# frosinastojanovska/image-captioning

Hardware: AMD Instinct MI355X
Metric: captions/sec (train step) on 1024px x 32RoI x 15tok synth (higher is better)
Workload: dtype f32 (split-bf16x3 products, fp32 accumulate: 73 of 85 conv layers on the bf16 pipe, the rest and the decoder exact fp32 MFMA); 1 GPU; BASELINE configs[2] (configs[3] at 8 GPUs): frozen ResNet-101+FPN fwd + PyramidROIAlign + RoI head + v2-inject decoder fwd/bwd + AMSGrad, 1024x1024 synth images, 32 RoI/img, 15-token captions, V=10000; backbone=resnet101, images_per_gpu=2, global_batch_images=2, parallelism=dp1, stage4_blocks=22, pipeline=encoder(i+1) || decoder(i), 2 HIP streams, rccl_ranks=1

## Files before the change

### image-captioning_amd/_lib.py

```python
import ctypes as C
import os

_HERE = os.path.dirname(os.path.abspath(__file__))
LIB_PATH = os.path.join(_HERE, "csrc", "libdcap_hip.so")

c_float_p = C.POINTER(C.c_float)
c_int32_p = C.POINTER(C.c_int32)
c_uint8_p = C.POINTER(C.c_uint8)


class GemmDesc(C.Structure):
    _fields_ = [("M", C.c_int), ("N", C.c_int), ("K", C.c_int),
                ("A", C.c_void_p), ("lda", C.c_int), ("a_trans", C.c_int),
                ("a_gather", C.c_void_p),
                ("B", C.c_void_p), ("ldb", C.c_int), ("b_trans", C.c_int),
                ("C", C.c_void_p), ("ldc", C.c_int),
                ("scale", C.c_void_p), ("shift", C.c_void_p),
                ("residual", C.c_void_p), ("ldr", C.c_int), ("res_rows", C.c_int),
                ("relu", C.c_int), ("accumulate", C.c_int), ("split_k", C.c_int)]


class GemmBf16Desc(C.Structure):
    _fields_ = [("M", C.c_int), ("N", C.c_int), ("K", C.c_int),
                ("A", C.c_void_p), ("lda", C.c_int), ("a_trans", C.c_int),
# ... 128 lines not shown


class RpnLossDesc(C.Structure):
    _fields_ = [("levels", C.c_int), ("anchors_per_loc", C.c_int), ("head_stride", C.c_int),
                ("heads", C.c_void_p * 5), ("dheads", C.c_void_p * 5), ("Hs", C.c_int * 5), ("Ws", C.c_int * 5),
                ("n_sel", C.c_int), ("n_pos", C.c_int),
                ("sel_level", C.c_void_p), ("sel_index", C.c_void_p), ("sel_match", C.c_void_p),
                ("target_deltas", C.c_void_p), ("losses", C.c_void_p), ("counts_dev", C.c_void_p)]


class DetectionTargetsDesc(C.Structure):
    _fields_ = [("n_proposals", C.c_int), ("n_gt", C.c_int), ("n_rois", C.c_int), ("T", C.c_int),
                ("proposals", C.c_void_p), ("gt_boxes", C.c_void_p), ("gt_captions", C.c_void_p),
                ("max_positive", C.c_int), ("inv_ratio", C.c_float), ("shuffle", C.c_int),
                ("seed", C.c_uint32), ("offset", C.c_uint32), ("offset_dev", C.c_void_p),
                ("rois", C.c_void_p), ("captions", C.c_void_p), ("counts", C.c_void_p)]


class PwChainDesc(C.Structure):
    _fields_ = [("M", C.c_int), ("K1", C.c_int), ("N1", C.c_int), ("N2", C.c_int),
                ("x", C.c_void_p), ("w1", C.c_void_p), ("scale1", C.c_void_p), ("shift1", C.c_void_p), ("residual", C.c_void_p),
                ("relu1", C.c_int), ("y", C.c_void_p), ("w2", C.c_void_p), ("scale2", C.c_void_p), ("shift2", C.c_void_p),
                ("relu2", C.c_int), ("z", C.c_void_p), ("w1_b3", C.c_void_p), ("w2_b3", C.c_void_p)]


class RegSegments(C.Structure):
    _fields_ = [("start", C.c_void_p), ("coef", C.c_void_p), ("mask", C.c_void_p), ("nseg", C.c_int)]


class AmsgradDesc(C.Structure):
    _fields_ = [("n", C.c_size_t), ("p", C.c_void_p), ("g", C.c_void_p), ("m", C.c_void_p),
                ("v", C.c_void_p), ("vhat", C.c_void_p),
                ("lr_t", C.c_float), ("beta1", C.c_float), ("beta2", C.c_float), ("eps", C.c_float),
                ("grad_scale", C.c_float), ("gnorm_sq", C.c_void_p), ("clipnorm", C.c_float),
                ("p_bf16", C.c_void_p), ("n_bf16", C.c_size_t), ("lr_t_dev", C.c_void_p), ("reg", C.POINTER(RegSegments))]


SYMBOLS = {
    "dc_version": (C.c_int, []),
    "dc_last_error": (C.c_char_p, []),
    "dc_gemm_workspace_bytes": (C.c_size_t, [C.POINTER(GemmDesc)]),
    "dc_gemm_f32": (C.c_int, [C.POINTER(GemmDesc), C.c_void_p, C.c_size_t, C.c_void_p]),
    "dc_gemm_bf16_workspace_bytes": (C.c_size_t, [C.POINTER(GemmBf16Desc)]),
    "dc_gemm_bf16_tile": (C.c_int, [C.POINTER(GemmBf16Desc), C.POINTER(C.c_int)]),
    "dc_gemm_bf16": (C.c_int, [C.POINTER(GemmBf16Desc), C.c_void_p, C.c_size_t, C.c_void_p]),
    "dc_conv2d_wgrad_bf16_workspace_bytes": (C.c_size_t, [C.POINTER(ConvWgradBf16Desc)]),
    "dc_conv2d_wgrad_bf16_tile": (C.c_int, [C.POINTER(ConvWgradBf16Desc), C.POINTER(C.c_int)]),
    "dc_conv2d_wgrad_bf16": (C.c_int, [C.POINTER(ConvWgradBf16Desc), C.c_void_p, C.c_size_t, C.c_void_p]),
    "dc_conv2d_bf16_workspace_bytes": (C.c_size_t, [C.POINTER(ConvBf16Desc)]),
    "dc_conv2d_bf16_tile": (C.c_int, [C.POINTER(ConvBf16Desc), C.POINTER(C.c_int)]),
    "dc_conv2d_bf16": (C.c_int, [C.POINTER(ConvBf16Desc), C.c_void_p, C.c_size_t, C.c_void_p]),
    "dc_cast_f32_bf16": (C.c_int, [C.c_void_p, C.c_void_p, C.c_size_t, C.c_void_p]),
    "dc_cast_bf16_f32": (C.c_int, [C.c_void_p, C.c_void_p, C.c_size_t, C.c_void_p]),
    "dc_cast_f32_bf16_2d": (C.c_int, [C.c_void_p, C.c_int, C.c_void_p, C.c_int, C.c_int, C.c_int, C.c_int, C.c_void_p]),
    "dc_split_bf16x3_f32": (C.c_int, [C.c_void_p, C.c_void_p, C.c_size_t, C.c_void_p]),
    "dc_conv2d_workspace_bytes": (C.c_size_t, [C.POINTER(ConvDesc)]),
    "dc_conv2d_nhwc_f32": (C.c_int, [C.POINTER(ConvDesc), C.c_void_p, C.c_size_t, C.c_void_p]),
    "dc_conv2d_tile_config": (C.c_int, [C.POINTER(ConvDesc), C.POINTER(C.c_int), C.POINTER(C.c_int), C.POINTER(C.c_int)]),
    "dc_conv2d_is_pointwise": (C.c_int, [C.POINTER(ConvDesc)]),
    "dc_conv2d_winograd_weight_bytes": (C.c_size_t, [C.c_int, C.c_int]),
    "dc_conv2d_winograd_pack_f32": (C.c_int, [C.c_void_p, C.c_void_p, C.c_int, C.c_int, C.c_void_p]),
    "dc_pw_chain_supported": (C.c_int, [C.c_int, C.c_int, C.c_int]),
    "dc_pw_chain_pack_f32": (C.c_int, [C.c_void_p, C.c_void_p, C.c_int, C.c_int, C.c_void_p]),
    "dc_pw_chain_pack_b3": (C.c_int, [C.c_void_p, C.c_void_p, C.c_int, C.c_int, C.c_void_p]),
    "dc_pw_chain_f32": (C.c_int, [C.POINTER(PwChainDesc), C.c_void_p]),
    "dc_pw_chain_kernel_name": (C.c_int, [C.POINTER(PwChainDesc), C.c_char_p, C.c_size_t]),
    "dc_conv2d_winograd_b3_weight_bytes": (C.c_size_t, [C.c_int, C.c_int]),
    "dc_conv2d_winograd_pack_b3": (C.c_int, [C.c_void_p, C.c_void_p, C.c_int, C.c_int, C.c_void_p]),
    "dc_conv2d_kernel_name": (C.c_int, [C.POINTER(ConvDesc), C.c_char_p, C.c_size_t]),
    "dc_conv2d_wgrad_workspace_bytes": (C.c_size_t, [C.POINTER(ConvDesc)]),
    "dc_conv2d_wgrad_f32": (C.c_int, [C.POINTER(ConvDesc), C.c_void_p, C.c_size_t, C.c_void_p]),
    "dc_roi_align_pyramid_bwd_f32": (C.c_int, [C.POINTER(RoiAlignDesc), C.c_void_p]),
    "dc_downsample2x_sum_f32": (C.c_int, [C.c_void_p, C.c_void_p, C.c_int, C.c_int, C.c_int, C.c_int, C.c_int, C.c_void_p]),
    "dc_downsample2x_sum_dual_f32": (C.c_int, [C.c_void_p, C.c_void_p, C.c_void_p, C.c_int, C.c_int, C.c_int, C.c_int, C.c_int, C.c_void_p]),
    "dc_maxpool2x2s2_f32": (C.c_int, [C.c_void_p, C.c_void_p, C.c_int, C.c_int, C.c_int, C.c_int, C.c_void_p]),
    "dc_maxpool3x3s2_same_f32": (C.c_int, [C.c_void_p, C.c_void_p, C.c_int, C.c_int, C.c_int, C.c_int, C.c_void_p]),
    "dc_mold_image_padded_f32": (C.c_int, [C.c_void_p, C.c_void_p, C.c_int, C.c_int, C.c_int, C.c_int, C.c_float, C.c_float, C.c_float, C.c_void_p]),
    "dc_mold_image_rgbx_f32": (C.c_int, [C.c_void_p, C.c_void_p, C.c_int, C.c_int, C.c_int,
                                         C.c_float, C.c_float, C.c_float, C.c_void_p]),
    "dc_roi_align_pyramid_f32": (C.c_int, [C.POINTER(RoiAlignDesc), C.c_void_p]),
    "dc_roi_tile_groups": (C.c_int, [C.POINTER(RoiGroupsDesc), C.c_void_p]),
    "dc_conv2d_winograd_group_count": (C.c_int, [C.c_int, C.c_int]),
    "dc_conv2d_winograd_groups_f32": (C.c_int, [C.POINTER(ConvDesc), C.c_void_p, C.c_void_p, C.c_void_p]),
    "dc_subsample2_f32": (C.c_int, [C.c_void_p, C.c_void_p, C.c_int, C.c_int, C.c_int, C.c_int, C.c_void_p]),
    "dc_proposals_workspace_bytes": (C.c_size_t, [C.POINTER(ProposalDesc)]),
    "dc_proposals_f32": (C.c_int, [C.POINTER(ProposalDesc), C.c_void_p, C.c_size_t, C.c_void_p]),
    "dc_lstm_seq_workspace_bytes": (C.c_size_t, [C.c_int, C.c_int, C.c_int]),
    "dc_lstm_seq_fwd_f32": (C.c_int, [C.POINTER(LstmFwdDesc), C.c_void_p, C.c_size_t, C.c_void_p]),
    "dc_lstm_seq_bwd_f32": (C.c_int, [C.POINTER(LstmBwdDesc), C.c_void_p, C.c_size_t, C.c_void_p]),
    "dc_lstm_pack_urec_f32": (C.c_int, [C.c_void_p, C.c_int, C.c_void_p, C.c_void_p]),
    "dc_lstm_step_workspace_bytes": (C.c_size_t, [C.c_int, C.c_int]),
    "dc_lstm_step_f32": (C.c_int, [C.POINTER(LstmStepDesc), C.c_void_p, C.c_size_t, C.c_void_p]),
    "dc_softmax_ce_f32": (C.c_int, [C.POINTER(SoftmaxCeDesc), C.c_void_p]),
    "dc_vocab_ce_workspace_bytes": (C.c_size_t, [C.POINTER(VocabCeDesc)]),
    "dc_vocab_ce": (C.c_int, [C.POINTER(VocabCeDesc), C.c_void_p, C.c_size_t, C.c_void_p]),
    "dc_vocab_top1_workspace_bytes": (C.c_size_t, [C.c_int, C.c_int]),
    "dc_vocab_top1_f32": (C.c_int, [C.POINTER(VocabTop1Desc), C.c_void_p, C.c_size_t, C.c_void_p]),
    "dc_vocab_topk_workspace_bytes": (C.c_size_t, [C.c_int, C.c_int, C.c_int]),
    "dc_vocab_topk_f32": (C.c_int, [C.POINTER(VocabTopkDesc), C.c_void_p, C.c_size_t, C.c_void_p]),
    "dc_vocab_topk_bf16_tile": (C.c_int, [C.c_int, C.c_int, C.c_int]),
    "dc_vocab_top1_bf16_workspace_bytes": (C.c_size_t, [C.c_int, C.c_int, C.c_int, C.c_int]),
    "dc_vocab_topk_bf16_workspace_bytes": (C.c_size_t, [C.c_int, C.c_int, C.c_int, C.c_int, C.c_int]),
    "dc_vocab_top1_bf16": (C.c_int, [C.POINTER(VocabTop1Bf16Desc), C.c_void_p, C.c_size_t, C.c_void_p]),
    "dc_vocab_topk_bf16": (C.c_int, [C.POINTER(VocabTopkBf16Desc), C.c_void_p, C.c_size_t, C.c_void_p]),
    "dc_beam_select_f32": (C.c_int, [C.POINTER(BeamSelectDesc), C.c_void_p]),
    "dc_beam_backtrace": (C.c_int, [C.c_void_p, C.c_void_p, C.c_int, C.c_int, C.c_int, C.c_void_p, C.c_void_p]),
    "dc_argmax_rows_f32": (C.c_int, [C.c_void_p, C.c_int, C.c_int, C.c_int, C.c_void_p, C.c_void_p]),
    "dc_gather_rows_f32": (C.c_int, [C.c_void_p, C.c_int, C.c_void_p, C.c_void_p, C.c_int, C.c_int, C.c_int, C.c_void_p]),
    "dc_bn_relu_fwd_f32": (C.c_int, [C.POINTER(BnReluDesc), C.c_void_p]),
    "dc_bn_relu_bwd_f32": (C.c_int, [C.POINTER(BnReluDesc), C.c_void_p]),
    "dc_conv_weight_dgrad_pack_f32": (C.c_int, [C.c_void_p, C.c_void_p, C.c_int, C.c_int, C.c_int, C.c_int, C.c_void_p]),
    "dc_rpn_loss_grad_f32": (C.c_int, [C.POINTER(RpnLossDesc), C.c_void_p]),
    "dc_scatter2_add_f32": (C.c_int, [C.c_void_p, C.c_void_p, C.c_int, C.c_int, C.c_int, C.c_int, C.c_void_p]),
    "dc_detection_targets_f32": (C.c_int, [C.POINTER(DetectionTargetsDesc), C.c_void_p]),
    "dc_caption_tables_i32": (C.c_int, [C.c_void_p, C.c_int, C.c_int, C.c_void_p, C.c_void_p, C.c_void_p, C.c_void_p, C.c_void_p, C.c_void_p]),
    "dc_set_persistent_cus": (C.c_int, [C.c_int]),
    "dc_get_persistent_cus": (C.c_int, []),
    "dc_l2_reg_workspace_bytes": (C.c_size_t, [C.c_size_t]),
    "dc_l2_reg_f32": (C.c_int, [C.c_void_p, C.c_void_p, C.c_void_p, C.c_void_p, C.c_size_t, C.c_void_p, C.c_void_p, C.c_size_t, C.c_void_p]),
    "dc_axpy_f32": (C.c_int, [C.c_float, C.c_void_p, C.c_void_p, C.c_size_t, C.c_void_p]),
    "dc_relu_bwd_f32": (C.c_int, [C.c_void_p, C.c_void_p, C.c_void_p, C.c_int, C.c_int, C.c_int, C.c_void_p]),
    "dc_relu_bwd_dual_f32": (C.c_int, [C.c_void_p, C.c_void_p, C.c_void_p, C.c_void_p, C.c_size_t, C.c_void_p]),
    "dc_fold_time_f32": (C.c_int, [C.c_void_p, C.c_int, C.c_int, C.c_int, C.c_int, C.c_void_p, C.c_int, C.c_void_p]),
    "dc_colsum_workspace_bytes": (C.c_size_t, [C.c_int, C.c_int, C.c_int]),
    "dc_colsum_f32": (C.c_int, [C.c_void_p, C.c_int, C.c_int, C.c_int, C.c_void_p, C.c_int, C.c_void_p, C.c_size_t, C.c_void_p]),
    "dc_sumsq_workspace_bytes": (C.c_size_t, [C.c_size_t]),
    "dc_sumsq_f32": (C.c_int, [C.c_void_p, C.c_size_t, C.c_void_p, C.c_int, C.c_void_p, C.c_size_t, C.c_void_p]),
    "dc_mean_f32": (C.c_int, [C.c_void_p, C.c_size_t, C.c_void_p, C.c_void_p]),
    "dc_bn_fold_f32": (C.c_int, [C.c_void_p] * 5 + [C.c_float, C.c_void_p, C.c_void_p, C.c_int, C.c_void_p]),
    "dc_bn_bwd_f32": (C.c_int, [C.c_void_p] * 8 + [C.c_long, C.c_int, C.c_void_p]),
    "dc_mul_f32": (C.c_int, [C.c_void_p, C.c_void_p, C.c_void_p, C.c_size_t, C.c_void_p]),
    "dc_maxpool3x3s2_same_bwd_f32": (C.c_int, [C.c_void_p] * 4 + [C.c_int] * 4 + [C.c_void_p]),
    "dc_dropout_mask_f32": (C.c_int, [C.c_void_p, C.c_size_t, C.c_float, C.c_uint32, C.c_uint32, C.c_void_p, C.c_void_p]),
    "dc_amsgrad_step_f32": (C.c_int, [C.POINTER(AmsgradDesc), C.c_void_p]),
    "dc_zero_fill": (C.c_int, [C.c_void_p, C.c_size_t, C.c_void_p]),
    "dc_reg_sumsq_workspace_bytes": (C.c_size_t, [C.c_size_t]),
    "dc_reg_sumsq_f32": (C.c_int, [C.c_void_p, C.c_void_p, C.POINTER(RegSegments), C.c_size_t, C.c_void_p, C.c_void_p, C.c_void_p, C.c_size_t, C.c_void_p]),
}

ABI_VERSION = 600
_lib = None


class DcapError(RuntimeError):
    pass


def load():
    global _lib
    if _lib is not None:
        return _lib
    path = os.environ.get("DCAP_LIB", LIB_PATH)
    if not os.path.exists(path):
        raise DcapError("%s is missing: build it with `python __graft_entry__.py` "
                        "(hipcc --offload-arch=gfx950); there is no CPU fallback" % path)
    import torch
    lib = C.CDLL(path)
    for name, (res, args) in SYMBOLS.items():
        fn = getattr(lib, name)
        fn.restype = res
        fn.argtypes = args
    got = lib.dc_version()
    if got // 100 != ABI_VERSION // 100:
        raise DcapError("%s is ABI version %d, these bindings are for %d: rebuild it (python __graft_entry__.py)" % (path, got, ABI_VERSION))
    _lib = lib
    return lib
# ... 7 lines not shown
```

### image-captioning_amd/csrc/conv.hip

```cpp
#include "igemm_core.h"
#include <cstdio>
#include <algorithm>

namespace dcap {

static int conv_validate(const dc_conv_desc* d, bool& stem) {
    DC_REQUIRE(d != nullptr, DC_EINVAL, "dc_conv2d: null descriptor");
    DC_REQUIRE(d->x && d->w && d->y, DC_EINVAL, "dc_conv2d: x, w, y must be non-null");
    DC_REQUIRE(d->N > 0 && d->H > 0 && d->W > 0 && d->Cout > 0 && d->Ho > 0 && d->Wo > 0, DC_EINVAL, "dc_conv2d: bad shape");
    stem = (d->Cin == 4);
    if (stem) {
        DC_REQUIRE(d->kh == 7 && d->kw == 7 && d->stride == 2 && d->pad_t == 3 && d->pad_l == 3, DC_EINVAL,
                   "dc_conv2d: Cin==4 is the RGBX stem path (7x7, stride 2, pad 3) only");
    } else {
        DC_REQUIRE(d->Cin % 32 == 0, DC_EINVAL, "dc_conv2d: Cin must be a multiple of 32 (got %d)", d->Cin);
        DC_REQUIRE(d->kh >= 1 && d->kw >= 1 && d->stride >= 1, DC_EINVAL, "dc_conv2d: bad kernel/stride");
    }
    DC_REQUIRE((d->Ho - 1) * d->stride - d->pad_t + d->kh - 1 < d->H + d->kh && (d->Wo - 1) * d->stride - d->pad_l < d->W,
               DC_EINVAL, "dc_conv2d: output size inconsistent with input/stride/pad");
    DC_REQUIRE(aligned16(d->x) && aligned16(d->w), DC_EALIGN, "dc_conv2d: x and w must be 16-byte aligned");
    DC_REQUIRE((size_t)d->N * d->H * d->W * d->Cin * sizeof(float) < (size_t)0x80000000u &&
                   (size_t)d->Cout * d->kh * d->kw * (stem ? 32 / 7.0 * 7 : d->Cin) * sizeof(float) < (size_t)0xFFFFFFFFu,
               DC_EINVAL, "dc_conv2d: x must be < 2 GiB and w < 4 GiB (32-bit offsets)");
    DC_REQUIRE(d->kh <= 8 && d->kw <= 8, DC_EINVAL, "dc_conv2d: kernel size up to 8x8");
// ... 178 lines not shown
}

using namespace dcap;

extern "C" size_t dc_conv2d_workspace_bytes(const dc_conv_desc* d) {
    bool stem;
    if (conv_validate(d, stem)) return 0;
    int M, N, K;
    conv_dims(d, stem, M, N, K);
    if (!stem && conv_winograd_supported(d)) return 0;
    const TileChoice t = conv_tile(d, M, N, K);
    return t.split > 1 ? (size_t)t.split * M * N * sizeof(float) : 0;
}

extern "C" int dc_conv2d_tile_config(const dc_conv_desc* d, int* bm, int* bn, int* split_k) {
    bool stem;
    int rc = conv_validate(d, stem);
    if (rc) return rc;
    int M, N, K;
    conv_dims(d, stem, M, N, K);
    const TileChoice t = conv_tile(d, M, N, K);
    if (bm) *bm = t.bm;
    if (bn) *bn = t.bn;
    if (split_k) *split_k = t.split;
    return DC_OK;
}

extern "C" int dc_conv2d_kernel_name(const dc_conv_desc* d, char* buf, size_t buf_bytes) {
    bool stem;
    int rc = conv_validate(d, stem);
    if (rc) return rc;
    DC_REQUIRE(buf && buf_bytes >= 96, DC_EINVAL, "dc_conv2d_kernel_name: need a buffer of >= 96 bytes");
    int M, N, K;
    conv_dims(d, stem, M, N, K);
    const TileChoice t = conv_tile(d, M, N, K);
    if (d->math != DC_MATH_F32) {
        snprintf(buf, buf_bytes, "igemm_bs_kernel<%d, %d>", t.bm, t.bn);
        return DC_OK;
    }
    if (!stem && conv_winograd_supported(d)) {
        snprintf(buf, buf_bytes, "wino%d%s_kernel", conv_winograd_tiles(d), conv_winograd_split_bf16(d) ? "b" : "");
        return DC_OK;
    }
    const bool pw = !stem && conv_is_pointwise(d);
    if (pw && t.split == 1 && conv_pw_stream_supported(d, conv_epilogue(d))) {
        snprintf(buf, buf_bytes, "pwconv_stream_kernel<%d, %d>", d->Cin, d->res_mode);
        return DC_OK;
    }
    snprintf(buf, buf_bytes, "%s<%d, %d, dcap::%s, dcap::DenseKCT<true> >", conv_uses_pc(t) ? "igemm_pc_kernel" : "igemm_kernel", t.bm, t.bn,
             stem ? "StemKC" : (pw ? "DenseKCT<true>" : "Im2colKCT<false>"));
    return DC_OK;
}

extern "C" int dc_conv2d_is_pointwise(const dc_conv_desc* d) { return d && d->Cin != 4 && d->math == DC_MATH_F32 && conv_is_pointwise(d) ? 1 : 0; }

extern "C" int dc_conv2d_nhwc_f32(const dc_conv_desc* d, void* workspace, size_t workspace_bytes, void* stream) {
    bool stem;
    int rc = conv_validate(d, stem);
    if (rc) return rc;
    hipStream_t s = static_cast<hipStream_t>(stream);
    int M, N, K;
    conv_dims(d, stem, M, N, K);
    const TileChoice t = conv_tile(d, M, N, K);
    const Epilogue ep = conv_epilogue(d);
    DC_REQUIRE(d->math == DC_MATH_F32 || d->math == DC_MATH_BF16X3 || d->math == DC_MATH_BF16X2 || d->math == DC_MATH_BF16, DC_EINVAL,
               "dc_conv2d: unknown math mode %d", d->math);
    if (d->math != DC_MATH_F32) return conv2d_bf16x3(d, stem, ep, M, N, K, t.bm, t.bn, t.split, workspace, workspace_bytes, s);
    if (!stem && conv_winograd_supported(d)) return conv2d_winograd(d, s);
    WeightKC bl{d->w, K, N, nullptr};
    if (stem) {
        StemKC al{d->x, d->H, d->W, d->Ho, d->Wo, M, (unsigned)((size_t)d->N * d->H * d->W * 4 * sizeof(float))};
        return conv_dispatch(al, bl, ep, M, N, K, t, workspace, workspace_bytes, s);
    }
    if (conv_is_pointwise(d)) {
        if (t.split == 1 && conv_pw_stream_supported(d, ep)) return conv2d_pointwise_stream(d, ep, M, N, s);
        DenseKCT<true> al{d->x, d->Cin, M, nullptr};
        return conv_dispatch(al, bl, ep, M, N, K, t, workspace, workspace_bytes, s);
    }
    Im2colKC al{d->x, d->H, d->W, d->Cin, d->Ho, d->Wo, d->stride, d->pad_t, d->pad_l, d->kw, d->kh * d->kw, M,
                (unsigned)((size_t)d->N * d->H * d->W * d->Cin * sizeof(float))};
    return conv_dispatch(al, bl, ep, M, N, K, t, workspace, workspace_bytes, s);
}

static int wgrad_validate(const dc_conv_desc* d) {
    DC_REQUIRE(d && d->x && d->w && d->y, DC_EINVAL, "dc_conv2d_wgrad: x, dy (y) and dw (w) must be non-null");
    DC_REQUIRE(d->N > 0 && d->H > 0 && d->W > 0 && d->Ho > 0 && d->Wo > 0 && d->kh >= 1 && d->kw >= 1 && d->kh <= 8 && d->kw <= 8 &&
                   d->stride >= 1,
               DC_EINVAL, "dc_conv2d_wgrad: bad shape");
    DC_REQUIRE(d->Cin % 64 == 0 && d->Cout % 4 == 0, DC_EINVAL, "dc_conv2d_wgrad: needs Cin %% 64 == 0 and Cout %% 4 == 0 (pad the head)");
    DC_REQUIRE(aligned16(d->x) && aligned16(d->y) && aligned16(d->w), DC_EALIGN, "dc_conv2d_wgrad: pointers must be 16-byte aligned");
    DC_REQUIRE((size_t)d->N * d->H * d->W * d->Cin * sizeof(float) < (size_t)0x80000000u &&
                   (size_t)d->N * d->Ho * d->Wo * d->Cout * sizeof(float) < (size_t)0xFFFFFFF0u,
               DC_EINVAL, "dc_conv2d_wgrad: x must be < 2 GiB and dy < 4 GiB");
    return DC_OK;
}

static TileChoice wgrad_tile(const dc_conv_desc* d) {
    const int M = d->Cout, N = d->kh * d->kw * d->Cin, K = d->N * d->Ho * d->Wo;
    const bool big = d->Cin % 128 == 0 && d->Cout >= 128 && K % 32 == 0;
    return choose_tile(M, N, K, d->split_k, big);
}

extern "C" size_t dc_conv2d_wgrad_workspace_bytes(const dc_conv_desc* d) {
    if (wgrad_validate(d)) return 0;
    const TileChoice t = wgrad_tile(d);
    return t.split > 1 ? (size_t)t.split * d->Cout * d->kh * d->kw * d->Cin * sizeof(float) : 0;
}

extern "C" int dc_conv2d_wgrad_f32(const dc_conv_desc* d, void* workspace, size_t workspace_bytes, void* stream) {
    int rc = wgrad_validate(d);
    if (rc) return rc;
    const int M = d->Cout, N = d->kh * d->kw * d->Cin, K = d->N * d->Ho * d->Wo;
    const TileChoice t = wgrad_tile(d);
    Epilogue ep{const_cast<float*>(d->w), N, nullptr, nullptr, nullptr, 0, 0, 0, 0, 0, d->accumulate, 1};
    Im2colMC bl{d->x, d->H, d->W, d->Cin, d->Ho, d->Wo, d->stride, d->pad_t, d->pad_l, d->kw, K,
                (unsigned)((size_t)d->N * d->H * d->W * d->Cin * sizeof(float))};
    if (K % 32 == 0) {
        DenseMCT<true> al{d->y, d->Cout, M, nullptr};
        hipStream_t s = static_cast<hipStream_t>(stream);
        if (t.bm == 128 && t.bn == 128)
            return launch_igemm<128, 128, DenseMCT<true>, Im2colMC>(al, bl, ep, M, N, K, t.split, workspace, workspace_bytes, s);
        if (t.bm == 128 && t.bn == 64)
            return launch_igemm<128, 64, DenseMCT<true>, Im2colMC>(al, bl, ep, M, N, K, t.split, workspace, workspace_bytes, s);
        return launch_igemm<64, 64, DenseMCT<true>, Im2colMC, true>(al, bl, ep, M, N, K, t.split, workspace, workspace_bytes, s);
    }
    DenseMCT<false> al{d->y, d->Cout, M, nullptr};
    return launch_igemm<64, 64, DenseMCT<false>, Im2colMC>(al, bl, ep, M, N, K, t.split, workspace, workspace_bytes,
                                                          static_cast<hipStream_t>(stream));
}

__global__ void dgrad_pack_kernel(const float* __restrict__ w, float* __restrict__ out, int Cout, int kh, int kw, int Cin) {
    const long total = (long)Cout * kh * kw * Cin;
    for (long idx = (long)blockIdx.x * blockDim.x + threadIdx.x; idx < total; idx += (long)gridDim.x * blockDim.x) {
        const int co = (int)(idx % Cout);
        long r = idx / Cout;
        const int tap = (int)(r % (kh * kw));
        const int ci = (int)(r / (kh * kw));
        const int ky = tap / kw, kx = tap - ky * kw;
        out[idx] = w[((long)co * kh * kw + (kh - 1 - ky) * kw + (kw - 1 - kx)) * Cin + ci];
    }
}

__global__ void scatter2_add_kernel(const float4* __restrict__ coarse, float4* __restrict__ fine, int N, int Hc, int Wc, int C4) {
    const long total = (long)N * Hc * Wc * C4;
    for (long idx = (long)blockIdx.x * blockDim.x + threadIdx.x; idx < total; idx += (long)gridDim.x * blockDim.x) {
        const int c = (int)(idx % C4);
        long p = idx / C4;
        const int x = (int)(p % Wc);
        p /= Wc;
        const int y = (int)(p % Hc), n = (int)(p / Hc);
        const long o = (((long)n * 2 * Hc + 2 * y) * 2 * Wc + 2 * x) * C4 + c;
        float4 f = fine[o];
        const float4 q = coarse[idx];
        f.x += q.x; f.y += q.y; f.z += q.z; f.w += q.w;
        fine[o] = f;
    }
}

extern "C" int dc_conv_weight_dgrad_pack_f32(const float* w, float* out, int Cout, int kh, int kw, int Cin, void* stream) {
    DC_REQUIRE(w && out && Cout > 0 && kh > 0 && kw > 0 && Cin > 0, DC_EINVAL, "dc_conv_weight_dgrad_pack: bad arguments");
    const long total = (long)Cout * kh * kw * Cin;
    const int blocks = (int)std::min<long>((total + 255) / 256, (long)kNumCU * 8);
    hipLaunchKernelGGL(dgrad_pack_kernel, dim3(blocks), dim3(256), 0, static_cast<hipStream_t>(stream), w, out, Cout, kh, kw, Cin);
    return check_launch("dgrad_pack_kernel");
}

// ... 103 lines not shown
```

### image-captioning_amd/csrc/conv_bs.hip

```cpp
#include "igemm_bf16s.h"
#include <algorithm>

namespace dcap {

using WeightKCb = DenseKCT<true>;

template <class AL, class BL>
static int dispatch_bs(const AL& al, const BL& bl, const Epilogue& ep, int M, int N, int K, int bm, int bn, int split, void* ws,
                       size_t wsb, hipStream_t s, int pieces) {
    if (pieces == 1) {
        if (bm == 128 && bn == 128) return launch_igemm_bs<128, 128, AL, BL, 1>(al, bl, ep, M, N, K, split, ws, wsb, s);
        if (bm == 128 && bn == 64) return launch_igemm_bs<128, 64, AL, BL, 1>(al, bl, ep, M, N, K, split, ws, wsb, s);
        return launch_igemm_bs<64, 64, AL, BL, 1>(al, bl, ep, M, N, K, split, ws, wsb, s);
    }
    if (pieces == 2) {
        if (bm == 128 && bn == 128) return launch_igemm_bs<128, 128, AL, BL, 2>(al, bl, ep, M, N, K, split, ws, wsb, s);
        if (bm == 128 && bn == 64) return launch_igemm_bs<128, 64, AL, BL, 2>(al, bl, ep, M, N, K, split, ws, wsb, s);
        return launch_igemm_bs<64, 64, AL, BL, 2>(al, bl, ep, M, N, K, split, ws, wsb, s);
    }
    if (bm == 128 && bn == 128) return launch_igemm_bs<128, 128, AL, BL>(al, bl, ep, M, N, K, split, ws, wsb, s);
    if (bm == 128 && bn == 64) return launch_igemm_bs<128, 64, AL, BL>(al, bl, ep, M, N, K, split, ws, wsb, s);
    return launch_igemm_bs<64, 64, AL, BL>(al, bl, ep, M, N, K, split, ws, wsb, s);
}

__global__ __launch_bounds__(256) void split_bf16x3_kernel(const float* __restrict__ x, unsigned short* __restrict__ out, size_t n) {
    const size_t pairs = (n + 1) / 2;
    for (size_t i = (size_t)blockIdx.x * 256 + threadIdx.x; i < pairs; i += (size_t)gridDim.x * 256) {
        const float a = x[2 * i], b = (2 * i + 1 < n) ? x[2 * i + 1] : 0.f;
        unsigned p0, p1, p2;
        split_pair(a, b, p0, p1, p2);
        out[2 * i] = (unsigned short)p0; out[n + 2 * i] = (unsigned short)p1; out[2 * n + 2 * i] = (unsigned short)p2;
        if (2 * i + 1 < n) {
            out[2 * i + 1] = (unsigned short)(p0 >> 16); out[n + 2 * i + 1] = (unsigned short)(p1 >> 16); out[2 * n + 2 * i + 1] = (unsigned short)(p2 >> 16);
        }
    }
}

int conv2d_bf16x3(const dc_conv_desc* d, bool stem, const Epilogue& ep, int M, int N, int K, int bm, int bn, int split, void* workspace,
                  size_t workspace_bytes, hipStream_t s) {
    const int pieces = d->math == DC_MATH_BF16 ? 1 : (d->math == DC_MATH_BF16X2 ? 2 : 3);
    if (stem) {
        WeightKCb bl{d->w, K, N, nullptr};
        StemKC al{d->x, d->H, d->W, d->Ho, d->Wo, M, (unsigned)((size_t)d->N * d->H * d->W * 4 * sizeof(float))};
        return dispatch_bs(al, bl, ep, M, N, K, bm, bn, split, workspace, workspace_bytes, s, pieces);
    }
    ConvWeightKC bl{d->w, K, N, d->kh * d->kw, d->Cin};
    Im2colKCcm al{d->x, d->H, d->W, d->Cin, d->Ho, d->Wo, d->stride, d->pad_t, d->pad_l, d->kw, d->kh * d->kw, M,
                (unsigned)((size_t)d->N * d->H * d->W * d->Cin * sizeof(float))};
    return dispatch_bs(al, bl, ep, M, N, K, bm, bn, split, workspace, workspace_bytes, s, pieces);
}

}

extern "C" int dc_split_bf16x3_f32(const float* x, uint16_t* out, size_t n, void* stream) {
    using namespace dcap;
    DC_REQUIRE(x && out && n > 0, DC_EINVAL, "dc_split_bf16x3: bad arguments");
    const int blocks = (int)std::min<size_t>((n / 2 + 255) / 256 + 1, (size_t)kNumCU * 8);
    hipLaunchKernelGGL(split_bf16x3_kernel, dim3(blocks), dim3(256), 0, static_cast<hipStream_t>(stream), x, out, n);
    return check_launch("split_bf16x3_kernel");
}
```

### image-captioning_amd/csrc/conv_wino.hip

```cpp
#include "igemm_bf16s.h"
#include <algorithm>

namespace dcap {
namespace wino {

constexpr int NTHREADS = 256;

struct Args {
    const float* x;
    const f4* u;
    float* y;
    const float* scale;
    const float* shift;
    int N, H, W, Cin, Cout, relu;
    int gy, gx, groups;
    unsigned x_bytes, u_bytes;
    const int* glist;
    const int* gcount;
};

__global__ void wino_pack_kernel(const float* __restrict__ w, float* __restrict__ u, int Cin, int Cout) {
    const long total = (long)Cin * Cout;
    const int NTG = Cout / 32, KC = Cin / 16;
    for (long idx = (long)blockIdx.x * blockDim.x + threadIdx.x; idx < total; idx += (long)gridDim.x * blockDim.x) {
        const int cin = (int)(idx % Cin), cout = (int)(idx / Cin);
        float g[3][3];
#pragma unroll
        for (int t = 0; t < 9; ++t) g[t / 3][t % 3] = w[((long)cout * 9 + t) * Cin + cin];
        float gg[4][3];
#pragma unroll
        for (int c = 0; c < 3; ++c) {
            gg[0][c] = g[0][c];
            gg[1][c] = 0.5f * (g[0][c] + g[1][c] + g[2][c]);
            gg[2][c] = 0.5f * (g[0][c] - g[1][c] + g[2][c]);
            gg[3][c] = g[2][c];
        }
        const int ntg = cout >> 5, i = cout & 31, kc = cin >> 4, kk = cin & 15, h = kk >> 3, j = (kk & 7) >> 2, e = kk & 3;
#pragma unroll
        for (int a = 0; a < 4; ++a) {
            const float r[4] = {gg[a][0], 0.5f * (gg[a][0] + gg[a][1] + gg[a][2]), 0.5f * (gg[a][0] - gg[a][1] + gg[a][2]), gg[a][2]};
#pragma unroll
            for (int b = 0; b < 4; ++b) {
                const int xi = 4 * a + b;
                u[((((long)(xi * NTG + ntg) * KC + kc) * 2 + j) * 64 + (h * 32 + i)) * 4 + e] = r[b];
            }
        }
    }
}

__global__ void wino_pack_b3_kernel(const float* __restrict__ w, unsigned short* __restrict__ u, int Cin, int Cout) {
    const long total = (long)Cin * Cout;
    const int NTG = Cout / 32, KC = Cin / 16;
    for (long idx = (long)blockIdx.x * blockDim.x + threadIdx.x; idx < total; idx += (long)gridDim.x * blockDim.x) {
        const int cin = (int)(idx % Cin), cout = (int)(idx / Cin);
        float g[3][3];
#pragma unroll
        for (int t = 0; t < 9; ++t) g[t / 3][t % 3] = w[((long)cout * 9 + t) * Cin + cin];
        float gg[4][3];
#pragma unroll
        for (int c = 0; c < 3; ++c) {
            gg[0][c] = g[0][c];
            gg[1][c] = 0.5f * (g[0][c] + g[1][c] + g[2][c]);
            gg[2][c] = 0.5f * (g[0][c] - g[1][c] + g[2][c]);
            gg[3][c] = g[2][c];
        }
        const int ntg = cout >> 5, i = cout & 31, kc = cin >> 4, kk = cin & 15, h = kk >> 3, jj = kk & 7;
#pragma unroll
        for (int a = 0; a < 4; ++a) {
            const float r[4] = {gg[a][0], 0.5f * (gg[a][0] + gg[a][1] + gg[a][2]), 0.5f * (gg[a][0] - gg[a][1] + gg[a][2]), gg[a][2]};
#pragma unroll
            for (int b = 0; b < 4; ++b) {
                const int xi = 4 * a + b;
                float x = r[b];
#pragma unroll
                for (int piece = 0; piece < 3; ++piece) {
                    const unsigned short pb = __builtin_bit_cast(unsigned short, (__bf16)x);
                    x -= __uint_as_float((unsigned)pb << 16);
                    u[((((long)(xi * NTG + ntg) * KC + kc) * 3 + piece) * 64 + (h * 32 + i)) * 8 + jj] = pb;
                }
            }
        }
    }
}

__device__ __forceinline__ unsigned img32_addr(int xi, int tile, int chunk) {
    return (unsigned)((((xi * 32 + tile) << 3) + (chunk ^ ((tile >> 1) & 7))) << 4);
}
__device__ __forceinline__ void bt_cols(const f4 (&t)[4], f4 (&v)[4]) {
    v[0] = t[0] - t[2];
    v[1] = t[1] + t[2];
    v[2] = t[2] - t[1];
    v[3] = t[1] - t[3];
}

namespace wp {
constexpr int PW = 18, NDMA = 6;
__device__ __forceinline__ int patch_index(int y, int x) { return y * PW + (x >> 1) + (PW / 2) * (x & 1); }
__device__ __forceinline__ int patch_swizzle(int y, int x) { return ((x >> 2) & 1) | (((y >> 1) & 3) << 1); }
template <int HALVES>
struct Cfg {
    static constexpr int NT = 256 * HALVES, TGY = kWinoTGY * HALVES, TGX = kWinoTGX, PH = 2 * TGY + 2, NPIX = PH * PW, SLOTS = NPIX * 8;
    static constexpr int BUF = 32768 * HALVES;
    static constexpr int LDS_BYTES = 2 * BUF;
    static_assert(NDMA * NT >= SLOTS && NDMA * NT * 16 <= BUF, "patch buffer; the kernel issues the pieces three per step");
};
}

typedef unsigned u32x4 __attribute__((ext_vector_type(4)));

__device__ __forceinline__ void split8(const f4& va, const f4& vb, u32x4& p0, u32x4& p1, u32x4& p2) {
    unsigned a0, a1, a2, b0, b1, b2, c0, c1, c2, d0, d1, d2;
    split_pair(va[0], va[1], a0, a1, a2);
    split_pair(va[2], va[3], b0, b1, b2);
    split_pair(vb[0], vb[1], c0, c1, c2);
    split_pair(vb[2], vb[3], d0, d1, d2);
    p0 = u32x4{a0, b0, c0, d0};
    p1 = u32x4{a1, b1, c1, d1};
    p2 = u32x4{a2, b2, c2, d2};
}
__device__ __forceinline__ f32x16 mfma_b(const u32x4& a, const u32x4& b, const f32x16& c) {
    return __builtin_amdgcn_mfma_f32_32x32x16_bf16(__builtin_bit_cast(bf16x8, a), __builtin_bit_cast(bf16x8, b), c, 0, 0, 0);
}

template <int HALVES, bool B3, int NCH = 1, bool LIST = false>
__device__ __forceinline__ void wino_body(const Args& a) {
    static_assert(NCH == 1 || (NCH == 2 && HALVES == 1 && B3), "64-channel items: the split-bf16 32-tile kernel only");
    static_assert(!LIST || (HALVES == 1 && B3), "list-driven item walk: the split-bf16 32-tile kernel only");
    using namespace wp;
    typedef Cfg<HALVES> C;
    constexpr int NT64 = C::NT, SLOTS = C::SLOTS, BUF = C::BUF;
    extern __shared__ __attribute__((aligned(16))) char smem[];
    const int tid = threadIdx.x, lane = tid & 63;
    const int wave = __builtin_amdgcn_readfirstlane(tid >> 6);
    const int wa = wave & 3, th = wave >> 2;
    const int gpi = a.gy * a.gx;
    const int NTG = a.Cout >> 5, KC = a.Cin >> 4, KP = a.Cin >> 5;
    int groups = a.groups;
    if constexpr (LIST) groups = min(max(*a.gcount, 0), a.groups);
    const int total = groups * (NTG / NCH);
    const __amdgpu_buffer_rsrc_t rsrc = __builtin_amdgcn_make_buffer_rsrc(const_cast<float*>(a.x), 0, (int)a.x_bytes, 0x00020000);

    int nb, img, gyi, gxi;
    unsigned doff[NDMA];
    const f4* ubase;
    unsigned ubyte3;
    auto setup = [&](int item) {
        const int bid = xcd_remap(item, total);
        nb = bid / groups;
        int g = bid - nb * groups;
        if constexpr (LIST) g = min(max(a.glist[g], 0), a.groups - 1);
        img = g / gpi;
        const int gr = g - img * gpi;
        gyi = gr / a.gx;
        gxi = gr - gyi * a.gx;
#pragma unroll
        for (int n = 0; n < NDMA; ++n) {
            const int s = n * NT64 + tid, pq = s >> 3, py = pq / PW, rem = pq - py * PW;
            const int px = rem < PW / 2 ? 2 * rem : 2 * (rem - PW / 2) + 1;
            const int iy = gyi * 2 * C::TGY - 1 + py, ix = gxi * 2 * C::TGX - 1 + px;
            const bool in = s < SLOTS && (unsigned)iy < (unsigned)a.H && (unsigned)ix < (unsigned)a.W;
            const int c8 = (s & 7) ^ patch_swizzle(py, px);
            doff[n] = in ? (unsigned)(((((long)img * a.H + iy) * a.W + ix) * a.Cin + 4 * c8) * 4) : kOobOffset;
        }
        ubase = a.u + lane + (((long)(4 * wa) * NTG + nb) * KC << 7);
        ubyte3 = (unsigned)((4 * wa) * NTG + NCH * nb) * (unsigned)KC * 3072u;
    };
    auto issue_dma_pieces = [&](int pair, int buf, int n0, int n1) {
#pragma unroll
        for (int n = n0; n < n1; ++n)
            __builtin_amdgcn_raw_ptr_buffer_load_lds(rsrc, (__attribute__((address_space(3))) void*)(smem + buf * BUF + (n * NT64 + wave * 64) * 16), 16,
                                                     (int)doff[n], pair * 128, 0, 0);
    };
    auto issue_dma = [&](int pair, int buf) { issue_dma_pieces(pair, buf, 0, NDMA); };
    const long ustep = (long)NTG * KC << 7;
    auto load_u_part = [&](f4 (&dst)[4][2], int kc, int b0, int b1) {
#pragma unroll
        for (int b = b0; b < b1; ++b) {
            const f4* p = ubase + b * ustep + ((long)kc << 7);
            dst[b][0] = p[0];
            dst[b][1] = p[64];
        }
    };
    auto load_u = [&](f4 (&dst)[4][2], int kc) { load_u_part(dst, kc, 0, 4); };
    const __amdgpu_buffer_rsrc_t rsrc_u = __builtin_amdgcn_make_buffer_rsrc(const_cast<f4*>(a.u), 0, (int)a.u_bytes, 0x00020000);
    const unsigned ustep3 = (unsigned)NTG * KC * 3 * 1024u;
    auto load_u3 = [&](u32x4 (&dst)[3], int kc, int b, int hc) {
        const unsigned so = __builtin_amdgcn_readfirstlane(ubyte3 + (unsigned)b * ustep3 + (unsigned)(hc * KC + kc) * 3072u);
        dst[0] = __builtin_bit_cast(u32x4, buf_f4s(rsrc_u, (unsigned)lane * 16u, so));
        dst[1] = __builtin_bit_cast(u32x4, buf_f4s(rsrc_u, (unsigned)lane * 16u, so + 1024u));
        dst[2] = __builtin_bit_cast(u32x4, buf_f4s(rsrc_u, (unsigned)lane * 16u, so + 2048u));
    };

    const int fi = lane & 31, fh = lane >> 5;
    const int tile = 32 * th + fi, tyl = tile >> 3, txl = tile & 7;
    const int r1 = (wa == 0) ? 0 : (wa == 2 ? 2 : 1), r2 = (wa == 0 || wa == 1) ? 2 : (wa == 2 ? 1 : 3);
    const float sgn = (wa == 1) ? 1.f : -1.f;
    unsigned paddr[2][4];
#pragma unroll
    for (int rr = 0; rr < 2; ++rr)
#pragma unroll
        for (int c = 0; c < 4; ++c) {
            const int py = 2 * tyl + (rr ? r2 : r1), px = 2 * txl + c;
            paddr[rr][c] = (unsigned)(patch_index(py, px) * 128 + (((2 * fh) ^ patch_swizzle(py, px)) << 4));
        }
    auto read_d = [&](f4 (&d)[2][4], int st) {
        const unsigned k = (unsigned)(((st & 1) << 4) ^ ((st >> 1) << 6));
#pragma unroll
        for (int rr = 0; rr < 2; ++rr)
#pragma unroll
            for (int c = 0; c < 4; ++c) d[rr][c] = *reinterpret_cast<const f4*>(smem + (paddr[rr][c] ^ k));
    };
    auto transform = [&](const f4 (&d)[2][4], f4 (&v)[4]) {
        f4 t[4];
#pragma unroll
        for (int c = 0; c < 4; ++c) t[c] = d[1][c] * sgn + d[0][c];
        bt_cols(t, v);
    };

    int item = blockIdx.x;
    if (item >= total) return;
    setup(item);
    issue_dma(0, 0);
    f4 ub[2][4][2];
    u32x4 u3[4][3];
    u32x4 w0[2][2], w1[2], w2[2];
    auto load_piece = [&](u32x4& dst, int kc, int b, int hc, int piece) {
        const unsigned so = __builtin_amdgcn_readfirstlane(ubyte3 + (unsigned)b * ustep3 + (unsigned)(hc * KC + kc) * 3072u + (unsigned)piece * 1024u);
        dst = __builtin_bit_cast(u32x4, buf_f4s(rsrc_u, (unsigned)lane * 16u, so));
    };
    auto load_u3_first = [&]() {
        if constexpr (NCH == 2) {
#pragma unroll
            for (int hc = 0; hc < 2; ++hc) {
                load_piece(w0[0][hc], 0, 0, hc, 0);
                load_piece(w1[hc], 0, 0, hc, 1);
                load_piece(w2[hc], 0, 0, hc, 2);
                load_piece(w0[1][hc], 0, 1, hc, 0);
            }
        } else {
#pragma unroll
            for (int b = 0; b < 4; ++b) load_u3(u3[b], 0, b, 0);
        }
    };
    if constexpr (B3) {
        load_u3_first();
    } else {
        load_u(ub[0], 0);
    }
    for (;;) {
        f32x16 acc[NCH][4];
#pragma unroll
        for (int hc = 0; hc < NCH; ++hc)
#pragma unroll
            for (int b = 0; b < 4; ++b)
#pragma unroll
                for (int r = 0; r < 16; ++r) acc[hc][b][r] = 0.f;
        auto pair = [&](int p, auto more_c) {
            constexpr bool more = decltype(more_c)::value;
            asm volatile("s_waitcnt vmcnt(0)" ::: "memory");
            __syncthreads();
            if constexpr (B3 && NCH == 2) {
                f4 t0[4], t1[4];
                u32x4 V[2][3];
                auto fetch_col = [&](int hf, int c) {
                    const unsigned ka = (unsigned)(hf << 6), kb = ka ^ 16u;
                    const f4 a0 = *reinterpret_cast<const f4*>(smem + (paddr[0][c] ^ ka));
                    const f4 a1 = *reinterpret_cast<const f4*>(smem + (paddr[1][c] ^ ka));
// ... 78 lines not shown
                    const int half = q >> 2, b = q & 3;
                    if (q == 1) read_d(dA, 2);
                    if (q == 2) read_d(dB, 3);
                    __builtin_amdgcn_sched_barrier(0);
                    if constexpr (more) if (q < NDMA) issue_dma_pieces(p + 1, (p + 1) & 1, q, q + 1);
                    const u32x4 (&vq)[3] = V[q & 1];
                    acc[0][b] = mfma_b(u3[b][0], vq[2], acc[0][b]);
                    acc[0][b] = mfma_b(u3[b][1], vq[1], acc[0][b]);
                    acc[0][b] = mfma_b(u3[b][2], vq[0], acc[0][b]);
                    acc[0][b] = mfma_b(u3[b][1], vq[0], acc[0][b]);
                    acc[0][b] = mfma_b(u3[b][0], vq[1], acc[0][b]);
                    acc[0][b] = mfma_b(u3[b][0], vq[0], acc[0][b]);
                    if (q == 3) make_t();
                    if (q < 7) prep(V[(q + 1) & 1], (q + 1) & 3);
                    load_u3(u3[b], min(2 * p + half + 1, KC - 1), b, 0);
#pragma unroll
                    for (int m = 0; m < 6; ++m) {
                        __builtin_amdgcn_sched_group_barrier(0x008, 1, 0);
                        __builtin_amdgcn_sched_group_barrier(0x020, 1, 0);
                        if (q == 3) __builtin_amdgcn_sched_group_barrier(0x002, 15, 0);
                        else __builtin_amdgcn_sched_group_barrier(0x002, 9, 0);
                    }
                    __builtin_amdgcn_sched_barrier(0);
                }
#pragma unroll
                for (int rr = 0; rr < 2; ++rr)
#pragma unroll
                    for (int c = 0; c < 4; ++c) paddr[rr][c] ^= (unsigned)BUF;
                return;
            }
            f4 d[2][4], vcur[4], vnext[4];
            read_d(d, 0);
            transform(d, vcur);
#pragma unroll
            for (int st = 0; st < 4; ++st) {
                const int half = st >> 1, j = st & 1;
                if (st < 3) read_d(d, st + 1);
                __builtin_amdgcn_sched_barrier(0);
                if constexpr (more) if (st < 2) issue_dma_pieces(p + 1, (p + 1) & 1, 3 * st, 3 * st + 3);
                load_u_part(ub[half ^ 1], min(2 * p + half + 1, KC - 1), 2 * j, 2 * j + 2);
#pragma unroll
                for (int e = 0; e < 2; ++e)
#pragma unroll
                    for (int b = 0; b < 4; ++b) acc[0][b] = __builtin_amdgcn_mfma_f32_32x32x2f32(ub[half][b][j][e], vcur[b][e], acc[0][b], 0, 0, 0);
#pragma unroll
                for (int m = 0; m < 8; ++m) {
                    __builtin_amdgcn_sched_group_barrier(0x008, 1, 0);
                    __builtin_amdgcn_sched_group_barrier(0x020, 1, 0);
                }
                __builtin_amdgcn_sched_barrier(0);
                if (st < 3) transform(d, vnext);
#pragma unroll
                for (int e = 2; e < 4; ++e)
#pragma unroll
                    for (int b = 0; b < 4; ++b) acc[0][b] = __builtin_amdgcn_mfma_f32_32x32x2f32(ub[half][b][j][e], vcur[b][e], acc[0][b], 0, 0, 0);
                if (st < 3) {
#pragma unroll
                    for (int m = 0; m < 8; ++m) {
                        __builtin_amdgcn_sched_group_barrier(0x008, 1, 0);
                        __builtin_amdgcn_sched_group_barrier(0x002, 4, 0);
                    }
                }
                __builtin_amdgcn_sched_barrier(0);
                if (st < 3) {
#pragma unroll
                    for (int b = 0; b < 4; ++b) vcur[b] = vnext[b];
                }
            }
#pragma unroll
            for (int rr = 0; rr < 2; ++rr)
#pragma unroll
                for (int c = 0; c < 4; ++c) paddr[rr][c] ^= (unsigned)BUF;
        };
        for (int p = 0; p < KP - 1; ++p) pair(p, std::true_type{});
        pair(KP - 1, std::false_type{});
        if (KP & 1) {
#pragma unroll
            for (int rr = 0; rr < 2; ++rr)
#pragma unroll
                for (int c = 0; c < 4; ++c) paddr[rr][c] ^= (unsigned)BUF;
        }

        const int onb = nb, oimg = img, ogy = gyi, ogx = gxi;
        const int next = item + (int)gridDim.x;
        const int oq = tid & 7, ocout = onb * (32 * NCH) + 4 * oq;
        f4 sc[NCH], sh[NCH];
#pragma unroll
        for (int hc = 0; hc < NCH; ++hc) {
            sc[hc] = a.scale ? *reinterpret_cast<const f4*>(a.scale + ocout + 32 * hc) : (f4)(1.f);
            sh[hc] = a.shift ? *reinterpret_cast<const f4*>(a.shift + ocout + 32 * hc) : (f4)(0.f);
        }
        __syncthreads();
        if (next < total) {
            setup(next);
            issue_dma(0, 0);
            if constexpr (B3) {
                load_u3_first();
            } else {
                load_u(ub[0], 0);
            }
        }
#pragma unroll
        for (int hc = 0; hc < NCH; ++hc) {
            if (hc) __syncthreads();
            {
                const f32x16 s0 = acc[hc][0] + acc[hc][1] + acc[hc][2], s1 = acc[hc][1] - acc[hc][2] - acc[hc][3];
#pragma unroll
                for (int gq = 0; gq < 4; ++gq) {
                    const f4 m0 = {s0[4 * gq], s0[4 * gq + 1], s0[4 * gq + 2], s0[4 * gq + 3]};
                    const f4 m1 = {s1[4 * gq], s1[4 * gq + 1], s1[4 * gq + 2], s1[4 * gq + 3]};
                    *reinterpret_cast<f4*>(smem + BUF + th * 32768 + img32_addr(2 * wa, fi, 2 * gq + fh)) = m0;
                    *reinterpret_cast<f4*>(smem + BUF + th * 32768 + img32_addr(2 * wa + 1, fi, 2 * gq + fh)) = m1;
                }
            }
            __syncthreads();
            {
                const int oth = tid >> 8, ti = (tid >> 3) & 31;
                f4 sv[4][2];
#pragma unroll
                for (int r = 0; r < 4; ++r)
#pragma unroll
                    for (int qx = 0; qx < 2; ++qx) sv[r][qx] = *reinterpret_cast<const f4*>(smem + BUF + oth * 32768 + img32_addr(2 * r + qx, ti, oq));
                const int otile = 32 * oth + ti, ty = ogy * C::TGY + (otile >> 3), tx = ogx * C::TGX + (otile & 7), cout = ocout + 32 * hc;
#pragma unroll
                for (int qx = 0; qx < 2; ++qx) {
                    const f4 o[2] = {sv[0][qx] + sv[1][qx] + sv[2][qx], sv[1][qx] - sv[2][qx] - sv[3][qx]};
#pragma unroll
                    for (int pr = 0; pr < 2; ++pr) {
                        f4 val = o[pr] * sc[hc] + sh[hc];
                        if (a.relu) val = f4{fmaxf(val[0], 0.f), fmaxf(val[1], 0.f), fmaxf(val[2], 0.f), fmaxf(val[3], 0.f)};
                        if (2 * ty + pr < a.H && 2 * tx + qx < a.W)
                            *reinterpret_cast<f4*>(a.y + (((long)oimg * a.H + 2 * ty + pr) * a.W + 2 * tx + qx) * a.Cout + cout) = val;
                    }
                }
            }
        }
        if (next >= total) break;
        item = next;
    }
}

__global__ __launch_bounds__(512, 1) void wino64_kernel(Args a) { wino_body<2, false>(a); }
__global__ __launch_bounds__(256, 2) void wino32_kernel(Args a) { wino_body<1, false>(a); }
__global__ __launch_bounds__(512, 1) void wino64b_kernel(Args a) { wino_body<2, true>(a); }
template <int NCH>
__global__ __launch_bounds__(256, 2) void wino32b_kernel(Args a) { wino_body<1, true, NCH>(a); }
template __global__ void wino32b_kernel<1>(Args);
template __global__ void wino32b_kernel<2>(Args);
template <int NCH>
__global__ __launch_bounds__(256, 2) void wino32b_list_kernel(Args a) { wino_body<1, true, NCH, true>(a); }
template __global__ void wino32b_list_kernel<1>(Args);
template __global__ void wino32b_list_kernel<2>(Args);

}

static bool wino_shape_ok(const dc_conv_desc* d, const void* u) {
    return u != nullptr && d->math == DC_MATH_F32 && d->kh == 3 && d->kw == 3 && d->stride == 1 && d->pad_t == 1 && d->pad_l == 1 &&
           d->Ho == d->H && d->Wo == d->W && d->Cin % 32 == 0 && d->Cout % 32 == 0 && d->res_mode == 0 && d->split_k <= 1 && aligned16(d->y) &&
           aligned16(u) && (!d->scale || aligned16(d->scale)) && (!d->shift || aligned16(d->shift)) &&
           (size_t)d->N * d->H * d->W * d->Cin * sizeof(float) < (1ull << 31);
}

static bool wino_b3(const dc_conv_desc* d) { return wino_shape_ok(d, d->w_wino_b3); }
bool conv_winograd_supported(const dc_conv_desc* d) { return wino_b3(d) || wino_shape_ok(d, d->w_wino); }
bool conv_winograd_split_bf16(const dc_conv_desc* d) { return wino_b3(d); }

static int wino_force() {
    static const int force = env_int("DCAP_WINO_TILES", 0);
    return force;
}

static std::atomic<int> g_persistent_cus{-1};
static int persistent_cus() {
    int v = g_persistent_cus.load(std::memory_order_relaxed);
    if (v < 0) {
        static const int env = env_int("DCAP_WINO_CUS", kNumCU);
        v = env;
    }
    v = std::max(8, std::min(v, kNumCU));
    return v / 8 * 8;
}

int conv_winograd_tiles(const dc_conv_desc* d) {
    const int force = wino_force();
    if (force == 32 || force == 64) return force;
    if (wino_b3(d)) return 32;
    const int th = (d->H + 1) / 2, tw = (d->W + 1) / 2;
    const long items64 = (long)d->N * ((th + 7) / 8) * ((tw + 7) / 8) * (d->Cout / 32);
    return items64 >= kNumCU ? 64 : 32;
}

static int wino_cout_force() {
    static const int force = env_int("DCAP_WINO_COUT", 0);
    return force;
}

static int conv_winograd_cout(const dc_conv_desc* d) {
    if (!wino_b3(d) || conv_winograd_tiles(d) != 32 || d->Cout % 64) return 32;
    const int force = wino_cout_force();
    if (force == 32 || force == 64) return force;
    const int th = (d->H + 1) / 2, tw = (d->W + 1) / 2;
    const long items = (long)d->N * ((th + 3) / 4) * ((tw + 7) / 8) * (d->Cout / 64);
    return items >= 2 * kNumCU ? 64 : 32;
}

static int wino_args(const dc_conv_desc* d, bool b3, bool big, wino::Args& a) {
    a.x = d->x;
    a.u = b3 ? reinterpret_cast<const f4*>(d->w_wino_b3) : reinterpret_cast<const f4*>(d->w_wino);
    a.y = d->y;
    a.scale = d->scale;
    a.shift = d->shift;
    a.N = d->N; a.H = d->H; a.W = d->W; a.Cin = d->Cin; a.Cout = d->Cout; a.relu = d->relu;
    const size_t x_bytes = (size_t)d->N * d->H * d->W * d->Cin * sizeof(float);
    DC_REQUIRE(x_bytes < (1ull << 31), DC_EINVAL, "dc_conv2d (winograd): the input tensor has %zu bytes, the kernel addresses < 2 GiB", x_bytes);
    a.x_bytes = (unsigned)x_bytes;
    a.u_bytes = (unsigned)((size_t)16 * d->Cin * d->Cout * (b3 ? 6 : 4));
    a.gy = big ? (wino_groups_y(d->H) + 1) / 2 : wino_groups_y(d->H);
    a.gx = wino_groups_x(d->W);
    a.groups = d->N * a.gy * a.gx;
    a.glist = nullptr;
    a.gcount = nullptr;
    return DC_OK;
}

int conv2d_winograd(const dc_conv_desc* d, hipStream_t s) {
    wino::Args a;
    const bool b3 = wino_b3(d);
    const bool big = conv_winograd_tiles(d) == 64;
    const int rc = wino_args(d, b3, big, a);
    if (rc) return rc;
    const bool wide = b3 && !big && conv_winograd_cout(d) == 64;
    const long items = (long)a.groups * (d->Cout / (wide ? 64 : 32));
    DC_REQUIRE(items < (1l << 31), DC_EINVAL, "dc_conv2d (winograd): grid too large");
    const int per_cu = big ? 1 : 2;
    const long full = (long)per_cu * kNumCU;
    const long slots = items >= 8 * full ? per_cu * persistent_cus() : full;
    const unsigned grid = items >= slots ? (unsigned)slots : (unsigned)std::max<long>(8, items / 8 * 8);
    if (b3 && big) {
        DC_ENSURE_DYN_LDS(wino::wino64b_kernel, wino::wp::Cfg<2>::LDS_BYTES);
        hipLaunchKernelGGL(wino::wino64b_kernel, dim3(grid), dim3(wino::wp::Cfg<2>::NT), wino::wp::Cfg<2>::LDS_BYTES, s, a);
    } else if (wide) {
        DC_ENSURE_DYN_LDS((&wino::wino32b_kernel<2>), wino::wp::Cfg<1>::LDS_BYTES);
        hipLaunchKernelGGL((wino::wino32b_kernel<2>), dim3(grid), dim3(wino::wp::Cfg<1>::NT), wino::wp::Cfg<1>::LDS_BYTES, s, a);
    } else if (b3) {
        DC_ENSURE_DYN_LDS((&wino::wino32b_kernel<1>), wino::wp::Cfg<1>::LDS_BYTES);
        hipLaunchKernelGGL((wino::wino32b_kernel<1>), dim3(grid), dim3(wino::wp::Cfg<1>::NT), wino::wp::Cfg<1>::LDS_BYTES, s, a);
    } else if (big) {
        DC_ENSURE_DYN_LDS(wino::wino64_kernel, wino::wp::Cfg<2>::LDS_BYTES);
        hipLaunchKernelGGL(wino::wino64_kernel, dim3(grid), dim3(wino::wp::Cfg<2>::NT), wino::wp::Cfg<2>::LDS_BYTES, s, a);
    } else {
        DC_ENSURE_DYN_LDS(wino::wino32_kernel, wino::wp::Cfg<1>::LDS_BYTES);
        hipLaunchKernelGGL(wino::wino32_kernel, dim3(grid), dim3(wino::wp::Cfg<1>::NT), wino::wp::Cfg<1>::LDS_BYTES, s, a);
    }
    return check_launch("dc_conv2d (winograd)");
}

int conv2d_winograd_groups(const dc_conv_desc* d, const int* glist, const int* gcount, hipStream_t s) {
    wino::Args a;
    const int rc = wino_args(d, true, false, a);
    if (rc) return rc;
    a.glist = glist;
    a.gcount = gcount;
    const bool wide = wino_cout_force() == 64 && d->Cout % 64 == 0;
    const long items = (long)a.groups * (d->Cout / (wide ? 64 : 32));
    DC_REQUIRE(items < (1l << 31), DC_EINVAL, "dc_conv2d_winograd_groups: grid too large");
    const long full = 2L * kNumCU;
    const unsigned grid = items >= full ? (unsigned)full : (unsigned)std::max<long>(8, items / 8 * 8);
    if (wide) {
        DC_ENSURE_DYN_LDS((&wino::wino32b_list_kernel<2>), wino::wp::Cfg<1>::LDS_BYTES);
        hipLaunchKernelGGL((wino::wino32b_list_kernel<2>), dim3(grid), dim3(wino::wp::Cfg<1>::NT), wino::wp::Cfg<1>::LDS_BYTES, s, a);
    } else {
        DC_ENSURE_DYN_LDS((&wino::wino32b_list_kernel<1>), wino::wp::Cfg<1>::LDS_BYTES);
        hipLaunchKernelGGL((wino::wino32b_list_kernel<1>), dim3(grid), dim3(wino::wp::Cfg<1>::NT), wino::wp::Cfg<1>::LDS_BYTES, s, a);
    }
    return check_launch("dc_conv2d_winograd_groups_f32");
}

}

using namespace dcap;

extern "C" int dc_conv2d_winograd_groups_f32(const dc_conv_desc* d, const int32_t* groups, const int32_t* count, void* stream) {
    DC_REQUIRE(d && d->x && d->y && groups && count, DC_EINVAL, "dc_conv2d_winograd_groups: null pointer");
    DC_REQUIRE(d->N > 0 && d->H > 0 && d->W > 0, DC_EINVAL, "dc_conv2d_winograd_groups: bad N/H/W");
    DC_REQUIRE(wino_b3(d), DC_EINVAL,
               "dc_conv2d_winograd_groups: the layer must be one the split-bf16 Winograd kernel takes (3x3, stride 1, pad 1, Cin and Cout "
               "multiples of 32, no residual, fp32 math, w_wino_b3 given, 16-byte aligned operands, input below 2 GiB)");
    return conv2d_winograd_groups(d, groups, count, static_cast<hipStream_t>(stream));
}

extern "C" int dc_conv2d_winograd_group_count(int H, int W) {
    if (H <= 0 || W <= 0) return 0;
    return wino_groups_y(H) * wino_groups_x(W);
}

extern "C" size_t dc_conv2d_winograd_weight_bytes(int Cin, int Cout) {
    if (Cin <= 0 || Cout <= 0 || Cin % 32 || Cout % 32) return 0;
    return (size_t)16 * Cin * Cout * sizeof(float);
}

extern "C" int dc_conv2d_winograd_pack_f32(const float* w, float* u, int Cin, int Cout, void* stream) {
    DC_REQUIRE(w && u, DC_EINVAL, "dc_conv2d_winograd_pack: null pointer");
    DC_REQUIRE(Cin > 0 && Cout > 0 && Cin % 32 == 0 && Cout % 32 == 0, DC_EINVAL, "dc_conv2d_winograd_pack: Cin and Cout must be multiples of 32");
    DC_REQUIRE(aligned16(u), DC_EALIGN, "dc_conv2d_winograd_pack: u must be 16-byte aligned");
    const long total = (long)Cin * Cout;
    const int blocks = (int)std::min<long>((total + 255) / 256, 4096);
    hipLaunchKernelGGL(wino::wino_pack_kernel, dim3(blocks), dim3(256), 0, static_cast<hipStream_t>(stream), w, u, Cin, Cout);
    return check_launch("dc_conv2d_winograd_pack_f32");
}

extern "C" size_t dc_conv2d_winograd_b3_weight_bytes(int Cin, int Cout) {
    if (Cin <= 0 || Cout <= 0 || Cin % 32 || Cout % 32) return 0;
    return (size_t)16 * Cin * Cout * 3 * sizeof(uint16_t);
}

extern "C" int dc_conv2d_winograd_pack_b3(const float* w, uint16_t* u, int Cin, int Cout, void* stream) {
    DC_REQUIRE(w && u, DC_EINVAL, "dc_conv2d_winograd_pack_b3: null pointer");
    DC_REQUIRE(Cin > 0 && Cout > 0 && Cin % 32 == 0 && Cout % 32 == 0, DC_EINVAL, "dc_conv2d_winograd_pack_b3: Cin and Cout must be multiples of 32");
    DC_REQUIRE(aligned16(u), DC_EALIGN, "dc_conv2d_winograd_pack_b3: u must be 16-byte aligned");
    const long total = (long)Cin * Cout;
    const int blocks = (int)std::min<long>((total + 255) / 256, 4096);
    hipLaunchKernelGGL(wino::wino_pack_b3_kernel, dim3(blocks), dim3(256), 0, static_cast<hipStream_t>(stream), w, u, Cin, Cout);
    return check_launch("dc_conv2d_winograd_pack_b3");
}

extern "C" int dc_set_persistent_cus(int n) {
    DC_REQUIRE(n == 0 || (n >= 8 && n <= kNumCU), DC_EINVAL, "dc_set_persistent_cus: 0 (default: DCAP_WINO_CUS or all 256) or 8..256, got %d", n);
    dcap::g_persistent_cus.store(n == 0 ? -1 : n, std::memory_order_relaxed);
    return DC_OK;
}

extern "C" int dc_get_persistent_cus(void) { return dcap::persistent_cus(); }
```

### image-captioning_amd/csrc/igemm_bf16s.h

```cpp
#pragma once
#include "igemm_core.h"

namespace dcap {

typedef __bf16 bf16x4 __attribute__((ext_vector_type(4)));
typedef __bf16 bf16x8 __attribute__((ext_vector_type(8)));

constexpr int LDB = BK + 8;

__device__ __forceinline__ unsigned cvt_pk_bf16(float lo, float hi) {
    unsigned r;
    asm("v_cvt_pk_bf16_f32 %0, %1, %2" : "=v"(r) : "v"(lo), "v"(hi));
    return r;
}
__device__ __forceinline__ void split_pair(float a, float b, unsigned& p0, unsigned& p1, unsigned& p2) {
    p0 = cvt_pk_bf16(a, b);
    a -= __uint_as_float(p0 << 16);
    b -= __uint_as_float(p0 & 0xffff0000u);
    p1 = cvt_pk_bf16(a, b);
    a -= __uint_as_float(p1 << 16);
    b -= __uint_as_float(p1 & 0xffff0000u);
    p2 = cvt_pk_bf16(a, b);
}

typedef unsigned u32x2 __attribute__((ext_vector_type(2)));

template <int BT, int NR, int NP = 3>
__device__ __forceinline__ void store_split_kc(__bf16* S, const f4 (&r)[NR], int tid) {
    static_assert(NR == BT / 32, "one f4 per 32 staged rows");
    const int q = tid & 7, rr = tid >> 3;
#pragma unroll
    for (int i = 0; i < BT / 32; ++i) {
        __bf16* d = S + (rr + 32 * i) * LDB + 4 * q;
        if constexpr (NP == 1) {
            *reinterpret_cast<u32x2*>(d) = u32x2{cvt_pk_bf16(r[i][0], r[i][1]), cvt_pk_bf16(r[i][2], r[i][3])};
            continue;
        }
        unsigned a0, a1, a2, b0, b1, b2;
        split_pair(r[i][0], r[i][1], a0, a1, a2);
        split_pair(r[i][2], r[i][3], b0, b1, b2);
        *reinterpret_cast<u32x2*>(d) = u32x2{a0, b0};
        *reinterpret_cast<u32x2*>(d + BT * LDB) = u32x2{a1, b1};
        if constexpr (NP == 3) *reinterpret_cast<u32x2*>(d + 2 * BT * LDB) = u32x2{a2, b2};
    }
}

template <int BM, int BN, int NP = 3>
constexpr size_t igemm_bs_lds_bytes() {
    constexpr size_t stage = (size_t)NP * (BM + BN) * LDB * sizeof(__bf16);
    constexpr size_t cimage = (size_t)BM * (BN + 4) * sizeof(float);
    return stage > cimage ? stage : cimage;
}

template <int BM, int BN, class AL, class BL, int NP = 3>
__global__ __launch_bounds__(256, 2) void igemm_bs_kernel(AL al, BL bl, Epilogue ep, int M, int N, int K, int klen,
                                                       float* __restrict__ partial) {
    static_assert(AL::KC && BL::KC, "split-bf16 main loop: both operands K-contiguous");
    extern __shared__ __attribute__((aligned(16))) float smem[];
    constexpr int TM = BM / 64, TN = BN / 64;
    __bf16* As = reinterpret_cast<__bf16*>(smem);
    __bf16* Bs = As + NP * BM * LDB;

    const int tid = threadIdx.x, lane = tid & 63, wave = tid >> 6;
    const int tiles_n = (N + BN - 1) / BN;
    const int lid = xcd_remap(blockIdx.x, gridDim.x);
    const int m0 = (lid / tiles_n) * BM, n0 = (lid % tiles_n) * BN;
    const int kbeg = blockIdx.z * klen;
    const int kend = min(K, kbeg + klen);
    const int wm = (wave >> 1) * (BM / 2), wn = (wave & 1) * (BN / 2);
    const int li = lane & 31, lh = lane >> 5;

    typename AL::template State<BM> sa;
    typename BL::template State<BN> sb;
    al.template init<BM>(sa, m0, tid);
    bl.template init<BN>(sb, n0, tid);

    f32x16 acc[TM][TN];
#pragma unroll
    for (int tm = 0; tm < TM; ++tm)
#pragma unroll
        for (int tn = 0; tn < TN; ++tn)
#pragma unroll
            for (int r = 0; r < 16; ++r) acc[tm][tn][r] = 0.f;

    f4 ra[2][BM / 32], rb[2][BN / 32];
    const int nkt = (kend - kbeg + BK - 1) / BK;
#pragma unroll
    for (int j = 0; j < 2; ++j) {
        const int k0 = kbeg + j * BK;
        al.template load<BM>(sa, ra[j], al.kclamp(k0, kend), kend, tid);
        bl.template load<BN>(sb, rb[j], bl.kclamp(k0, kend), kend, tid);
    }

    const __bf16* afrag = As + (wm + li) * LDB + 8 * lh;
    const __bf16* bfrag = Bs + (wn + li) * LDB + 8 * lh;

    auto phase = [&](int kt, f4 (&qa)[BM / 32], f4 (&qb)[BN / 32]) {
        store_split_kc<BM, BM / 32, NP>(As, qa, tid);
        store_split_kc<BN, BN / 32, NP>(Bs, qb, tid);
        __syncthreads();
        {
            const int k0 = kbeg + (kt + 2) * BK;
            al.template load<BM>(sa, qa, al.kclamp(k0, kend), kend, tid);
            bl.template load<BN>(sb, qb, bl.kclamp(k0, kend), kend, tid);
        }
#pragma unroll
        for (int s = 0; s < BK / 16; ++s) {
            bf16x8 a[TM][NP], b[TN][NP];
#pragma unroll
            for (int p = 0; p < NP; ++p) {
#pragma unroll
                for (int tm = 0; tm < TM; ++tm) a[tm][p] = *reinterpret_cast<const bf16x8*>(afrag + (p * BM + tm * 32) * LDB + 16 * s);
#pragma unroll
                for (int tn = 0; tn < TN; ++tn) b[tn][p] = *reinterpret_cast<const bf16x8*>(bfrag + (p * BN + tn * 32) * LDB + 16 * s);
            }
#pragma unroll
            for (int tm = 0; tm < TM; ++tm)
#pragma unroll
                for (int tn = 0; tn < TN; ++tn) {
                    f32x16 c = acc[tm][tn];
                    if constexpr (NP == 3) {
                        c = __builtin_amdgcn_mfma_f32_32x32x16_bf16(a[tm][2], b[tn][0], c, 0, 0, 0);
                        c = __builtin_amdgcn_mfma_f32_32x32x16_bf16(a[tm][1], b[tn][1], c, 0, 0, 0);
                        c = __builtin_amdgcn_mfma_f32_32x32x16_bf16(a[tm][0], b[tn][2], c, 0, 0, 0);
                    }
                    if constexpr (NP >= 2) {
                        c = __builtin_amdgcn_mfma_f32_32x32x16_bf16(a[tm][1], b[tn][0], c, 0, 0, 0);
                        c = __builtin_amdgcn_mfma_f32_32x32x16_bf16(a[tm][0], b[tn][1], c, 0, 0, 0);
                    }
                    c = __builtin_amdgcn_mfma_f32_32x32x16_bf16(a[tm][0], b[tn][0], c, 0, 0, 0);
                    acc[tm][tn] = c;
                }
        }
        __syncthreads();
    };
    for (int kt = 0; kt < nkt; kt += 2) {
        phase(kt, ra[0], rb[0]);
        if (kt + 1 < nkt) phase(kt + 1, ra[1], rb[1]);
    }
    store_tile<BM, BN>(acc, smem, ep, partial, M, N, m0, n0, wm, wn);
}

template <int BM, int BN, class AL, class BL, int NP = 3>
int launch_igemm_bs(const AL& al, const BL& bl, const Epilogue& ep, int M, int N, int K, int split_k, void* workspace,
                    size_t workspace_bytes, hipStream_t stream) {
    const int tiles = ((M + BM - 1) / BM) * ((N + BN - 1) / BN);
    const int ktiles = (K + BK - 1) / BK;
    if (split_k < 1) split_k = 1;
    if (split_k > ktiles) split_k = ktiles;
    const int klen = ((ktiles + split_k - 1) / split_k) * BK;
    split_k = (K + klen - 1) / klen;
    float* partial = nullptr;
    if (split_k > 1) {
        const size_t need = (size_t)split_k * M * N * sizeof(float);
        DC_REQUIRE(workspace != nullptr && workspace_bytes >= need, DC_EWORKSPACE,
                   "igemm split-K needs %zu workspace bytes, got %zu", need, workspace_bytes);
        partial = static_cast<float*>(workspace);
    }
    constexpr size_t lds = igemm_bs_lds_bytes<BM, BN, NP>();
    DC_ENSURE_DYN_LDS((&igemm_bs_kernel<BM, BN, AL, BL, NP>), 160 * 1024);
    dim3 grid(tiles, 1, split_k);
    hipLaunchKernelGGL((igemm_bs_kernel<BM, BN, AL, BL, NP>), grid, dim3(256), lds, stream, al, bl, ep, M, N, K, klen, partial);
    int rc = check_launch("igemm_bs_kernel");
    if (rc) return rc;
    if (split_k > 1) {
        const long total = (long)M * N;
        hipLaunchKernelGGL(splitk_reduce_kernel, dim3(splitk_reduce_blocks(total)), dim3(256), 0, stream, partial, split_k, M, N, ep);
        rc = check_launch("splitk_reduce_kernel");
    }
    return rc;
}

}
```

### image-captioning_amd/csrc/igemm_core.h

```cpp
#pragma once
#include <math.h>
#include "dcap_internal.h"
#include <stdlib.h>

namespace dcap {

typedef float f32x16 __attribute__((ext_vector_type(16)));
typedef float f4 __attribute__((ext_vector_type(4)));
__device__ __forceinline__ f4 f4_zero() { return (f4)(0.f); }

constexpr int BK = 32;
constexpr int LDKC = BK + 4;


template <int BT>
__device__ __forceinline__ void store_kc(float* S, const f4 (&r)[BT / 32], int tid) {
    const int q = tid & 7, rr = tid >> 3;
#pragma unroll
    for (int i = 0; i < BT / 32; ++i) *reinterpret_cast<f4*>(&S[(rr + 32 * i) * LDKC + 4 * q]) = r[i];
}

template <int BT>
__device__ __forceinline__ void store_mc(float* S, const f4 (&r)[BT / 32], int tid) {
    constexpr int QPR = BT / 4, RPP = 256 / QPR;
// ... 192 lines not shown
            s.rsrc = __builtin_amdgcn_make_buffer_rsrc(const_cast<float*>(x), 0, (int)x_bytes, 0x00020000);
        } else {
            const long bias = ((long)pad_t * W + pad_l) * Cin;
            s.rsrc = __builtin_amdgcn_make_buffer_rsrc(const_cast<float*>(x) - bias, 0, (int)(x_bytes + bias * 4), 0x00020000);
        }
        s.ky = -1;
        s.fresh = 1;
#pragma unroll
        for (int i = 0; i < BT / 32; ++i) {
            const int m = min(row0 + rr + 32 * i, M - 1);
            const int n = m / (Ho * Wo), rem = m - n * (Ho * Wo);
            const int oy = rem / Wo, ox = rem - oy * Wo;
            s.boff[i] = (unsigned)(((((long)n * H + oy * stride) * W + ox * stride) * Cin + 4 * (tid & 7)) * 4);
            unsigned ym = 0, xm = 0;
            for (int t = 0; t < 8; ++t) {
                ym |= ((unsigned)(oy * stride - pad_t + t) < (unsigned)H) ? (1u << t) : 0u;
                xm |= ((unsigned)(ox * stride - pad_l + t) < (unsigned)W) ? (1u << t) : 0u;
            }
            unsigned long long mk = 0;
            for (int ty = 0; ty < 8; ++ty)
                if ((ym >> ty) & 1u) mk |= (unsigned long long)(xm & ((1u << kw) - 1u)) << (ty * kw);
            s.mask[i] = mk;
        }
    }
    template <int BT>
    __device__ __forceinline__ void load(State<BT>& s, f4 (&r)[BT / 32], int k0, int kend, int tid) const {
        if (s.ky < 0) {
            const int kt = k0 >> 5;
            int tap;
            if constexpr (CM) {
                const int chunk = kt / taps;
                tap = kt - chunk * taps;
                s.c = chunk * 32;
            } else {
                const int cin_tiles = Cin >> 5;
                tap = kt / cin_tiles;
                s.c = (kt - tap * cin_tiles) * 32;
            }
            s.ky = tap / kw;
            s.kx = tap - s.ky * kw;
        }
        const int ky = s.ky, kx = s.kx;
        const int tap = ky * kw + kx;
        if constexpr (CM) {
            const int ubytes = (((ky - pad_t) * W + (kx - pad_l)) * Cin + s.c) * 4;
#pragma unroll
            for (int i = 0; i < BT / 32; ++i) {
                const bool in = tap < taps && ((s.mask[i] >> (tap & 63)) & 1ull) != 0;
                r[i] = buf_f4(s.rsrc, in ? s.boff[i] + (unsigned)ubytes : kOobOffset);
            }
        } else {
            if (s.fresh) {
                s.fresh = 0;
#pragma unroll
                for (int i = 0; i < BT / 32; ++i)
                    s.sel[i] = (tap < taps && ((s.mask[i] >> (tap & 63)) & 1ull)) ? s.boff[i] : kOobOffset;
            }
            const unsigned soff = (unsigned)(((ky * W + kx) * Cin + s.c) * 4);
#pragma unroll
            for (int i = 0; i < BT / 32; ++i) r[i] = buf_f4s(s.rsrc, s.sel[i], soff);
        }
        if constexpr (CM) {
            if (++s.kx == kw) {
                s.kx = 0;
                if ((s.ky + 1) * kw == taps) { s.ky = 0; s.c += 32; } else { ++s.ky; }
            }
        } else {
            s.c += 32;
            if (s.c == Cin) {
                s.c = 0;
                s.fresh = 1;
                if (++s.kx == kw) { s.kx = 0; ++s.ky; }
            }
        }
    }
    template <int BT>
    __device__ __forceinline__ void store(const State<BT>&, float* S, f4 (&r)[BT / 32], int tid) const {
        store_kc<BT>(S, r, tid);
    }
};

using Im2colKC = Im2colKCT<false>;
using Im2colKCcm = Im2colKCT<true>;

struct Im2colMC {
    static constexpr bool KC = false;
    __device__ __forceinline__ int kclamp(int k0, int) const { return k0; }
    const float* x;
    int H, W, Cin, Ho, Wo, stride, pad_t, pad_l, kw, P;
    unsigned x_bytes;
    template <int BT>
    struct State {
        __amdgpu_buffer_rsrc_t rsrc;
        int oy[BT / 32], ox[BT / 32], n[BT / 32];
        int dy, dx;
        unsigned coff;
        int started;
    };
    template <int BT>
    __device__ __forceinline__ void init(State<BT>& s, int col0, int tid) const {
        constexpr int QPR = BT / 4;
        s.rsrc = __builtin_amdgcn_make_buffer_rsrc(const_cast<float*>(x), 0, (int)x_bytes, 0x00020000);
        const int tap = col0 / Cin, ci0 = col0 - tap * Cin;
        const int ky = tap / kw, kx = tap - ky * kw;
        s.dy = ky - pad_t;
        s.dx = kx - pad_l;
        s.coff = (unsigned)((ci0 + 4 * (tid % QPR)) * 4);
        s.started = 0;
    }
    template <int BT>
    __device__ __forceinline__ void load(State<BT>& s, f4 (&r)[BT / 32], int k0, int kend, int tid) const {
        constexpr int QPR = BT / 4, RPP = 256 / QPR;
        if (!s.started) {
            s.started = 1;
#pragma unroll
            for (int i = 0; i < BT / 32; ++i) {
                const int p = k0 + tid / QPR + RPP * i;
                const int n = p / (Ho * Wo), rem = p - n * (Ho * Wo);
                s.n[i] = n;
                s.oy[i] = rem / Wo;
                s.ox[i] = rem - s.oy[i] * Wo;
            }
        }
#pragma unroll
        for (int i = 0; i < BT / 32; ++i) {
            const int iy = s.oy[i] * stride + s.dy, ix = s.ox[i] * stride + s.dx;
            const bool in = (unsigned)iy < (unsigned)H && (unsigned)ix < (unsigned)W && s.n[i] * (Ho * Wo) + s.oy[i] * Wo + s.ox[i] < min(P, kend);
            const unsigned off = (unsigned)((((long)s.n[i] * H + iy) * W + ix) * Cin * 4) + s.coff;
            r[i] = buf_f4(s.rsrc, in ? off : kOobOffset);
            s.ox[i] += BK;
            while (s.ox[i] >= Wo) { s.ox[i] -= Wo; ++s.oy[i]; }
            while (s.oy[i] >= Ho) { s.oy[i] -= Ho; ++s.n[i]; }
        }
    }
    template <int BT>
    __device__ __forceinline__ void store(const State<BT>&, float* S, f4 (&r)[BT / 32], int tid) const {
        store_mc<BT>(S, r, tid);
    }
};

struct StemKC {
    static constexpr bool KC = true;
    __device__ __forceinline__ int kclamp(int k0, int) const { return k0; }
    const float* x;
    int H, W, Ho, Wo, M;
    unsigned x_bytes;
    template <int BT>
    struct State {
        __amdgpu_buffer_rsrc_t rsrc;
        unsigned boff[BT / 32];
        unsigned mask[BT / 32];
    };
    template <int BT>
    __device__ __forceinline__ void init(State<BT>& s, int row0, int tid) const {
        const int rr = tid >> 3, q = tid & 7;
        s.rsrc = __builtin_amdgcn_make_buffer_rsrc(const_cast<float*>(x), 0, (int)x_bytes, 0x00020000);
#pragma unroll
        for (int i = 0; i < BT / 32; ++i) {
            const int m = min(row0 + rr + 32 * i, M - 1);
            const int n = m / (Ho * Wo), rem = m - n * (Ho * Wo);
            const int oy = rem / Wo, ox = rem - oy * Wo;
            s.boff[i] = (unsigned)((((long)n * H + oy * 2) * W + ox * 2) * 16);
            unsigned mk = ((unsigned)(ox * 2 - 3 + q) < (unsigned)W) ? (1u << 8) : 0u;
            for (int t = 0; t < 7; ++t) mk |= ((unsigned)(oy * 2 - 3 + t) < (unsigned)H) ? (1u << t) : 0u;
            s.mask[i] = mk;
        }
// ... 157 lines not shown
    auto prefetch = [&](int p0) {
#pragma unroll
        for (int g = 0; g < G; ++g) {
            const int row = min(m0 + (p0 + g) * RPP + rp, M - 1);
            if (pre_res) qres[g] = *reinterpret_cast<const f4*>(ep.res_row(row) + col);
            if (pre_acc) qacc[g] = *reinterpret_cast<const f4*>(ep.C + (long)row * ep.ldc + col);
        }
    };
    prefetch(0);
    float* Cs = smem;
    {
        const int i = lane & 31, h = lane >> 5;
#pragma unroll
        for (int tm = 0; tm < TM; ++tm)
#pragma unroll
            for (int tn = 0; tn < TN; ++tn)
#pragma unroll
                for (int r = 0; r < 16; ++r)
                    Cs[(wm + tm * 32 + (r & 3) + 8 * (r >> 2) + 4 * h) * LDC + wn + tn * 32 + i] = acc[tm][tn][r];
    }
    __syncthreads();
    if (col >= N) return;
    if (partial) {
        float* prow = partial + (long)blockIdx.z * M * N;
#pragma unroll 4
        for (int p = 0; p < PASSES; ++p) {
            const int lr = p * RPP + rp, row = m0 + lr;
            if (row >= M) break;
            const float4 v = *reinterpret_cast<const float4*>(&Cs[lr * LDC + 4 * c4]);
            float* o = prow + (long)row * N + col;
            if ((N & 3) == 0) {
                *reinterpret_cast<float4*>(o) = v;
            } else {
                o[0] = v.x;
                if (col + 1 < N) o[1] = v.y;
                if (col + 2 < N) o[2] = v.z;
                if (col + 3 < N) o[3] = v.w;
            }
        }
        return;
    }
    if (full) {
        float4 sc = make_float4(1.f, 1.f, 1.f, 1.f), sh = make_float4(0.f, 0.f, 0.f, 0.f);
        if (ep.scale) sc = *reinterpret_cast<const float4*>(ep.scale + col);
        if (ep.shift) sh = *reinterpret_cast<const float4*>(ep.shift + col);
#pragma unroll
        for (int p0 = 0; p0 < PASSES; p0 += G) {
            if (p0 > 0) prefetch(p0);
#pragma unroll
            for (int g = 0; g < G; ++g) {
                const int lr = (p0 + g) * RPP + rp, row = m0 + lr;
                float4 v = *reinterpret_cast<const float4*>(&Cs[lr * LDC + 4 * c4]);
                v.x = v.x * sc.x + sh.x; v.y = v.y * sc.y + sh.y; v.z = v.z * sc.z + sh.z; v.w = v.w * sc.w + sh.w;
                if (pre_res) { v.x += qres[g][0]; v.y += qres[g][1]; v.z += qres[g][2]; v.w += qres[g][3]; }
                if (ep.relu) { v.x = fmaxf(v.x, 0.f); v.y = fmaxf(v.y, 0.f); v.z = fmaxf(v.z, 0.f); v.w = fmaxf(v.w, 0.f); }
                if (pre_acc) { v.x += qacc[g][0]; v.y += qacc[g][1]; v.z += qacc[g][2]; v.w += qacc[g][3]; }
                if (row < M) {
                    if (ep.C) *reinterpret_cast<float4*>(ep.C + (long)row * ep.ldc + col) = v;
                    if (ep.Cb) {
                        typedef unsigned short us4 __attribute__((ext_vector_type(4)));
                        *reinterpret_cast<us4*>(ep.Cb + (long)row * ep.ldcb + col) =
                            us4{Epilogue::bf16_bits(v.x), Epilogue::bf16_bits(v.y), Epilogue::bf16_bits(v.z), Epilogue::bf16_bits(v.w)};
                    }
                }
            }
        }
        return;
    }
#pragma unroll 4
    for (int p = 0; p < PASSES; ++p) {
        const int lr = p * RPP + rp, row = m0 + lr;
        if (row >= M) break;
        const float4 v = *reinterpret_cast<const float4*>(&Cs[lr * LDC + 4 * c4]);
        float* crow = ep.C + (long)row * ep.ldc;
        const float* rr = ep.res_row(row);
#define DC_TAIL(j, e)                                                                                       \
    if (col + j < N)                                                                                        \
        ep.put(row, col + j, ep.finish(e, ep.scale ? ep.scale[col + j] : 1.f, ep.shift ? ep.shift[col + j] : 0.f, rr, crow, col + j));
        DC_TAIL(0, v.x) DC_TAIL(1, v.y) DC_TAIL(2, v.z) DC_TAIL(3, v.w)
#undef DC_TAIL
    }
}

template <int BM, int BN, class AL, class BL>
__device__ __forceinline__ void igemm_mainloop(const AL& al, const BL& bl, float* smem, int m0, int n0, int kbeg, int kend,
                                               f32x16 (&acc)[BM / 64][BN / 64], int wm, int wn) {
    constexpr int TM = BM / 64, TN = BN / 64;
    constexpr int A_FL = lds_floats<BM, AL::KC>(), B_FL = lds_floats<BN, BL::KC>(), STAGE = A_FL + B_FL;
    const int tid = threadIdx.x, lane = tid & 63;
    typename AL::template State<BM> sa;
    typename BL::template State<BN> sb;
    al.template init<BM>(sa, m0, tid);
    bl.template init<BN>(sb, n0, tid);

#pragma unroll
    for (int tm = 0; tm < TM; ++tm)
#pragma unroll
        for (int tn = 0; tn < TN; ++tn)
#pragma unroll
            for (int r = 0; r < 16; ++r) acc[tm][tn][r] = 0.f;

    constexpr int KT = tiles_per_sync<BM, BN>();
    f4 ra[KT][BM / 32], rb[KT][BN / 32];
    const int nkt = (kend - kbeg + BK - 1) / BK;
#pragma unroll
    for (int j = 0; j < KT; ++j)
        if (j < nkt) {
            al.template load<BM>(sa, ra[j], kbeg + j * BK, kend, tid);
            bl.template load<BN>(sb, rb[j], kbeg + j * BK, kend, tid);
        }
#pragma unroll
    for (int j = 0; j < KT; ++j)
        if (j < nkt) {
            al.template store<BM>(sa, smem + j * STAGE, ra[j], tid);
            bl.template store<BN>(sb, smem + j * STAGE + A_FL, rb[j], tid);
        }
    __syncthreads();
    auto step = [&](int kt, float* cur, float* nxt) {
#pragma unroll
        for (int j = 0; j < KT; ++j) {
            const int k0 = kbeg + (kt + KT + j) * BK;
            al.template load<BM>(sa, ra[j], al.kclamp(k0, kend), kend, tid);
            bl.template load<BN>(sb, rb[j], bl.kclamp(k0, kend), kend, tid);
        }
#pragma unroll
        for (int j = 0; j < KT; ++j)
            if (kt + j < nkt) mma_tile<BM, BN, AL::KC, BL::KC>(cur + j * STAGE, cur + j * STAGE + A_FL, acc, wm, wn, lane);
#pragma unroll
        for (int j = 0; j < KT; ++j)
            if (kt + KT + j < nkt) {
                al.template store<BM>(sa, nxt + j * STAGE, ra[j], tid);
                bl.template store<BN>(sb, nxt + j * STAGE + A_FL, rb[j], tid);
            }
        __syncthreads();
    };
    float* const stage0 = smem;
    float* const stage1 = smem + KT * STAGE;
    for (int kt = 0; kt < nkt; kt += 2 * KT) {
        step(kt, stage0, stage1);
        if (kt + KT < nkt) step(kt + KT, stage1, stage0);
    }

}

template <int BM, int BN, class AL, class BL>
__global__ __launch_bounds__(256, 2) void igemm_kernel(AL al, BL bl, Epilogue ep, int M, int N, int K, int klen,
                                                    float* __restrict__ partial) {
    extern __shared__ __attribute__((aligned(16))) float smem[];
    const int wave = threadIdx.x >> 6;
    const int tiles_n = (N + BN - 1) / BN;
    const int lid = xcd_remap(blockIdx.x, gridDim.x);
    const int m0 = (lid / tiles_n) * BM, n0 = (lid % tiles_n) * BN;
    const int kbeg = blockIdx.z * klen;
    const int kend = min(K, kbeg + klen);
    const int wm = (wave >> 1) * (BM / 2), wn = (wave & 1) * (BN / 2);
    f32x16 acc[BM / 64][BN / 64];
    igemm_mainloop<BM, BN, AL, BL>(al, bl, smem, m0, n0, kbeg, kend, acc, wm, wn);
    store_tile<BM, BN>(acc, smem, ep, partial, M, N, m0, n0, wm, wn);
}

template <int BM, int BN>
constexpr int pc_stages() { return (BM * BN <= 64 * 64) ? 4 : (BM * BN >= 128 * 128 ? 3 : 2); }

template <int BM, int BN, class AL, class BL>
constexpr size_t igemm_pc_lds_bytes() {
    constexpr size_t ring = (size_t)pc_stages<BM, BN>() * (lds_floats<BM, AL::KC>() + lds_floats<BN, BL::KC>()) * sizeof(float);
    constexpr size_t cimage = (size_t)BM * (BN + 4) * sizeof(float);
    return ring > cimage ? ring : cimage;
}

template <int BM, int BN, class AL, class BL>
__global__ __launch_bounds__(512, (BM * BN >= 128 * 128) ? 1 : 2) void igemm_pc_kernel(AL al, BL bl, Epilogue ep, int M, int N, int K, int klen,
                                                       float* __restrict__ partial) {
    extern __shared__ __attribute__((aligned(16))) float smem[];
    constexpr int TM = BM / 64, TN = BN / 64, NS = pc_stages<BM, BN>();
    constexpr int A_FL = lds_floats<BM, AL::KC>(), B_FL = lds_floats<BN, BL::KC>(), STAGE = A_FL + B_FL;
    const int tid = threadIdx.x, wave = tid >> 6;
    const int tiles_n = (N + BN - 1) / BN;
    const int lid = xcd_remap(blockIdx.x, gridDim.x);
    const int m0 = (lid / tiles_n) * BM, n0 = (lid % tiles_n) * BN;
    const int kbeg = blockIdx.z * klen;
    const int kend = min(K, kbeg + klen);
    const int nkt = (kend - kbeg + BK - 1) / BK;

    if (wave >= 4) {
        const int ptid = tid - 256;
        typename AL::template State<BM> sa;
        typename BL::template State<BN> sb;
        al.template init<BM>(sa, m0, ptid);
        bl.template init<BN>(sb, n0, ptid);
        f4 ra[NS][BM / 32], rb[NS][BN / 32];
#pragma unroll
        for (int j = 0; j < NS; ++j) {
            const int k0 = kbeg + j * BK;
            al.template load<BM>(sa, ra[j], al.kclamp(k0, kend), kend, ptid);
            bl.template load<BN>(sb, rb[j], bl.kclamp(k0, kend), kend, ptid);
        }
        auto fill = [&](int t, float* st, f4 (&qa)[BM / 32], f4 (&qb)[BN / 32]) {
            if (t < nkt) {
                al.template store<BM>(sa, st, qa, ptid);
                bl.template store<BN>(sb, st + A_FL, qb, ptid);
            }
            const int k0 = kbeg + (t + NS) * BK;
            al.template load<BM>(sa, qa, al.kclamp(k0, kend), kend, ptid);
            bl.template load<BN>(sb, qb, bl.kclamp(k0, kend), kend, ptid);
        };
#pragma unroll
        for (int j = 0; j < NS - 1; ++j) fill(j, smem + j * STAGE, ra[j], rb[j]);
        __syncthreads();
        for (int t0 = 0; t0 < nkt; t0 += NS) {
#pragma unroll
            for (int u = 0; u < NS; ++u) {
                if (t0 + u < nkt) {
                    fill(t0 + u + NS - 1, smem + ((u + NS - 1) % NS) * STAGE, ra[(u + NS - 1) % NS], rb[(u + NS - 1) % NS]);
                    __syncthreads();
                }
            }
        }
        __syncthreads();
        return;
    }
    const int lane = tid & 63;
    const int wm = (wave >> 1) * (BM / 2), wn = (wave & 1) * (BN / 2);
    f32x16 acc[TM][TN];
#pragma unroll
    for (int tm = 0; tm < TM; ++tm)
#pragma unroll
        for (int tn = 0; tn < TN; ++tn)
#pragma unroll
            for (int r = 0; r < 16; ++r) acc[tm][tn][r] = 0.f;
    __syncthreads();
    for (int t0 = 0; t0 < nkt; t0 += NS) {
#pragma unroll
        for (int u = 0; u < NS; ++u) {
            if (t0 + u < nkt) {
                mma_tile<BM, BN, AL::KC, BL::KC>(smem + u * STAGE, smem + u * STAGE + A_FL, acc, wm, wn, lane);
                __syncthreads();
            }
        }
    }
    store_tile<BM, BN>(acc, smem, ep, partial, M, N, m0, n0, wm, wn);
}

__global__ void splitk_reduce_kernel(const float* __restrict__ partial, int splits, int M, int N, Epilogue ep);
inline int splitk_reduce_blocks(long total) { return (int)((total + 1023) / 1024); }

int conv2d_bf16x3(const dc_conv_desc* d, bool stem, const Epilogue& ep, int M, int N, int K, int bm, int bn, int split, void* workspace,
                  size_t workspace_bytes, hipStream_t s);

bool conv_pw_stream_supported(const dc_conv_desc* d, const Epilogue& ep);
int conv2d_pointwise_stream(const dc_conv_desc* d, const Epilogue& ep, int M, int N, hipStream_t s);
bool conv_winograd_supported(const dc_conv_desc* d);
bool conv_winograd_split_bf16(const dc_conv_desc* d);
int conv_winograd_tiles(const dc_conv_desc* d);
int conv2d_winograd(const dc_conv_desc* d, hipStream_t s);

template <int BM, int BN, class AL, class BL, bool PC = false>
int launch_igemm(const AL& al, const BL& bl, const Epilogue& ep, int M, int N, int K, int split_k, void* workspace,
                 size_t workspace_bytes, hipStream_t stream) {
    const int tiles = ((M + BM - 1) / BM) * ((N + BN - 1) / BN);
    const int ktiles = (K + BK - 1) / BK;
    if (split_k < 1) split_k = 1;
    if (split_k > ktiles) split_k = ktiles;
    const int klen = ((ktiles + split_k - 1) / split_k) * BK;
    split_k = (K + klen - 1) / klen;
    float* partial = nullptr;
    if (split_k > 1) {
        const size_t need = (size_t)split_k * M * N * sizeof(float);
        DC_REQUIRE(workspace != nullptr && workspace_bytes >= need, DC_EWORKSPACE,
                   "igemm split-K needs %zu workspace bytes, got %zu", need, workspace_bytes);
        partial = static_cast<float*>(workspace);
    }
    constexpr size_t lds = PC ? igemm_pc_lds_bytes<BM, BN, AL, BL>() : igemm_lds_bytes<BM, BN, AL, BL>();
    dim3 grid(tiles, 1, split_k);
    if constexpr (PC) {
        DC_ENSURE_DYN_LDS((&igemm_pc_kernel<BM, BN, AL, BL>), 160 * 1024);
        hipLaunchKernelGGL((igemm_pc_kernel<BM, BN, AL, BL>), grid, dim3(512), lds, stream, al, bl, ep, M, N, K, klen, partial);
    } else {
        DC_ENSURE_DYN_LDS((&igemm_kernel<BM, BN, AL, BL>), 160 * 1024);
        hipLaunchKernelGGL((igemm_kernel<BM, BN, AL, BL>), grid, dim3(256), lds, stream, al, bl, ep, M, N, K, klen, partial);
    }
    int rc = check_launch("igemm_kernel");
    if (rc) return rc;
    if (split_k > 1) {
        const long total = (long)M * N;
        hipLaunchKernelGGL(splitk_reduce_kernel, dim3(splitk_reduce_blocks(total)), dim3(256), 0, stream, partial, split_k, M, N, ep);
        rc = check_launch("splitk_reduce_kernel");
    }
    return rc;
}

struct TileChoice {
    int bm, bn, split;
    bool pc = false;
};
inline TileChoice choose_tile(int M, int N, int K, int user_split, bool allow_128 = true) {
    auto nb = [&](int bm, int bn) { return ((M + bm - 1) / bm) * ((N + bn - 1) / bn); };
    TileChoice t{64, 64, 1};
    const int ktiles = (K + BK - 1) / BK;
    bool priced = false;
    if (!allow_128) t = {64, 64, 1};
    else if (N >= 128 && nb(128, 128) >= 2 * kNumCU) t = {128, 128, 1};
    else if (nb(128, 64) >= 2 * kNumCU) t = {128, 64, 1};
    else if (user_split <= 0 && N >= 64 && ktiles >= 256) priced = true;
    if (priced) {
        const int cand[3][2] = {{128, 128}, {128, 64}, {64, 64}};
        const double eff[3] = {0.70, 0.58, 0.45};
        const double cu_flops = 157.3e12 / kNumCU;
        double best = 1e30;
        for (int c = 0; c < 3; ++c) {
            const int bm = cand[c][0], bn = cand[c][1];
            if (bn > 64 && N < 128) continue;
            const double blocks = nb(bm, bn);
            const double t_tile = 2.0 * bm * bn * BK / (cu_flops * eff[c]);
            for (int sp = 1; sp <= 32; sp = sp < 4 ? sp + 1 : sp + sp / 2) {
                if (sp > 1 && ktiles / sp < 4) break;
                const double w = blocks * sp / kNumCU;
                const double waves = w <= 1.0 ? 1.0 : ceil(w * 2.0) / 2.0;
                double cost = waves * ((ktiles + sp - 1) / sp) * t_tile + 4e-6;
                if (sp > 1) cost += (double)M * N * 4.0 * (sp + 1) / 4e12 + 3e-6;
                if (cost < best) { best = cost; t = {bm, bn, sp}; }
            }
        }
        return t;
    }
    if (user_split > 0) {
        t.split = user_split;
    } else {
        const int blocks = nb(t.bm, t.bn);
        if (blocks < kNumCU && ktiles >= 8) {
            int s = (2 * kNumCU + blocks - 1) / blocks;
// ... 11 lines not shown
```

### image-captioning_amd/csrc/roialign.hip

```cpp
#include "dcap_internal.h"
#include <math.h>
#include <algorithm>

#pragma clang fp contract(off)
namespace dcap {
__device__ __forceinline__ float mul_rn(float a, float b) { return a * b; }
__device__ __forceinline__ float add_rn(float a, float b) { return a + b; }
__device__ __forceinline__ float sub_rn(float a, float b) { return a - b; }
__device__ __forceinline__ float div_rn(float a, float b) { return a / b; }
}

namespace dcap {

__device__ __forceinline__ int roi_level(float y1, float x1, float y2, float x2, float image_area) {
    const float h = sub_rn(y2, y1), w = sub_rn(x2, x1);
    const float ratio = div_rn(__fsqrt_rn(mul_rn(h, w)), div_rn(224.0f, __fsqrt_rn(image_area)));
    const float lvl = div_rn(logf(ratio), logf(2.0f));
    if (!(lvl > -100.f)) return 2;
    const int r = (int)rintf(lvl);
    return min(5, max(2, 4 + r));
}

__device__ __forceinline__ float roi_sample(float lo, float hi, int p, int n, int pool) {
    if (pool > 1) {
// ... 72 lines not shown
    const int pix = (int)(wv - (long)img * per_img);
    const int y = pix / W, x = pix - y * W;
    const float4* boxes = reinterpret_cast<const float4*>(d.boxes) + (long)img * d.R;
    const int bins = d.pool * d.pool;
    float4 acc[4];
    const int C4 = d.C >> 2, nchunk = (C4 + 63) >> 6;
#pragma unroll
    for (int k = 0; k < 4; ++k) acc[k] = make_float4(0.f, 0.f, 0.f, 0.f);
    bool any = false;
    for (int b0 = 0; b0 < d.R; b0 += 64) {
        const int bi = b0 + lane;
        bool hit = false;
        if (bi < d.R) {
            const float4 bx = boxes[bi];
            if (roi_level(bx.x, bx.y, bx.z, bx.w, d.image_area) - 2 == li) {
                const float ya = roi_sample(bx.x, bx.z, 0, H, d.pool), yb = roi_sample(bx.x, bx.z, d.pool - 1, H, d.pool);
                const float xa = roi_sample(bx.y, bx.w, 0, W, d.pool), xb = roi_sample(bx.y, bx.w, d.pool - 1, W, d.pool);
                hit = fminf(ya, yb) < (float)y + 1.f && fmaxf(ya, yb) > (float)y - 1.f && fminf(xa, xb) < (float)x + 1.f && fmaxf(xa, xb) > (float)x - 1.f;
            }
        }
        unsigned long long m = __ballot(hit);
        while (m) {
            const int j = __ffsll((long long)m) - 1;
            m &= m - 1;
            const int box = b0 + j;
            const float4 bx = boxes[box];
            float wys[RA_MAX_POOL], wxs[RA_MAX_POOL];
#pragma unroll 1
            for (int p = 0; p < d.pool; ++p) {
                const float iy = roi_sample(bx.x, bx.z, p, H, d.pool), ix = roi_sample(bx.y, bx.w, p, W, d.pool);
                float wy = 0.f, wx = 0.f;
                if (iy >= 0.f && iy <= (float)(H - 1)) {
                    const float ly = iy - floorf(iy);
                    if ((int)floorf(iy) == y) wy += 1.f - ly;
                    if ((int)ceilf(iy) == y) wy += ly;
                } else {
                    wy = -1.f;
                }
                if (ix >= 0.f && ix <= (float)(W - 1)) {
                    const float lx = ix - floorf(ix);
                    if ((int)floorf(ix) == x) wx += 1.f - lx;
                    if ((int)ceilf(ix) == x) wx += lx;
                } else {
                    wx = -1.f;
                }
                wys[p] = wy;
                wxs[p] = wx;
            }
            const float* go = d.out + ((long)(img * d.R + box) * bins) * d.C;
#pragma unroll 1
            for (int py = 0; py < d.pool; ++py) {
                if (!(wys[py] > 0.f)) continue;
#pragma unroll 1
                for (int px = 0; px < d.pool; ++px) {
                    if (!(wxs[px] > 0.f)) continue;
                    const float wgt = wys[py] * wxs[px];
                    const float4* row = reinterpret_cast<const float4*>(go + (long)(py * d.pool + px) * d.C);
#pragma unroll
                    for (int k = 0; k < 4; ++k)
                        if (k < nchunk && lane + 64 * k < C4) {
                            const float4 g = row[lane + 64 * k];
                            acc[k].x += g.x * wgt; acc[k].y += g.y * wgt; acc[k].z += g.z * wgt; acc[k].w += g.w * wgt;
                        }
                    any = true;
                }
            }
        }
    }
    if (!any) return;
    float4* dst = reinterpret_cast<float4*>(const_cast<float*>(d.maps[li]) + ((long)img * per_img + pix) * d.C);
#pragma unroll
    for (int k = 0; k < 4; ++k)
        if (k < nchunk && lane + 64 * k < C4) {
            float4 v = dst[lane + 64 * k];
            v.x += acc[k].x; v.y += acc[k].y; v.z += acc[k].z; v.w += acc[k].w;
            dst[lane + 64 * k] = v;
        }
}

constexpr int RG_THREADS = 1024, RG_WAVES = RG_THREADS / 64, RG_LDS_MARKS = 8192;
struct RoiGroupsArgs {
    dc_roi_groups_desc d;
    int gy[4], gx[4], off[5];
};

__global__ __launch_bounds__(RG_THREADS) void roi_tile_groups_kernel(RoiGroupsArgs a) {
    const dc_roi_groups_desc& d = a.d;
    const int tid = threadIdx.x, lane = tid & 63, wave = tid >> 6;
    __shared__ int lds_marks[RG_LDS_MARKS];
    __shared__ int wsum[4][RG_WAVES];
    const int nmarks = a.off[4];
    int* marks = nmarks <= RG_LDS_MARKS ? lds_marks : d.marks;
    for (int i = tid; i < nmarks; i += RG_THREADS) marks[i] = 0;
    __syncthreads();
    const int bins = d.pool * d.pool, samples = d.B * d.R * bins;
    for (int s = tid; s < samples; s += RG_THREADS) {
        const int box = s / bins, bin = s - box * bins;
        const int py = bin / d.pool, px = bin - py * d.pool;
        const float4 bx = reinterpret_cast<const float4*>(d.boxes)[box];
        const int li = roi_level(bx.x, bx.y, bx.z, bx.w, d.image_area) - 2;
        const RoiBin sb = roi_bin(bx, py, px, d.Hs[li], d.Ws[li], d.pool);
        if (!sb.ok) continue;
        int* m = marks + a.off[li] + (box / d.R) * a.gy[li] * a.gx[li];
        const int gt = sb.top / kWinoGroupH * a.gx[li], gb = sb.bot / kWinoGroupH * a.gx[li];
        const int gl = sb.left / kWinoGroupW, gr = sb.right / kWinoGroupW;
        m[gt + gl] = 1;
        m[gt + gr] = 1;
        m[gb + gl] = 1;
        m[gb + gr] = 1;
    }
    __syncthreads();
    int below[4] = {0, 0, 0, 0};
    for (int c0 = 0; c0 < nmarks; c0 += RG_THREADS) {
        const int i = c0 + tid;
        const bool on = i < nmarks && marks[i] != 0;
        const int l = i >= a.off[3] ? 3 : (i >= a.off[2] ? 2 : (i >= a.off[1] ? 1 : 0));
        const int first = l == 3 ? a.off[3] : (l == 2 ? a.off[2] : (l == 1 ? a.off[1] : 0));
        const unsigned long long b = __ballot(on);
        const unsigned long long b1 = __ballot(on && i < a.off[1]), b2 = __ballot(on && i < a.off[2]), b3 = __ballot(on && i < a.off[3]);
        if (lane == 0) {
            wsum[0][wave] = __popcll(b);
            wsum[1][wave] = __popcll(b1);
            wsum[2][wave] = __popcll(b2);
            wsum[3][wave] = __popcll(b3);
        }
        __syncthreads();
        int before = 0, add[4] = {0, 0, 0, 0};
#pragma unroll
        for (int w = 0; w < RG_WAVES; ++w) {
            before += w < wave ? wsum[0][w] : 0;
#pragma unroll
            for (int k = 0; k < 4; ++k) add[k] += wsum[k][w];
        }
        const int rank = below[0] + before + __popcll(b & ((1ull << lane) - 1ull));
        const int lower = l == 3 ? below[3] + add[3] : (l == 2 ? below[2] + add[2] : (l == 1 ? below[1] + add[1] : 0));
        if (on) d.lists[l][rank - lower] = i - first;
#pragma unroll
        for (int k = 0; k < 4; ++k) below[k] += add[k];
        __syncthreads();
    }
    if (tid < 4) {
        const int lo = tid == 3 ? below[3] : (tid == 2 ? below[2] : (tid == 1 ? below[1] : 0));
        const int hi = tid == 3 ? below[0] : (tid == 2 ? below[3] : (tid == 1 ? below[2] : below[1]));
        d.counts[tid] = hi - lo;
    }
}

}

using namespace dcap;

extern "C" int dc_roi_tile_groups(const dc_roi_groups_desc* d, void* stream) {
    DC_REQUIRE(d && d->boxes && d->marks && d->counts, DC_EINVAL, "dc_roi_tile_groups: null pointer");
    DC_REQUIRE(d->B > 0 && d->R > 0 && d->pool > 0, DC_EINVAL, "dc_roi_tile_groups: bad B/R/pool");
    DC_REQUIRE(aligned16(d->boxes), DC_EALIGN, "dc_roi_tile_groups: boxes not 16-byte aligned");
    RoiGroupsArgs a;
    a.d = *d;
    long off = 0;
    for (int l = 0; l < 4; ++l) {
        DC_REQUIRE(d->lists[l] && d->Hs[l] > 0 && d->Ws[l] > 0, DC_EINVAL, "dc_roi_tile_groups: bad level %d", l);
        a.gy[l] = wino_groups_y(d->Hs[l]);
        a.gx[l] = wino_groups_x(d->Ws[l]);
        a.off[l] = (int)off;
        off += (long)d->B * a.gy[l] * a.gx[l];
    }
    a.off[4] = (int)off;
    DC_REQUIRE(off < (1l << 30) && (long)d->B * d->R * d->pool * d->pool < (1l << 30), DC_EINVAL, "dc_roi_tile_groups: too many groups / samples");
    hipLaunchKernelGGL(roi_tile_groups_kernel, dim3(1), dim3(RG_THREADS), 0, static_cast<hipStream_t>(stream), a);
    return check_launch("roi_tile_groups_kernel");
}

extern "C" int dc_roi_align_pyramid_bwd_f32(const dc_roialign_desc* d, void* stream) {
    DC_REQUIRE(d && d->boxes && d->out, DC_EINVAL, "dc_roi_align_pyramid_bwd: null pointer");
    DC_REQUIRE(d->B > 0 && d->R > 0 && d->pool > 0 && d->pool <= RA_MAX_POOL && d->C > 0 && (d->C & 3) == 0 && d->C <= 1024, DC_EINVAL,
               "dc_roi_align_pyramid_bwd: bad B/R/pool/C (pool <= 16, C a multiple of 4 and <= 1024)");
    for (int l = 0; l < 4; ++l) {
        DC_REQUIRE(d->maps[l] && d->Hs[l] > 0 && d->Ws[l] > 0, DC_EINVAL, "dc_roi_align_pyramid_bwd: bad map %d", l);
        DC_REQUIRE(aligned16(d->maps[l]), DC_EALIGN, "dc_roi_align_pyramid_bwd: gradient map %d not 16-byte aligned", l);
    }
    DC_REQUIRE(aligned16(d->boxes) && aligned16(d->out), DC_EALIGN, "dc_roi_align_pyramid_bwd: boxes / dout not 16-byte aligned");
    for (int l = 0; l < 4; ++l) {
        const long waves = (long)d->B * d->Hs[l] * d->Ws[l];
        for (long w0 = 0; w0 < waves; w0 += 4L * 0x40000000) {
            const long n = std::min(waves - w0, 4L * 0x40000000);
            hipLaunchKernelGGL(roi_align_bwd_gather_kernel, dim3((unsigned)((n + 3) / 4)), dim3(256), 0, static_cast<hipStream_t>(stream), *d, l, w0);
        }
        int rc = check_launch("roi_align_bwd_gather_kernel");
        if (rc) return rc;
    }
    return DC_OK;
}

extern "C" int dc_roi_align_pyramid_f32(const dc_roialign_desc* d, void* stream) {
    DC_REQUIRE(d && d->boxes && d->out, DC_EINVAL, "dc_roi_align_pyramid: null pointer");
    DC_REQUIRE(d->B > 0 && d->R > 0 && d->pool > 0 && d->C > 0 && (d->C & 3) == 0, DC_EINVAL, "dc_roi_align_pyramid: bad B/R/pool/C");
    for (int l = 0; l < 4; ++l) {
        DC_REQUIRE(d->maps[l] && d->Hs[l] > 0 && d->Ws[l] > 0, DC_EINVAL, "dc_roi_align_pyramid: bad feature map %d", l);
        DC_REQUIRE(aligned16(d->maps[l]), DC_EALIGN, "dc_roi_align_pyramid: feature map %d not 16-byte aligned", l);
    }
    DC_REQUIRE(aligned16(d->boxes) && aligned16(d->out), DC_EALIGN, "dc_roi_align_pyramid: boxes/out not 16-byte aligned");
    const long waves = (long)d->B * d->R * d->pool * d->pool;
    const int blocks = (int)((waves + 3) / 4);
    hipLaunchKernelGGL(roi_align_kernel, dim3(blocks), dim3(256), 0, static_cast<hipStream_t>(stream), *d);
    return check_launch("roi_align_kernel");
}
```

### image-captioning_amd/encoder.py

```python
import ctypes as C

import numpy as np
import torch

from . import _lib, ops, step_graph
from ._lib import ConvBf16Desc, ConvDesc, PwChainDesc, check
from .layers import ConvSpec, resnet_fpn_convs
from .packing import fold_bn, pack_conv_kernel, pack_stem_kernel


DEFAULT_CONV_MATH = "f32"


def conv_math_mode(math=None):
    import os
    name = math if math is not None else os.environ.get("DCAP_CONV_MATH", DEFAULT_CONV_MATH)
    try:
        return {"f32": _lib.MATH_F32, "bf16x3": _lib.MATH_BF16X3, "bf16x2": _lib.MATH_BF16X2, "bf16": _lib.MATH_BF16}[name]
    except KeyError:
        raise ValueError("conv math must be 'f32', 'bf16x3', 'bf16x2' or 'bf16', got %r" % (name,))


def conv_math_name(mode):
    return {_lib.MATH_F32: "f32", _lib.MATH_BF16X3: "bf16x3", _lib.MATH_BF16X2: "bf16x2", _lib.MATH_BF16: "bf16"}.get(mode, str(mode))
# ... 207 lines not shown
        self.flops += 2.0 * d.M * (d.K1 * d.N1 + d.N1 * d.N2)

    def _build(self):
        B, H, W = self.B, self.H, self.W
        self._ops, self._ws_bytes, self.flops, self._bufs = [], 0, 0.0, []
        self._twin, self._wb = {}, {}
        self.images = torch.empty((B, H, W, 3), dtype=torch.uint8, device=self.device)
        rgbx = torch.empty((B, H, W, 4), dtype=torch.float32, device=self.device)
        for name, bnp in self._external_bn.items():
            _, sc, sh = self._external[name]
            self._ops.append(("bnfold", bnp, sc, sh))
        self._ops.append(("mold", self.images, rgbx))
        c1 = self._buf(H // 2, W // 2, 64)
        self._conv("conv1", rgbx, c1)
        x = self._buf(H // 4, W // 4, 64)
        self._ops.append(("pool", c1, x))
        if self.fast_bf16:
            self._ops.append(("cast", x, self._bf(x)))
        self.saved[1] = dict(rgbx=rgbx, c1=c1, pooled=x)

        def stage(s, blocks, mid, cout, stride, x):
            h, w = x.shape[1] // stride, x.shape[2] // stride
            keep = s in self.train_stages
            if not keep:
                m1, m2, sc = self._buf(h, w, mid), self._buf(h, w, mid), self._buf(h, w, cout)
                pp = [self._buf(h, w, cout), self._buf(h, w, cout)]
            final = self._buf(h, w, cout)
            self.saved[s] = []
            pending = None
            for i, blk in enumerate(blocks):
                cn = "res%d%s_branch" % (s, blk)
                if keep:
                    m1, m2 = self._buf(h, w, mid), self._buf(h, w, mid)
                    sc = self._buf(h, w, cout) if i == 0 else None
                    out = final if i == len(blocks) - 1 else self._buf(h, w, cout)
                    self.saved[s].append(dict(name=cn, x=x, m1=m1, m2=m2, sc=sc, out=out, stride=stride if i == 0 else 1))
                else:
                    out = final if i == len(blocks) - 1 else pp[i & 1]
                if pending is not None:
                    self._chain(pending[0], pending[1], x, pending[2], cn + "2a", m1)
                    pending = None
                else:
                    self._conv(cn + "2a", x, m1, f32=keep, bf16=True)
                self._conv(cn + "2b", m1, m2, f32=keep, bf16=True)
                res = x
                if i == 0:
                    self._conv(cn + "1", x, sc, relu=False)
                    res = sc
                nxt = "res%d%s_branch2a" % (s, blocks[i + 1]) if i + 1 < len(blocks) else None
                if nxt is not None and not keep and self._chain_ok(cn + "2c", nxt, mid, cout, x.shape[0] * m2.shape[1] * m2.shape[2]):
                    pending = (cn + "2c", m2, res)
                else:
                    self._conv(cn + "2c", m2, out, residual=res, res_mode=1, bf16=True)
                x = out
            return x

        C2 = stage(2, "abc", 64, 256, 1, x)
        C3 = stage(3, "abcd", 128, 512, 2, C2)
        C4 = stage(4, ["a"] + [chr(98 + i) for i in range(self.stage4_blocks)], 256, 1024, 2, C3)
        C5 = stage(5, "abc", 512, 2048, 2, C4)
        self.C = (C2, C3, C4, C5)
        self._n_trunk = len(self._ops)
        self.pre = None
        t5, t4 = self._buf(H // 32, W // 32, 256), self._buf(H // 16, W // 16, 256)
        t3, t2 = self._buf(H // 8, W // 8, 256), self._buf(H // 4, W // 4, 256)
        self._conv("fpn_c5p5", C5, t5, relu=False, bf16=True)
        self._conv("fpn_c4p4", C4, t4, residual=t5, res_mode=2, relu=False, bf16=True)
        self._conv("fpn_c3p3", C3, t3, residual=t4, res_mode=2, relu=False, bf16=True)
        self._conv("fpn_c2p2", C2, t2, residual=t3, res_mode=2, relu=False, bf16=True)
        P2, P3 = self._buf(H // 4, W // 4, 256), self._buf(H // 8, W // 8, 256)
        P4, P5 = self._buf(H // 16, W // 16, 256), self._buf(H // 32, W // 32, 256)
        rp = self.rpn is not None
        self._n_lateral = len(self._ops)
        self._conv("fpn_p2", t2, P2, relu=False, bf16=rp)
        self._conv("fpn_p3", t3, P3, relu=False, bf16=rp)
        self._conv("fpn_p4", t4, P4, relu=False, bf16=rp)
        self._conv("fpn_p5", t5, P5, relu=False, bf16=rp)
        self.P = (P2, P3, P4, P5)
        self.pre = (t2, t3, t4, t5)
        pops = self._ops[self._n_lateral:]
        self.sparse_rois = (self.rpn is None and not self.fast_bf16 and not self.train_stages and not self._external_bn and len(pops) == 4 and
                            all(op[0] == "conv" and op[2] == "fpn_p%d" % (2 + i) and op[2] not in self._external and op[1].w_wino_b3
                                for i, op in enumerate(pops)))
        self._roi_groups = None
        self._roi_boxes = {}
        if self.rpn is not None:
            from .utils import generate_pyramid_anchors
            P6 = self._buf(H // 64, W // 64, 256)
            self._ops.append(("sub2", P5, P6))
            if self.fast_bf16:
                self._ops.append(("cast", P6, self._bf(P6)))
            self.P6 = P6
            self.rpn_heads, self.rpn_shared = [], []
            for p in (P2, P3, P4, P5, P6):
                sh = self._buf(p.shape[1], p.shape[2], 512)
                hd = self._buf(p.shape[1], p.shape[2], self.head_channels)
                self._conv("rpn_conv_shared", p, sh, bf16=True)
                self._conv("rpn_head", sh, hd, relu=False)
                self.rpn_heads.append(hd)
                self.rpn_shared.append(sh)
            shapes = [[-(-H // st), -(-W // st)] for st in self.rpn["strides"]]
            anchors = generate_pyramid_anchors(self.rpn["scales"], self.rpn["ratios"], shapes, self.rpn["strides"],
                                               self.rpn.get("anchor_stride", 1)).astype(np.float32)
            self.anchors = torch.tensor(anchors, device=self.device)
        self._bufs.append(rgbx)
        self._ws = torch.empty(max(self._ws_bytes, 16), dtype=torch.uint8, device=self.device)

    def _run_ops(self, lo=0, hi=None):
        lib = self.lib
        stream = C.c_void_p(torch.cuda.current_stream().cuda_stream)
        wsp, wsb = C.c_void_p(self._ws.data_ptr()), self._ws.numel()
        for op in self._ops[lo:hi]:
            kind = op[0]
            if kind == "conv":
                rc = lib.dc_conv2d_nhwc_f32(C.byref(op[1]), wsp, wsb, stream)
                if rc:
                    check(rc, "dc_conv2d_nhwc_f32(%s)" % op[2])
            elif kind == "chain":
                rc = lib.dc_pw_chain_f32(C.byref(op[1]), stream)
                if rc:
                    check(rc, "dc_pw_chain_f32(%s)" % op[2])
            elif kind == "bconv":
                rc = lib.dc_conv2d_bf16(C.byref(op[1]), wsp, wsb, stream)
                if rc:
                    check(rc, "dc_conv2d_bf16(%s)" % op[2])
            elif kind == "cast":
                ops.to_bf16(op[1], out=op[2])
            elif kind == "bnfold":
                b = op[1]
                ops.bn_fold(b["gamma"], b["beta"], b["bias"], b["mean"], b["var"], op[2], op[3])
            elif kind == "mold":
                ops.mold_image_rgbx(op[1], self.mean_pixel, out=op[2])
            elif kind == "sub2":
                ops.subsample2(op[1], out=op[2])
            else:
                ops.maxpool3x3s2_same(op[1], out=op[2])

    def conv_table(self):
        rows = []
        for op in self._ops:
            if op[0] == "chain":
                d, buf = op[1], C.create_string_buffer(64)
                check(self.lib.dc_pw_chain_kernel_name(C.byref(d), buf, 64), "dc_pw_chain_kernel_name")
                rows.append((op[2], 2.0 * d.M * (d.K1 * d.N1 + d.N1 * d.N2), 32, d.N1, 1, buf.value.decode()))
                continue
            if op[0] != "conv":
                continue
            d, bm, bn, sk = op[1], C.c_int(), C.c_int(), C.c_int()
            check(self.lib.dc_conv2d_tile_config(C.byref(d), C.byref(bm), C.byref(bn), C.byref(sk)), "dc_conv2d_tile_config")
            buf = C.create_string_buffer(128)
            check(self.lib.dc_conv2d_kernel_name(C.byref(d), buf, 128), "dc_conv2d_kernel_name")
            s = self._specs[op[2]]
            rows.append((op[2], 2.0 * d.N * d.Ho * d.Wo * d.Cout * s.k * s.k * s.cin, bm.value, bn.value, sk.value, buf.value.decode()))
        return rows

    def conv_algorithmic_bytes(self):
        out = {}
        for op in self._ops:
            if op[0] == "chain":
                d = op[1]
                out[op[2]] = 4.0 * (d.M * (d.K1 + (2 if d.residual else 1) * d.N1 + d.N2) + d.K1 * d.N1 + d.N1 * d.N2)
                continue
            if op[0] != "conv":
                continue
            d, s = op[1], self._specs[op[2]]
            wbytes = ((16 * (6 if self.wino_products == "b3" else 4)) if op[2] in self._wwino else s.k * s.k * 4) * d.Cin * s.cout
            b = 4.0 * d.N * d.H * d.W * d.Cin + 4.0 * d.N * d.Ho * d.Wo * d.Cout + wbytes
            if d.res_mode == 1:
                b += 4.0 * d.N * d.Ho * d.Wo * d.Cout
            elif d.res_mode == 2:
                b += 1.0 * d.N * d.Ho * d.Wo * d.Cout
            out[op[2]] = b
        return out

    def time_convs(self, reps=3, beside=None):
        lib = self.lib
        stream = C.c_void_p(torch.cuda.current_stream().cuda_stream)
        wsp, wsb = C.c_void_p(self._ws.data_ptr()), self._ws.numel()
        convs = [op for op in self._ops if op[0] in ("conv", "chain")]
        acc = [0.0] * len(convs)
        for _ in range(reps):
            self._run_ops()
            torch.cuda.synchronize()
            if beside is not None:
                beside()
            evs = []
            for op in convs:
                e0, e1 = torch.cuda.Event(enable_timing=True), torch.cuda.Event(enable_timing=True)
                e0.record()
                rc = lib.dc_pw_chain_f32(C.byref(op[1]), stream) if op[0] == "chain" else lib.dc_conv2d_nhwc_f32(C.byref(op[1]), wsp, wsb, stream)
                e1.record()
                if rc:
                    check(rc, "dc_conv2d_nhwc_f32(%s)" % op[2])
                evs.append((e0, e1))
            torch.cuda.synchronize()
            for i, (e0, e1) in enumerate(evs):
                acc[i] += e0.elapsed_time(e1)
        return [(op[2], a / reps) for op, a in zip(convs, acc)]

    def time_bconvs(self, reps=3):
        lib = self.lib
        stream = C.c_void_p(torch.cuda.current_stream().cuda_stream)
        wsp, wsb = C.c_void_p(self._ws.data_ptr()), self._ws.numel()
        convs = [op for op in self._ops if op[0] == "bconv"]
        acc = [0.0] * len(convs)
        for _ in range(reps):
            self._run_ops()
            torch.cuda.synchronize()
            evs = []
            for op in convs:
                e0, e1 = torch.cuda.Event(enable_timing=True), torch.cuda.Event(enable_timing=True)
                e0.record()
                rc = lib.dc_conv2d_bf16(C.byref(op[1]), wsp, wsb, stream)
                e1.record()
                if rc:
                    check(rc, "dc_conv2d_bf16(%s)" % op[2])
                evs.append((e0, e1))
            torch.cuda.synchronize()
            for i, (e0, e1) in enumerate(evs):
                acc[i] += e0.elapsed_time(e1)
        rows = []
        for op, a in zip(convs, acc):
            d, sk = op[1], C.c_int(0)
            tile = int(lib.dc_conv2d_bf16_tile(C.byref(d), C.byref(sk)))
            rows.append((op[2], 2.0 * d.N * d.Ho * d.Wo * d.Cout * d.kh * d.kw * d.Cin, a / reps, tile, int(sk.value)))
        return rows

    def forward(self, images_u8=None):
        if images_u8 is not None:
            self.images.copy_(images_u8, non_blocking=bool(images_u8.is_cuda or images_u8.is_pinned()))
        self._run_part("all", self._run_ops)
        return self.P

    def _run_part(self, part, body):
        if not self.use_graph:
            body()
            return
        cs = self._steps.get(part)
        if cs is None:
            cs = self._steps[part] = step_graph.CapturedStep()
        cs.run(body, warm_calls=1, propagate=True)

    def _run_rois(self, boxes):
        g = ops.roi_tile_groups(boxes, self._roi_groups, float(self.H * self.W), 7)
        stream = C.c_void_p(torch.cuda.current_stream().cuda_stream)
        for l, op in enumerate(self._ops[self._n_lateral:]):
            rc = self.lib.dc_conv2d_winograd_groups_f32(C.byref(op[1]), C.c_void_p(g.lists[l].data_ptr()), g.count_ptr(l), stream)
            if rc:
                check(rc, "dc_conv2d_winograd_groups_f32(%s)" % op[2])

    def forward_rois(self, images_u8, boxes_norm, out=None, before_align=None):
        if not self.sparse_rois:
            self.forward(images_u8)
            if before_align is not None:
                before_align()
            return self.roi_features(boxes_norm=boxes_norm.to(self.device, torch.float32).contiguous(), out=out)
        if images_u8 is not None:
            self.images.copy_(images_u8, non_blocking=bool(images_u8.is_cuda or images_u8.is_pinned()))
        B, R = int(boxes_norm.shape[0]), int(boxes_norm.shape[1])
        if B != self.B or tuple(boxes_norm.shape[2:]) != (4,):
            raise ValueError("forward_rois: boxes must be [%d,R,4], got %s" % (self.B, tuple(boxes_norm.shape)))
        if self._roi_groups is None:
            self._roi_groups = ops.RoiTileGroups(self.B, [(p.shape[1], p.shape[2]) for p in self.P], self.device)
        boxes = self._roi_boxes.get(R)
        if boxes is None:
            boxes = self._roi_boxes[R] = torch.zeros((self.B, R, 4), dtype=torch.float32, device=self.device)
        boxes.copy_(boxes_norm, non_blocking=bool(boxes_norm.is_cuda or boxes_norm.is_pinned()))
        self._run_part("lat", lambda: self._run_ops(0, self._n_lateral))
        self._run_part("rois%d" % R, lambda: self._run_rois(boxes))
        if before_align is not None:
            before_align()
        return ops.roi_align_pyramid(list(self.P), boxes, float(self.H * self.W), 7, out=out)

    def forward_trunk(self, images_u8=None):
        if self._external_bn:
            raise RuntimeError("forward_trunk: this plan folds trainable BatchNorm layers inside the backbone pass; use forward()")
        if images_u8 is not None:
            self.images.copy_(images_u8, non_blocking=bool(images_u8.is_cuda or images_u8.is_pinned()))
        self._run_part("trunk", lambda: self._run_ops(0, self._n_trunk))
        return self.C

    def forward_top(self):
        self._run_part("top", lambda: self._run_ops(self._n_trunk, None))
        return self.P

    def proposals(self, debug=False):
        if self.rpn is None:
            raise RuntimeError("this plan was built without the RPN")
        r = self.rpn
        return ops.rpn_proposals(self.rpn_heads, self.anchors, (self.H, self.W), r["proposal_count"], r["nms_threshold"],
                                 r.get("bbox_std", (0.1, 0.1, 0.2, 0.2)), anchors_per_loc=len(r["ratios"]), debug=debug,
                                 head_stride=self.head_channels)

    def normalize_boxes(self, rois_px):
        hw = np.array([self.H, self.W, self.H, self.W], np.float32)
        if isinstance(rois_px, torch.Tensor):
            rois_px = rois_px.detach().cpu().numpy()
        return torch.tensor(np.asarray(rois_px, np.float32) / hw, device=self.device).contiguous()

    def roi_features(self, rois_px=None, out=None, boxes_norm=None):
        boxes = boxes_norm if boxes_norm is not None else self.normalize_boxes(rois_px)
        return ops.roi_align_pyramid(list(self.P), boxes, float(self.H * self.W), 7, out=out)


class Vgg16Plan(EncoderPlan):
    feat_channels = 512

    def __init__(self, weights, batch, height, width, device, mean_pixel=(123.7, 116.8, 103.9), use_graph=True, math=None, winograd=None,
                 wino_products=None):
        from .layers import vgg16_convs
        import os
        if height % 16 or width % 16:
            raise ValueError("Image size must be dividable by 16 (got %dx%d)" % (height, width))
        self.lib = _lib.load()
        self.math = conv_math_mode(math)
        self.winograd = (os.environ.get("DCAP_WINOGRAD", "1") != "0") if winograd is None else bool(winograd)
        self.wino_products = wino_products or os.environ.get("DCAP_WINO_PRODUCTS", "b3")
        self._wwino = {}
        self.layer_math = False
        self.B, self.H, self.W = batch, height, width
        self.device = torch.device(device)
        self.mean_pixel = [float(v) for v in mean_pixel]
        self.use_graph = use_graph
        self._steps = {}
        self._specs = {s.name: s for s in vgg16_convs()}
        self.rpn = None
        self._external = {}
        self._w = {}
        self._upload(weights)
        self._build()

    def _upload(self, W):
        dev = self.device
        for s in self._specs.values():
            k = np.asarray(W[s.name + "/kernel"], np.float32)
            if tuple(k.shape) != (s.k, s.k, s.cin, s.cout):
                raise ValueError("%s/kernel has shape %s, expected %s" % (s.name, k.shape, (s.k, s.k, s.cin, s.cout)))
            if s.cin == 3:
                k = np.concatenate([k, np.zeros((s.k, s.k, 29, s.cout), np.float32)], axis=2)
            self._w[s.name] = (torch.tensor(pack_conv_kernel(k), device=dev), None,
                               torch.tensor(np.asarray(W[s.name + "/bias"], np.float32), device=dev))

    def _build(self):
        B, H, W = self.B, self.H, self.W
        self._ops, self._ws_bytes, self.flops, self._bufs = [], 0, 0.0, []
        self.images = torch.empty((B, H, W, 3), dtype=torch.uint8, device=self.device)
        x32 = torch.empty((B, H, W, 32), dtype=torch.float32, device=self.device)
        self._bufs += [x32]
        self._ops.append(("mold32", self.images, x32))
        x, h, w = x32, H, W
        for b, (n, cout) in enumerate(((2, 64), (2, 128), (3, 256), (3, 512), (3, 512)), 1):
# ... 34 lines not shown
```

### image-captioning_amd/ops.py

```python
import contextlib
import ctypes as C
import os

import numpy as np

import torch

from . import _lib
from ._lib import (PwChainDesc, ConvBf16Desc, AmsgradDesc, DetectionTargetsDesc, BnReluDesc, ConvDesc, ConvWgradBf16Desc, GemmBf16Desc, VocabCeDesc, ProposalDesc, RpnLossDesc, GemmDesc, LstmBwdDesc, LstmFwdDesc, RoiAlignDesc, RoiGroupsDesc,
                   SoftmaxCeDesc, VocabTop1Desc, VocabTopkDesc, VocabTop1Bf16Desc, VocabTopkBf16Desc, BeamSelectDesc, LstmStepDesc, check)


def _stream():
    return C.c_void_p(torch.cuda.current_stream().cuda_stream)


def _ptr(t):
    return None if t is None else C.c_void_p(t.data_ptr())


def _chk(t, dtype=torch.float32, name="tensor"):
    if not t.is_cuda:
        raise _lib.DcapError("%s must live on the GPU (no CPU path exists)" % name)
    if t.dtype != dtype:
# ... 414 lines not shown
    d.out = _chk(dout, name="dout").data_ptr()
    check(lib.dc_roi_align_pyramid_bwd_f32(C.byref(d), _stream()), "dc_roi_align_pyramid_bwd_f32")
    return dmaps


def maxpool3x3s2_same(x, out=None):
    lib = _lib.load()
    _chk(x, name="x")
    N, H, W, Cc = x.shape
    if out is None:
        out = torch.empty((N, (H + 1) // 2, (W + 1) // 2, Cc), dtype=torch.float32, device=x.device)
    check(lib.dc_maxpool3x3s2_same_f32(_ptr(x), _ptr(out), N, H, W, Cc, _stream()), "dc_maxpool3x3s2_same_f32")
    return out


def maxpool2x2s2(x, out=None):
    lib = _lib.load()
    _chk(x, name="x")
    N, H, W, Cc = x.shape
    if out is None:
        out = torch.empty((N, H // 2, W // 2, Cc), dtype=torch.float32, device=x.device)
    check(lib.dc_maxpool2x2s2_f32(_ptr(x), _ptr(out), N, H, W, Cc, _stream()), "dc_maxpool2x2s2_f32")
    return out


def mold_image_rgbx(img_u8, mean_pixel, out=None):
    lib = _lib.load()
    _chk(img_u8, torch.uint8, "images")
    N, H, W, c = img_u8.shape
    if c != 3 or not img_u8.is_contiguous():
        raise _lib.DcapError("mold_image: images must be contiguous [N,H,W,3] uint8")
    if out is None:
        out = torch.empty((N, H, W, 4), dtype=torch.float32, device=img_u8.device)
    check(lib.dc_mold_image_rgbx_f32(_ptr(img_u8), _ptr(out), N, H, W, float(mean_pixel[0]), float(mean_pixel[1]),
                                     float(mean_pixel[2]), _stream()), "dc_mold_image_rgbx_f32")
    return out


def mold_image_padded(img_u8, mean_pixel, out):
    lib = _lib.load()
    _chk(img_u8, torch.uint8, "images"), _chk(out, name="out")
    N, H, W, c = img_u8.shape
    if c != 3 or not img_u8.is_contiguous() or not out.is_contiguous() or tuple(out.shape[:3]) != (N, H, W):
        raise _lib.DcapError("mold_image_padded: images contiguous [N,H,W,3] uint8, out contiguous [N,H,W,C]")
    check(lib.dc_mold_image_padded_f32(_ptr(img_u8), _ptr(out), N, H, W, out.shape[3], float(mean_pixel[0]), float(mean_pixel[1]),
                                       float(mean_pixel[2]), _stream()), "dc_mold_image_padded_f32")
    return out


def roi_align_pyramid(maps, boxes, image_area, pool=7, out=None, levels_out=None):
    lib = _lib.load()
    B, R, _ = boxes.shape
    Cc = maps[0].shape[-1]
    _chk(boxes, name="boxes")
    if not boxes.is_contiguous():
        raise _lib.DcapError("roi_align: boxes must be contiguous")
    if out is None:
        out = torch.empty((B, R, pool, pool, Cc), dtype=torch.float32, device=boxes.device)
    d = RoiAlignDesc()
    d.B, d.R, d.C, d.pool = B, R, Cc, pool
    for i, m in enumerate(maps):
        _chk(m, name="map")
        if not m.is_contiguous() or m.shape[0] != B or m.shape[-1] != Cc:
            raise _lib.DcapError("roi_align: feature maps must be contiguous [B,H,W,C]")
        d.maps[i] = m.data_ptr()
        d.Hs[i], d.Ws[i] = m.shape[1], m.shape[2]
    d.boxes, d.image_area, d.out = boxes.data_ptr(), float(image_area), out.data_ptr()
    d.levels_out = None if levels_out is None else _chk(levels_out, torch.int32, "levels").data_ptr()
    check(lib.dc_roi_align_pyramid_f32(C.byref(d), _stream()), "dc_roi_align_pyramid_f32")
    return out


class RoiTileGroups(object):

    def __init__(self, B, hw, device):
        lib = _lib.load()
        self.B, self.hw = int(B), [(int(h), int(w)) for h, w in hw]
        if len(self.hw) != 4:
            raise _lib.DcapError("RoiTileGroups: four pyramid levels expected")
        self.per_image = [lib.dc_conv2d_winograd_group_count(h, w) for h, w in self.hw]
        self.lists = [torch.zeros(self.B * n, dtype=torch.int32, device=device) for n in self.per_image]
        self.counts = torch.zeros(4, dtype=torch.int32, device=device)
        self.marks = torch.zeros(self.B * sum(self.per_image), dtype=torch.int32, device=device)

    def count_ptr(self, level):
        return C.c_void_p(self.counts.data_ptr() + 4 * level)


def roi_tile_groups(boxes, groups, image_area, pool=7):
    lib = _lib.load()
    _chk(boxes, name="boxes")
    B, R, _ = boxes.shape
    if not boxes.is_contiguous() or B != groups.B:
        raise _lib.DcapError("roi_tile_groups: boxes must be contiguous [B,R,4] with the B the group buffers were made for")
    d = RoiGroupsDesc()
    d.B, d.R, d.pool = B, R, pool
    for i, (h, w) in enumerate(groups.hw):
        d.Hs[i], d.Ws[i] = h, w
        d.lists[i] = groups.lists[i].data_ptr()
    d.boxes, d.image_area = boxes.data_ptr(), float(image_area)
    d.marks, d.counts = groups.marks.data_ptr(), groups.counts.data_ptr()
    check(lib.dc_roi_tile_groups(C.byref(d), _stream()), "dc_roi_tile_groups")
    return groups


def conv2d_winograd_groups(x, w_packed, w_wino_b3, group_list, count, out, scale=None, shift=None, relu=False):
    lib = _lib.load()
    _chk(x, name="x"), _chk(w_packed, name="w"), _chk(out, name="out")
    _chk(group_list, torch.int32, "group_list"), _chk(count, torch.int32, "count")
    N, H, W, Cin = x.shape
    Cout = w_packed.shape[0]
    if not x.is_contiguous() or not out.is_contiguous() or tuple(out.shape) != (N, H, W, Cout):
        raise _lib.DcapError("conv2d_winograd_groups: x and out must be contiguous [N,H,W,C]")
    if not w_wino_b3.is_contiguous() or w_wino_b3.numel() != 48 * Cin * Cout:
        raise _lib.DcapError("conv2d_winograd_groups: w_wino_b3 must be the contiguous winograd_pack_b3() of this layer's kernel")
    if group_list.numel() < N * lib.dc_conv2d_winograd_group_count(H, W) or count.numel() < 1:
        raise _lib.DcapError("conv2d_winograd_groups: the list must have room for every tile group of the layer")
    d = ConvDesc()
    d.N, d.H, d.W, d.Cin = N, H, W, Cin
    d.Cout, d.kh, d.kw, d.stride, d.pad_t, d.pad_l, d.Ho, d.Wo = Cout, 3, 3, 1, 1, 1, H, W
    d.x, d.w, d.y = x.data_ptr(), w_packed.data_ptr(), out.data_ptr()
    d.scale = None if scale is None else scale.data_ptr()
    d.shift = None if shift is None else shift.data_ptr()
    d.relu = int(relu)
    d.w_wino_b3 = _chk(w_wino_b3, torch.int16, "w_wino_b3").data_ptr()
    check(lib.dc_conv2d_winograd_groups_f32(C.byref(d), _ptr(group_list), _ptr(count), _stream()), "dc_conv2d_winograd_groups_f32")
    return out


def subsample2(x, out=None):
    lib = _lib.load()
    _chk(x, name="x")
    N, H, W, Cc = x.shape
    if out is None:
        out = torch.empty((N, (H + 1) // 2, (W + 1) // 2, Cc), dtype=torch.float32, device=x.device)
    check(lib.dc_subsample2_f32(_ptr(x), _ptr(out), N, H, W, Cc, _stream()), "dc_subsample2_f32")
    return out


def rpn_proposals(heads, anchors, image_hw, proposal_count, nms_threshold, std_dev=(0.1, 0.1, 0.2, 0.2), pre_nms_limit=6000,
                  anchors_per_loc=3, out=None, debug=False, head_stride=0):
    lib = _lib.load()
    B = heads[0].shape[0]
    d = ProposalDesc()
    d.B, d.levels, d.anchors_per_loc = B, len(heads), anchors_per_loc
    for i, h in enumerate(heads):
        if not _chk(h, name="head").is_contiguous() or h.shape[-1] != (head_stride or anchors_per_loc * 6):
            raise _lib.DcapError("rpn_proposals: heads must be contiguous [B,H,W,A*6] (or [B,H,W,head_stride])")
        d.heads[i] = h.data_ptr()
        d.Hs[i], d.Ws[i] = h.shape[1], h.shape[2]
    d.head_stride = int(head_stride)
    d.anchors, d.A_total = _chk(anchors, name="anchors").data_ptr(), anchors.shape[0]
    for i in range(4):
        d.std_dev[i] = float(std_dev[i])
    d.image_h, d.image_w = float(image_hw[0]), float(image_hw[1])
    d.pre_nms_limit, d.proposal_count, d.nms_threshold = int(pre_nms_limit), int(proposal_count), float(nms_threshold)
    dev = heads[0].device
    if out is None:
        out = torch.empty((B, proposal_count, 4), dtype=torch.float32, device=dev)
    d.proposals = out.data_ptr()
    extra = None
    if debug:
        k = min(pre_nms_limit, anchors.shape[0])
        extra = (torch.empty((B, anchors.shape[0]), dtype=torch.float32, device=dev),
                 torch.empty((B, k), dtype=torch.int32, device=dev),
                 torch.empty((B, proposal_count), dtype=torch.int32, device=dev))
        d.scores_out, d.order_out, d.keep_out = (t.data_ptr() for t in extra)
    ws, wsb = WORKSPACE.get(lib.dc_proposals_workspace_bytes(C.byref(d)), dev)
    check(lib.dc_proposals_f32(C.byref(d), _ptr(ws), wsb, _stream()), "dc_proposals_f32")
    return (out, extra) if debug else out


def _rec_masks(rec_masks, B, U):
    if rec_masks is None:
        return None
    if tuple(_chk(rec_masks, name="rec_masks").shape) != (4, B, U) or not rec_masks.is_contiguous():
        raise _lib.DcapError("rec_masks must be a contiguous float32 [4,B,U] tensor")
    return rec_masks.data_ptr()


def lstm_seq_fwd(z, U_rec, mask, B, T, h_seq=None, c_seq=None, rec_masks=None):
    lib = _lib.load()
    U = U_rec.shape[0]
    _chk(z, name="z"), _chk(U_rec, name="U_rec")
    if not z.is_contiguous() or not U_rec.is_contiguous() or tuple(z.shape) != (T * B, 4 * U):
        raise _lib.DcapError("lstm_seq_fwd: z must be contiguous [T*B,4U], U_rec contiguous [U,4U]")
    if h_seq is None:
        h_seq = torch.empty((T * B, U), dtype=torch.float32, device=z.device)
    if c_seq is None:
        c_seq = torch.empty((T * B, U), dtype=torch.float32, device=z.device)
    d = LstmFwdDesc()
    d.B, d.T, d.U = B, T, U
    d.z, d.U_rec = z.data_ptr(), U_rec.data_ptr()
    d.mask = None if mask is None else _chk(mask, torch.uint8, "mask").data_ptr()
    d.h_seq, d.c_seq = h_seq.data_ptr(), c_seq.data_ptr()
    d.rec_masks = _rec_masks(rec_masks, B, U)
    ws, wsb = WORKSPACE.get(lib.dc_lstm_seq_workspace_bytes(B, T, U), z.device)
    check(lib.dc_lstm_seq_fwd_f32(C.byref(d), _ptr(ws), wsb, _stream()), "dc_lstm_seq_fwd_f32")
    return h_seq, c_seq


def lstm_pack_urec(U_rec, out=None):
    _chk(U_rec, name="U_rec")
    lib = _lib.load()
    U = U_rec.shape[0]
    if not U_rec.is_contiguous() or tuple(U_rec.shape) != (U, 4 * U):
        raise _lib.DcapError("lstm_pack_urec: U_rec must be contiguous [U,4U]")
    if out is None:
        out = torch.empty((U, 4 * U), dtype=torch.float32, device=U_rec.device)
    if not _chk(out, name="out").is_contiguous() or out.numel() != 4 * U * U:
# ... 575 lines not shown
```

### include/dcap.h

```cpp
#ifndef DCAP_H
#define DCAP_H

#include <stddef.h>
#include <stdint.h>

#ifdef __cplusplus
extern "C" {
#endif

#define DC_OK            0
#define DC_EINVAL       -1
#define DC_EALIGN       -2
#define DC_EWORKSPACE   -3
#define DC_ELAUNCH      -4

#define DC_ABI_VERSION 600
int         dc_version(void);
const char* dc_last_error(void);

typedef struct {
    int M, N, K;
    const float*   A;  int lda;  int a_trans;
    const int32_t* a_gather;
    const float*   B;  int ldb;  int b_trans;
// ... 84 lines not shown
    int relu;
    int split_k;
    int accumulate;
    int math;
    const float* w_wino;
    const uint16_t* w_wino_b3;
} dc_conv_desc;

int dc_split_bf16x3_f32(const float* x, uint16_t* out, size_t n, void* stream);
size_t dc_conv2d_workspace_bytes(const dc_conv_desc* d);
int    dc_conv2d_nhwc_f32(const dc_conv_desc* d, void* workspace, size_t workspace_bytes, void* stream);

int    dc_conv2d_tile_config(const dc_conv_desc* d, int* bm, int* bn, int* split_k);
int    dc_conv2d_kernel_name(const dc_conv_desc* d, char* buf, size_t buf_bytes);
int    dc_conv2d_is_pointwise(const dc_conv_desc* d);
size_t dc_conv2d_winograd_weight_bytes(int Cin, int Cout);
int    dc_conv2d_winograd_pack_f32(const float* w, float* u, int Cin, int Cout, void* stream);
size_t dc_conv2d_winograd_b3_weight_bytes(int Cin, int Cout);
int    dc_conv2d_winograd_pack_b3(const float* w, uint16_t* u, int Cin, int Cout, void* stream);
typedef struct {
    int M, K1, N1, N2;
    const float* x;
    const float* w1;
    const float* scale1;
    const float* shift1;
    const float* residual;
    int relu1;
    float* y;
    const float* w2;
    const float* scale2;
    const float* shift2;
    int relu2;
    float* z;
    const uint16_t* w1_b3;
    const uint16_t* w2_b3;
} dc_pw_chain_desc;
int dc_pw_chain_supported(int K1, int N1, int N2);
int dc_pw_chain_pack_f32(const float* w, float* out, int N, int K, void* stream);
int dc_pw_chain_pack_b3(const float* w, uint16_t* out, int N, int K, void* stream);
int dc_pw_chain_f32(const dc_pw_chain_desc* d, void* stream);
int dc_pw_chain_kernel_name(const dc_pw_chain_desc* d, char* buf, size_t buf_bytes);

int    dc_set_persistent_cus(int n);
int    dc_get_persistent_cus(void);

size_t dc_conv2d_wgrad_workspace_bytes(const dc_conv_desc* d);
int    dc_conv2d_wgrad_f32(const dc_conv_desc* d, void* workspace, size_t workspace_bytes, void* stream);

int dc_maxpool3x3s2_same_f32(const float* x, float* y, int N, int H, int W, int C, void* stream);

int dc_maxpool2x2s2_f32(const float* x, float* y, int N, int H, int W, int C, void* stream);

int dc_mold_image_rgbx_f32(const uint8_t* img, float* out, int N, int H, int W,
                           float mean_r, float mean_g, float mean_b, void* stream);
int dc_mold_image_padded_f32(const uint8_t* img, float* out, int N, int H, int W, int channels,
                             float mean_r, float mean_g, float mean_b, void* stream);

typedef struct {
    int B, R, C, pool;
    const float* maps[4];
    int Hs[4], Ws[4];
    const float* boxes;
    float image_area;
    float* out;
    int32_t* levels_out;
} dc_roialign_desc;

int dc_roi_align_pyramid_f32(const dc_roialign_desc* d, void* stream);

typedef struct {
    int B, R, pool;
    int Hs[4], Ws[4];
    const float* boxes;
    float image_area;
    int32_t* marks;
    int32_t* lists[4];
    int32_t* counts;
} dc_roi_groups_desc;

int dc_roi_tile_groups(const dc_roi_groups_desc* d, void* stream);
int dc_conv2d_winograd_group_count(int H, int W);
int dc_conv2d_winograd_groups_f32(const dc_conv_desc* d, const int32_t* groups, const int32_t* count, void* stream);

int dc_subsample2_f32(const float* x, float* y, int N, int H, int W, int C, void* stream);

typedef struct {
    int B, levels, anchors_per_loc;
    const float* heads[5];
    int Hs[5], Ws[5];
    int head_stride;
    const float* anchors;
    int A_total;
    float std_dev[4];
    float image_h, image_w;
    int pre_nms_limit, proposal_count;
    float nms_threshold;
    float* proposals;
    float* scores_out;
    int32_t* order_out;
    int32_t* keep_out;
} dc_proposal_desc;

size_t dc_proposals_workspace_bytes(const dc_proposal_desc* d);
int    dc_proposals_f32(const dc_proposal_desc* d, void* workspace, size_t workspace_bytes, void* stream);

int dc_roi_align_pyramid_bwd_f32(const dc_roialign_desc* d, void* stream);

int dc_downsample2x_sum_f32(const float* fine, float* out, int N, int Ho, int Wo, int C, int accumulate, void* stream);
int dc_downsample2x_sum_dual_f32(const float* fine, float* out, uint16_t* out_bf16, int N, int Ho, int Wo, int C, int accumulate, void* stream);

typedef struct {
    int B, T, U;
    float* z;
    const float* U_rec;
    const uint8_t* mask;
    float* h_seq;
    float* c_seq;
    const float* rec_masks;
} dc_lstm_fwd_desc;

size_t dc_lstm_seq_workspace_bytes(int B, int T, int U);
int    dc_lstm_seq_fwd_f32(const dc_lstm_fwd_desc* d, void* workspace, size_t workspace_bytes, void* stream);

typedef struct {
    int B, T, U;
    const float* z;
    const float* U_rec;
    const uint8_t* mask;
    const float* h_seq;
    const float* c_seq;
    const float* dh_seq;
    const float* dh_last;
    float* dz;
    float* dU_rec;
    int accumulate_dU;
    const float* rec_masks;
} dc_lstm_bwd_desc;

int dc_lstm_seq_bwd_f32(const dc_lstm_bwd_desc* d, void* workspace, size_t workspace_bytes, void* stream);

typedef struct {
    int B, U;
    float* z;
    const float* U_rec;
    const float* U_packed;
    const float* h_prev;
    const float* c_prev;
    const uint8_t* mask;
    float* h;
    float* c;
} dc_lstm_step_desc;

int    dc_lstm_pack_urec_f32(const float* U_rec, int U, float* U_packed, void* stream);
size_t dc_lstm_step_workspace_bytes(int B, int U);
int    dc_lstm_step_f32(const dc_lstm_step_desc* d, void* workspace, size_t workspace_bytes, void* stream);

typedef struct {
    int M, V, ld;
    const float* logits;
    const int32_t* targets;
    float* probs;
    float* loss_rows;
    float* dlogits;
    float grad_scale;
    const float* row_weights;
    int keras_sparse;
// ... 215 lines not shown
```

Baseline: 12150 captions/s.

## Batch FPN RoI-level Winograd convs into one launch and sparsify last lateral conv

Replaces four per-level list-driven Winograd launches for the FPN P2..P5 output convs with a single kernel that walks the concatenated per-level tile-group lists, which cuts launch overhead and tail underfill across small levels. Also computes only the RoI-touched tiles of the last lateral 1x1 conv through a new tile-list-driven bf16x3 GEMM path, fed by a lateral tile-group builder. This adds device-side level selection and a persistent tile loop in the GEMM kernel, which may cost registers and occupancy.

Result: faster. 12500 captions/s, median of 6 (+2.9%).

```diff
diff --git a/image-captioning_amd/_lib.py b/image-captioning_amd/_lib.py
--- a/image-captioning_amd/_lib.py
+++ b/image-captioning_amd/_lib.py
@@ -234,6 +234,9 @@
     "dc_roi_tile_groups": (C.c_int, [C.POINTER(RoiGroupsDesc), C.c_void_p]),
     "dc_conv2d_winograd_group_count": (C.c_int, [C.c_int, C.c_int]),
     "dc_conv2d_winograd_groups_f32": (C.c_int, [C.POINTER(ConvDesc), C.c_void_p, C.c_void_p, C.c_void_p]),
+    "dc_conv2d_winograd_levels_f32": (C.c_int, [C.POINTER(ConvDesc), C.c_int, C.POINTER(C.c_void_p), C.c_void_p, C.c_void_p]),
+    "dc_roi_tile_groups_lateral": (C.c_int, [C.POINTER(RoiGroupsDesc), C.c_void_p, C.c_void_p, C.c_void_p]),
+    "dc_conv2d_nhwc_tiles_f32": (C.c_int, [C.POINTER(ConvDesc), C.c_void_p, C.c_void_p, C.c_void_p]),
     "dc_subsample2_f32": (C.c_int, [C.c_void_p, C.c_void_p, C.c_int, C.c_int, C.c_int, C.c_int, C.c_void_p]),
     "dc_proposals_workspace_bytes": (C.c_size_t, [C.POINTER(ProposalDesc)]),
     "dc_proposals_f32": (C.c_int, [C.POINTER(ProposalDesc), C.c_void_p, C.c_size_t, C.c_void_p]),
diff --git a/image-captioning_amd/csrc/conv.hip b/image-captioning_amd/csrc/conv.hip
--- a/image-captioning_amd/csrc/conv.hip
+++ b/image-captioning_amd/csrc/conv.hip
@@ -284,6 +284,24 @@
     return conv_dispatch(al, bl, ep, M, N, K, t, workspace, workspace_bytes, s);
 }
 
+extern "C" int dc_conv2d_nhwc_tiles_f32(const dc_conv_desc* d, const int32_t* tiles, const int32_t* count, void* stream) {
+    bool stem;
+    int rc = conv_validate(d, stem);
+    if (rc) return rc;
+    DC_REQUIRE(tiles && count, DC_EINVAL, "dc_conv2d_nhwc_tiles: null list / count");
+    int M, N, K;
+    conv_dims(d, stem, M, N, K);
+    const TileChoice t = conv_tile_bs(M, N, K, d->split_k);
+    const Epilogue ep = conv_epilogue(d);
+    DC_REQUIRE(!stem && conv_is_pointwise(d) && d->math == DC_MATH_BF16X3 && d->split_k <= 1 && t.bm == 128 && t.bn == 128 && t.split == 1 &&
+                   (d->res_mode == 0 || d->res_mode == 2) && !d->accumulate && ep.vec4,
+               DC_EINVAL,
+               "dc_conv2d_nhwc_tiles: the layer must be a 1x1 / stride 1 convolution in DC_MATH_BF16X3 that the dense launch runs on 128 x 128 "
+               "tiles without split-K (set split_k = 1 where the dense rule would split), res_mode 0 or 2, no accumulate, Cout %% 4 == 0 and "
+               "16-byte aligned operands: there is no other list-driven path");
+    return conv2d_bf16x3_tiles(d, ep, tiles, count, static_cast<hipStream_t>(stream));
+}
+
 static int wgrad_validate(const dc_conv_desc* d) {
     DC_REQUIRE(d && d->x && d->w && d->y, DC_EINVAL, "dc_conv2d_wgrad: x, dy (y) and dw (w) must be non-null");
     DC_REQUIRE(d->N > 0 && d->H > 0 && d->W > 0 && d->Ho > 0 && d->Wo > 0 && d->kh >= 1 && d->kw >= 1 && d->kh <= 8 && d->kw <= 8 &&
diff --git a/image-captioning_amd/csrc/conv_bs.hip b/image-captioning_amd/csrc/conv_bs.hip
--- a/image-captioning_amd/csrc/conv_bs.hip
+++ b/image-captioning_amd/csrc/conv_bs.hip
@@ -50,6 +50,13 @@
     return dispatch_bs(al, bl, ep, M, N, K, bm, bn, split, workspace, workspace_bytes, s, pieces);
 }
 
+int conv2d_bf16x3_tiles(const dc_conv_desc* d, const Epilogue& ep, const int* tiles, const int* count, hipStream_t s) {
+    const int gy = wino_groups_y(d->H), gx = wino_groups_x(d->W);
+    ConvWeightKC bl{d->w, d->Cin, d->Cout, 1, d->Cin};
+    TileListKC al{d->x, d->H, d->W, d->Cin, gy, gx, d->N * gy * gx, (unsigned)((size_t)d->N * d->H * d->W * d->Cin * sizeof(float)), tiles, count};
+    return launch_igemm_bs_list<128, 128, TileListKC, ConvWeightKC>(al, bl, ep, d->N * gy * gx, d->Cout, d->Cin, s);
+}
+
 }
 
 extern "C" int dc_split_bf16x3_f32(const float* x, uint16_t* out, size_t n, void* stream) {
diff --git a/image-captioning_amd/csrc/conv_wino.hip b/image-captioning_amd/csrc/conv_wino.hip
--- a/image-captioning_amd/csrc/conv_wino.hip
+++ b/image-captioning_amd/csrc/conv_wino.hip
@@ -19,6 +19,22 @@
     const int* gcount;
 };
 
+struct LevelArgs {
+    const float* x;
+    const f4* u;
+    float* y;
+    const float* scale;
+    const float* shift;
+    int H, W, gy, gx, groups;
+    unsigned x_bytes, u_bytes;
+    const int* glist;
+    const int* gcount;
+};
+struct LevelsArgs {
+    LevelArgs lv[4];
+    int nlevels, N, Cin, Cout, relu;
+};
+
 __global__ void wino_pack_kernel(const float* __restrict__ w, float* __restrict__ u, int Cin, int Cout) {
     const long total = (long)Cin * Cout;
     const int NTG = Cout / 32, KC = Cin / 16;
@@ -108,6 +124,9 @@
 
 typedef unsigned u32x4 __attribute__((ext_vector_type(4)));
 
+template <class T>
+__device__ __forceinline__ T sel4(int l, T v0, T v1, T v2, T v3) { return l == 0 ? v0 : (l == 1 ? v1 : (l == 2 ? v2 : v3)); }
+
 __device__ __forceinline__ void split8(const f4& va, const f4& vb, u32x4& p0, u32x4& p1, u32x4& p2) {
     unsigned a0, a1, a2, b0, b1, b2, c0, c1, c2, d0, d1, d2;
     split_pair(va[0], va[1], a0, a1, a2);
@@ -122,10 +141,25 @@
     return __builtin_amdgcn_mfma_f32_32x32x16_bf16(__builtin_bit_cast(bf16x8, a), __builtin_bit_cast(bf16x8, b), c, 0, 0, 0);
 }
 
-template <int HALVES, bool B3, int NCH = 1, bool LIST = false>
-__device__ __forceinline__ void wino_body(const Args& a) {
+template <int HALVES, bool B3, int NCH = 1, int LIST = 0, class KA = Args>
+__device__ __forceinline__ void wino_body(const KA& ka) {
     static_assert(NCH == 1 || (NCH == 2 && HALVES == 1 && B3), "64-channel items: the split-bf16 32-tile kernel only");
     static_assert(!LIST || (HALVES == 1 && B3), "list-driven item walk: the split-bf16 32-tile kernel only");
+    Args cur;
+    const Args& a = [&]() -> const Args& {
+        if constexpr (LIST == 2) return cur;
+        else return ka;
+    }();
+    int cum[4] = {0, 0, 0, 0};
+    if constexpr (LIST == 2) {
+        cur.N = ka.N; cur.Cin = ka.Cin; cur.Cout = ka.Cout; cur.relu = ka.relu;
+#define DC_CNT(l) (l < ka.nlevels ? min(max(ka.lv[l].gcount[0], 0), ka.lv[l].groups) : 0)
+        cum[1] = DC_CNT(0);
+        cum[2] = cum[1] + DC_CNT(1);
+        cum[3] = cum[2] + DC_CNT(2);
+        cur.groups = cum[3] + DC_CNT(3);
+#undef DC_CNT
+    }
     using namespace wp;
     typedef Cfg<HALVES> C;
     constexpr int NT64 = C::NT, SLOTS = C::SLOTS, BUF = C::BUF;
@@ -133,12 +167,27 @@
     const int tid = threadIdx.x, lane = tid & 63;
     const int wave = __builtin_amdgcn_readfirstlane(tid >> 6);
     const int wa = wave & 3, th = wave >> 2;
-    const int gpi = a.gy * a.gx;
+    int gpi = LIST == 2 ? 0 : a.gy * a.gx;
     const int NTG = a.Cout >> 5, KC = a.Cin >> 4, KP = a.Cin >> 5;
     int groups = a.groups;
-    if constexpr (LIST) groups = min(max(*a.gcount, 0), a.groups);
+    if constexpr (LIST == 1) groups = min(max(*a.gcount, 0), a.groups);
     const int total = groups * (NTG / NCH);
-    const __amdgpu_buffer_rsrc_t rsrc = __builtin_amdgcn_make_buffer_rsrc(const_cast<float*>(a.x), 0, (int)a.x_bytes, 0x00020000);
+    __amdgpu_buffer_rsrc_t rsrc, rsrc_u;
+    if constexpr (LIST != 2) rsrc = __builtin_amdgcn_make_buffer_rsrc(const_cast<float*>(a.x), 0, (int)a.x_bytes, 0x00020000);
+    int lgroups = 0;
+    auto set_level = [&](int l) {
+#define DC_LV(f) sel4(l, ka.lv[0].f, ka.lv[1].f, ka.lv[2].f, ka.lv[3].f)
+        if constexpr (LIST == 2) {
+            cur.x = DC_LV(x); cur.u = DC_LV(u); cur.y = DC_LV(y); cur.scale = DC_LV(scale); cur.shift = DC_LV(shift);
+            cur.H = DC_LV(H); cur.W = DC_LV(W); cur.gy = DC_LV(gy); cur.gx = DC_LV(gx);
+            cur.x_bytes = DC_LV(x_bytes); cur.u_bytes = DC_LV(u_bytes); cur.glist = DC_LV(glist);
+            lgroups = DC_LV(groups);
+            gpi = cur.gy * cur.gx;
+            rsrc = __builtin_amdgcn_make_buffer_rsrc(const_cast<float*>(cur.x), 0, (int)cur.x_bytes, 0x00020000);
+            rsrc_u = __builtin_amdgcn_make_buffer_rsrc(const_cast<f4*>(cur.u), 0, (int)cur.u_bytes, 0x00020000);
+        }
+#undef DC_LV
+    };
 
     int nb, img, gyi, gxi;
     unsigned doff[NDMA];
@@ -148,7 +197,13 @@
         const int bid = xcd_remap(item, total);
         nb = bid / groups;
         int g = bid - nb * groups;
-        if constexpr (LIST) g = min(max(a.glist[g], 0), a.groups - 1);
+        if constexpr (LIST == 1) g = min(max(a.glist[g], 0), a.groups - 1);
+        if constexpr (LIST == 2) {
+            const int l = g >= cum[3] ? 3 : (g >= cum[2] ? 2 : (g >= cum[1] ? 1 : 0));
+            g -= l == 3 ? cum[3] : (l == 2 ? cum[2] : (l == 1 ? cum[1] : 0));
+            set_level(l);
+            g = min(max(a.glist[g], 0), lgroups - 1);
+        }
         img = g / gpi;
         const int gr = g - img * gpi;
         gyi = gr / a.gx;
@@ -182,7 +237,7 @@
         }
     };
     auto load_u = [&](f4 (&dst)[4][2], int kc) { load_u_part(dst, kc, 0, 4); };
-    const __amdgpu_buffer_rsrc_t rsrc_u = __builtin_amdgcn_make_buffer_rsrc(const_cast<f4*>(a.u), 0, (int)a.u_bytes, 0x00020000);
+    if constexpr (LIST != 2) rsrc_u = __builtin_amdgcn_make_buffer_rsrc(const_cast<f4*>(a.u), 0, (int)a.u_bytes, 0x00020000);
     const unsigned ustep3 = (unsigned)NTG * KC * 3 * 1024u;
     auto load_u3 = [&](u32x4 (&dst)[3], int kc, int b, int hc) {
         const unsigned so = __builtin_amdgcn_readfirstlane(ubyte3 + (unsigned)b * ustep3 + (unsigned)(hc * KC + kc) * 3072u);
@@ -427,6 +482,8 @@
         }
 
         const int onb = nb, oimg = img, ogy = gyi, ogx = gxi;
+        const int oH = a.H, oW = a.W;
+        float* const oy = a.y;
         const int next = item + (int)gridDim.x;
         const int oq = tid & 7, ocout = onb * (32 * NCH) + 4 * oq;
         f4 sc[NCH], sh[NCH];
@@ -474,8 +531,8 @@
                     for (int pr = 0; pr < 2; ++pr) {
                         f4 val = o[pr] * sc[hc] + sh[hc];
                         if (a.relu) val = f4{fmaxf(val[0], 0.f), fmaxf(val[1], 0.f), fmaxf(val[2], 0.f), fmaxf(val[3], 0.f)};
-                        if (2 * ty + pr < a.H && 2 * tx + qx < a.W)
-                            *reinterpret_cast<f4*>(a.y + (((long)oimg * a.H + 2 * ty + pr) * a.W + 2 * tx + qx) * a.Cout + cout) = val;
+                        if (2 * ty + pr < oH && 2 * tx + qx < oW)
+                            *reinterpret_cast<f4*>(oy + (((long)oimg * oH + 2 * ty + pr) * oW + 2 * tx + qx) * a.Cout + cout) = val;
                     }
                 }
             }
@@ -493,9 +550,10 @@
 template __global__ void wino32b_kernel<1>(Args);
 template __global__ void wino32b_kernel<2>(Args);
 template <int NCH>
-__global__ __launch_bounds__(256, 2) void wino32b_list_kernel(Args a) { wino_body<1, true, NCH, true>(a); }
+__global__ __launch_bounds__(256, 2) void wino32b_list_kernel(Args a) { wino_body<1, true, NCH, 1>(a); }
 template __global__ void wino32b_list_kernel<1>(Args);
 template __global__ void wino32b_list_kernel<2>(Args);
+__global__ __launch_bounds__(256, 2) void wino32b_levels_kernel(LevelsArgs m) { wino_body<1, true, 1, 2>(m); }
 
 }
 
@@ -621,9 +679,43 @@
     return check_launch("dc_conv2d_winograd_groups_f32");
 }
 
+int conv2d_winograd_levels(const dc_conv_desc* d, int nlevels, const int* const* lists, const int* counts, hipStream_t s) {
+    wino::LevelsArgs m;
+    m.nlevels = nlevels;
+    m.N = d[0].N; m.Cin = d[0].Cin; m.Cout = d[0].Cout; m.relu = d[0].relu;
+    long items = 0;
+    for (int l = 0; l < 4; ++l) {
+        const int k = l < nlevels ? l : 0;
+        wino::Args a;
+        const int rc = wino_args(&d[k], true, false, a);
+        if (rc) return rc;
+        m.lv[l] = wino::LevelArgs{a.x, a.u, a.y, a.scale, a.shift, a.H, a.W, a.gy, a.gx, a.groups, a.x_bytes, a.u_bytes, lists[k], counts + k};
+        if (l < nlevels) items += (long)a.groups * (d[0].Cout / 32);
+    }
+    DC_REQUIRE(items < (1l << 31), DC_EINVAL, "dc_conv2d_winograd_levels: grid too large");
+    const long full = 2L * kNumCU;
+    const unsigned grid = items >= full ? (unsigned)full : (unsigned)std::max<long>(8, items / 8 * 8);
+    DC_ENSURE_DYN_LDS(wino::wino32b_levels_kernel, wino::wp::Cfg<1>::LDS_BYTES);
+    hipLaunchKernelGGL(wino::wino32b_levels_kernel, dim3(grid), dim3(wino::wp::Cfg<1>::NT), wino::wp::Cfg<1>::LDS_BYTES, s, m);
+    return check_launch("dc_conv2d_winograd_levels_f32");
+}
+
 }
 
 using namespace dcap;
+
+extern "C" int dc_conv2d_winograd_levels_f32(const dc_conv_desc* d, int nlevels, const int32_t* const* lists, const int32_t* counts, void* stream) {
+    DC_REQUIRE(d && lists && counts && nlevels >= 1 && nlevels <= 4, DC_EINVAL, "dc_conv2d_winograd_levels: null pointer or nlevels outside 1..4");
+    for (int l = 0; l < nlevels; ++l) {
+        DC_REQUIRE(d[l].x && d[l].y && lists[l] && d[l].N > 0 && d[l].H > 0 && d[l].W > 0, DC_EINVAL, "dc_conv2d_winograd_levels: bad level %d", l);
+        DC_REQUIRE(wino_b3(&d[l]), DC_EINVAL,
+                   "dc_conv2d_winograd_levels: level %d must be a layer the split-bf16 Winograd kernel takes (3x3, stride 1, pad 1, Cin and Cout "
+                   "multiples of 32, no residual, fp32 math, w_wino_b3 given, 16-byte aligned operands, input below 2 GiB)", l);
+        DC_REQUIRE(d[l].N == d[0].N && d[l].Cin == d[0].Cin && d[l].Cout == d[0].Cout && (d[l].relu != 0) == (d[0].relu != 0), DC_EINVAL,
+                   "dc_conv2d_winograd_levels: level %d differs from level 0 in N, Cin, Cout or relu (equal-cost items only)", l);
+    }
+    return conv2d_winograd_levels(d, nlevels, lists, counts, static_cast<hipStream_t>(stream));
+}
 
 extern "C" int dc_conv2d_winograd_groups_f32(const dc_conv_desc* d, const int32_t* groups, const int32_t* count, void* stream) {
     DC_REQUIRE(d && d->x && d->y && groups && count, DC_EINVAL, "dc_conv2d_winograd_groups: null pointer");
diff --git a/image-captioning_amd/csrc/igemm_bf16s.h b/image-captioning_amd/csrc/igemm_bf16s.h
--- a/image-captioning_amd/csrc/igemm_bf16s.h
+++ b/image-captioning_amd/csrc/igemm_bf16s.h
@@ -1,5 +1,6 @@
 #pragma once
 #include "igemm_core.h"
+#include <algorithm>
 
 namespace dcap {
 
@@ -63,82 +64,118 @@
 
     const int tid = threadIdx.x, lane = tid & 63, wave = tid >> 6;
     const int tiles_n = (N + BN - 1) / BN;
-    const int lid = xcd_remap(blockIdx.x, gridDim.x);
-    const int m0 = (lid / tiles_n) * BM, n0 = (lid % tiles_n) * BN;
+    constexpr bool LIST = is_tile_list<AL>::value;
+    int lid = xcd_remap(blockIdx.x, gridDim.x);
+    int items = 0;
+    if constexpr (LIST) {
+        items = al.entries() * tiles_n;
+        if (lid >= items) return;
+    }
     const int kbeg = blockIdx.z * klen;
     const int kend = min(K, kbeg + klen);
     const int wm = (wave >> 1) * (BM / 2), wn = (wave & 1) * (BN / 2);
     const int li = lane & 31, lh = lane >> 5;
-
-    typename AL::template State<BM> sa;
-    typename BL::template State<BN> sb;
-    al.template init<BM>(sa, m0, tid);
-    bl.template init<BN>(sb, n0, tid);
-
-    f32x16 acc[TM][TN];
-#pragma unroll
-    for (int tm = 0; tm < TM; ++tm)
-#pragma unroll
-        for (int tn = 0; tn < TN; ++tn)
-#pragma unroll
-            for (int r = 0; r < 16; ++r) acc[tm][tn][r] = 0.f;
-
-    f4 ra[2][BM / 32], rb[2][BN / 32];
-    const int nkt = (kend - kbeg + BK - 1) / BK;
-#pragma unroll
-    for (int j = 0; j < 2; ++j) {
-        const int k0 = kbeg + j * BK;
-        al.template load<BM>(sa, ra[j], al.kclamp(k0, kend), kend, tid);
-        bl.template load<BN>(sb, rb[j], bl.kclamp(k0, kend), kend, tid);
-    }
-
-    const __bf16* afrag = As + (wm + li) * LDB + 8 * lh;
-    const __bf16* bfrag = Bs + (wn + li) * LDB + 8 * lh;
-
-    auto phase = [&](int kt, f4 (&qa)[BM / 32], f4 (&qb)[BN / 32]) {
-        store_split_kc<BM, BM / 32, NP>(As, qa, tid);
-        store_split_kc<BN, BN / 32, NP>(Bs, qb, tid);
-        __syncthreads();
-        {
-            const int k0 = kbeg + (kt + 2) * BK;
-            al.template load<BM>(sa, qa, al.kclamp(k0, kend), kend, tid);
-            bl.template load<BN>(sb, qb, bl.kclamp(k0, kend), kend, tid);
-        }
-#pragma unroll
-        for (int s = 0; s < BK / 16; ++s) {
-            bf16x8 a[TM][NP], b[TN][NP];
-#pragma unroll
-            for (int p = 0; p < NP; ++p) {
-#pragma unroll
-                for (int tm = 0; tm < TM; ++tm) a[tm][p] = *reinterpret_cast<const bf16x8*>(afrag + (p * BM + tm * 32) * LDB + 16 * s);
-#pragma unroll
-                for (int tn = 0; tn < TN; ++tn) b[tn][p] = *reinterpret_cast<const bf16x8*>(bfrag + (p * BN + tn * 32) * LDB + 16 * s);
+    for (;;) {
+        const int m0 = (lid / tiles_n) * BM, n0 = (lid % tiles_n) * BN;
+
+        typename AL::template State<BM> sa;
+        typename BL::template State<BN> sb;
+        al.template init<BM>(sa, m0, tid);
+        bl.template init<BN>(sb, n0, tid);
+
+        f32x16 acc[TM][TN];
+#pragma unroll
+        for (int tm = 0; tm < TM; ++tm)
+#pragma unroll
+            for (int tn = 0; tn < TN; ++tn)
+#pragma unroll
+                for (int r = 0; r < 16; ++r) acc[tm][tn][r] = 0.f;
+
+        f4 ra[2][BM / 32], rb[2][BN / 32];
+        const int nkt = (kend - kbeg + BK - 1) / BK;
+#pragma unroll
+        for (int j = 0; j < 2; ++j) {
+            const int k0 = kbeg + j * BK;
+            al.template load<BM>(sa, ra[j], al.kclamp(k0, kend), kend, tid);
+            bl.template load<BN>(sb, rb[j], bl.kclamp(k0, kend), kend, tid);
+        }
+
+        const __bf16* afrag = As + (wm + li) * LDB + 8 * lh;
+        const __bf16* bfrag = Bs + (wn + li) * LDB + 8 * lh;
+
+        auto phase = [&](int kt, f4 (&qa)[BM / 32], f4 (&qb)[BN / 32]) {
+            store_split_kc<BM, BM / 32, NP>(As, qa, tid);
+            store_split_kc<BN, BN / 32, NP>(Bs, qb, tid);
+            __syncthreads();
+            {
+                const int k0 = kbeg + (kt + 2) * BK;
+                al.template load<BM>(sa, qa, al.kclamp(k0, kend), kend, tid);
+                bl.template load<BN>(sb, qb, bl.kclamp(k0, kend), kend, tid);
             }
 #pragma unroll
-            for (int tm = 0; tm < TM; ++tm)
-#pragma unroll
-                for (int tn = 0; tn < TN; ++tn) {
-                    f32x16 c = acc[tm][tn];
-                    if constexpr (NP == 3) {
-                        c = __builtin_amdgcn_mfma_f32_32x32x16_bf16(a[tm][2], b[tn][0], c, 0, 0, 0);
-                        c = __builtin_amdgcn_mfma_f32_32x32x16_bf16(a[tm][1], b[tn][1], c, 0, 0, 0);
-                        c = __builtin_amdgcn_mfma_f32_32x32x16_bf16(a[tm][0], b[tn][2], c, 0, 0, 0);
+            for (int s = 0; s < BK / 16; ++s) {
+                bf16x8 a[TM][NP], b[TN][NP];
+#pragma unroll
+                for (int p = 0; p < NP; ++p) {
+#pragma unroll
+                    for (int tm = 0; tm < TM; ++tm) a[tm][p] = *reinterpret_cast<const bf16x8*>(afrag + (p * BM + tm * 32) * LDB + 16 * s);
+#pragma unroll
+                    for (int tn = 0; tn < TN; ++tn) b[tn][p] = *reinterpret_cast<const bf16x8*>(bfrag + (p * BN + tn * 32) * LDB + 16 * s);
+                }
+#pragma unroll
+                for (int tm = 0; tm < TM; ++tm)
+#pragma unroll
+                    for (int tn = 0; tn < TN; ++tn) {
+                        f32x16 c = acc[tm][tn];
+                        if constexpr (NP == 3) {
+                            c = __builtin_amdgcn_mfma_f32_32x32x16_bf16(a[tm][2], b[tn][0], c, 0, 0, 0);
+                            c = __builtin_amdgcn_mfma_f32_32x32x16_bf16(a[tm][1], b[tn][1], c, 0, 0, 0);
+                            c = __builtin_amdgcn_mfma_f32_32x32x16_bf16(a[tm][0], b[tn][2], c, 0, 0, 0);
+                        }
+                        if constexpr (NP >= 2) {
+                            c = __builtin_amdgcn_mfma_f32_32x32x16_bf16(a[tm][1], b[tn][0], c, 0, 0, 0);
+                            c = __builtin_amdgcn_mfma_f32_32x32x16_bf16(a[tm][0], b[tn][1], c, 0, 0, 0);
+                        }
+                        c = __builtin_amdgcn_mfma_f32_32x32x16_bf16(a[tm][0], b[tn][0], c, 0, 0, 0);
+                        acc[tm][tn] = c;
                     }
-                    if constexpr (NP >= 2) {
-                        c = __builtin_amdgcn_mfma_f32_32x32x16_bf16(a[tm][1], b[tn][0], c, 0, 0, 0);
-                        c = __builtin_amdgcn_mfma_f32_32x32x16_bf16(a[tm][0], b[tn][1], c, 0, 0, 0);
-                    }
-                    c = __builtin_amdgcn_mfma_f32_32x32x16_bf16(a[tm][0], b[tn][0], c, 0, 0, 0);
-                    acc[tm][tn] = c;
-                }
-        }
-        __syncthreads();
-    };
-    for (int kt = 0; kt < nkt; kt += 2) {
-        phase(kt, ra[0], rb[0]);
-        if (kt + 1 < nkt) phase(kt + 1, ra[1], rb[1]);
-    }
-    store_tile<BM, BN>(acc, smem, ep, partial, M, N, m0, n0, wm, wn);
+            }
+            __syncthreads();
+        };
+        for (int kt = 0; kt < nkt; kt += 2) {
+            phase(kt, ra[0], rb[0]);
+            if (kt + 1 < nkt) phase(kt + 1, ra[1], rb[1]);
+        }
+        if constexpr (LIST) {
+            int img, y0, x0;
+            al.origin(lid / tiles_n, img, y0, x0);
+            store_tile_list<BM, BN>(acc, smem, ep, N, img, y0, x0, al.H, al.W, n0, wm, wn);
+            lid += gridDim.x;
+            if (lid >= items) break;
+            __syncthreads();
+        } else {
+            store_tile<BM, BN>(acc, smem, ep, partial, M, N, m0, n0, wm, wn);
+            break;
+        }
+    }
+}
+
+template <int BM, int BN, class AL, class BL, int NP = 3>
+int launch_igemm_bs_list(const AL& al, const BL& bl, const Epilogue& ep, int entries, int N, int K, hipStream_t stream) {
+    const long items = (long)entries * ((N + BN - 1) / BN);
+    DC_REQUIRE(items > 0 && items * BM < (1l << 31), DC_EINVAL, "igemm (tile list): bad item count %ld", items);
+    const int klen = ((K + BK - 1) / BK) * BK;
+    constexpr size_t lds = igemm_bs_lds_bytes<BM, BN, NP>();
+    DC_ENSURE_DYN_LDS((&igemm_bs_kernel<BM, BN, AL, BL, NP>), 160 * 1024);
+#ifdef DCAP_EXP_LIST_GRID_ALL
+    const long full = items;
+#else
+    const long full = 2L * kNumCU;
+#endif
+    const unsigned grid = items >= full ? (unsigned)((full + 7) / 8 * 8) : (unsigned)std::max<long>(8, items / 8 * 8);
+    hipLaunchKernelGGL((igemm_bs_kernel<BM, BN, AL, BL, NP>), dim3(grid), dim3(256), lds, stream, al, bl, ep, (int)(entries * BM), N, K, klen,
+                       static_cast<float*>(nullptr));
+    return check_launch("igemm_bs_kernel (tile list)");
 }
 
 template <int BM, int BN, class AL, class BL, int NP = 3>
diff --git a/image-captioning_amd/csrc/igemm_core.h b/image-captioning_amd/csrc/igemm_core.h
--- a/image-captioning_amd/csrc/igemm_core.h
+++ b/image-captioning_amd/csrc/igemm_core.h
@@ -298,6 +298,52 @@
 
 using Im2colKC = Im2colKCT<false>;
 using Im2colKCcm = Im2colKCT<true>;
+
+struct TileListKC {
+    static constexpr bool KC = true;
+    static constexpr int ROWS = kWinoGroupH * kWinoGroupW;
+    __device__ __forceinline__ int kclamp(int k0, int kend) const { return min(k0, kend - BK); }
+    const float* x;
+    int H, W, Cin, gy, gx, groups;
+    unsigned x_bytes;
+    const int* list;
+    const int* count;
+    __device__ __forceinline__ int entries() const { return min(max(count[0], 0), groups); }
+    __device__ __forceinline__ void origin(int e, int& img, int& y0, int& x0) const {
+        const int g = min(max(list[e], 0), groups - 1);
+        img = g / (gy * gx);
+        const int gr = g - img * (gy * gx), gyi = gr / gx;
+        y0 = gyi * kWinoGroupH;
+        x0 = (gr - gyi * gx) * kWinoGroupW;
+    }
+    template <int BT>
+    struct State {
+        __amdgpu_buffer_rsrc_t rsrc;
+        unsigned boff[BT / 32];
+    };
+    template <int BT>
+    __device__ __forceinline__ void init(State<BT>& s, int row0, int tid) const {
+        static_assert(BT == ROWS, "one M tile is one 8 x 16 tile group");
+        s.rsrc = __builtin_amdgcn_make_buffer_rsrc(const_cast<float*>(x), 0, (int)x_bytes, 0x00020000);
+        int img, y0, x0;
+        origin(row0 / BT, img, y0, x0);
+        const int rr = tid >> 3;
+#pragma unroll
+        for (int i = 0; i < BT / 32; ++i) {
+            const int r = rr + 32 * i, y = y0 + r / kWinoGroupW, xx = x0 + r % kWinoGroupW;
+            s.boff[i] = (y < H && xx < W) ? (unsigned)(((((long)img * H + y) * W + xx) * Cin + 4 * (tid & 7)) * 4) : kOobOffset;
+        }
+    }
+    template <int BT>
+    __device__ __forceinline__ void load(State<BT>& s, f4 (&r)[BT / 32], int k0, int, int) const {
+#pragma unroll
+        for (int i = 0; i < BT / 32; ++i) r[i] = buf_f4s(s.rsrc, s.boff[i], (unsigned)k0 * 4u);
+    }
+};
+template <class AL>
+struct is_tile_list { static constexpr bool value = false; };
+template <>
+struct is_tile_list<TileListKC> { static constexpr bool value = true; };
 
 struct Im2colMC {
     static constexpr bool KC = false;
@@ -621,6 +667,58 @@
     }
 }
 
+template <int BM, int BN, int TM = BM / 64, int TN = BN / 64>
+__device__ __forceinline__ void store_tile_list(f32x16 (&acc)[TM][TN], float* smem, const Epilogue& ep, int N, int img, int y0, int x0,
+                                                int H, int W, int n0, int wm, int wn) {
+    const int tid = threadIdx.x, lane = tid & 63;
+    constexpr int LDC = BN + 4;
+    constexpr int CPR = BN / 4, RPP = 256 / CPR;
+    constexpr int PASSES = BM / RPP, G = PASSES < 8 ? PASSES : 8;
+    const int c4 = tid % CPR, rp = tid / CPR;
+    const int col = n0 + 4 * c4;
+    const bool pre_res = ep.res_mode == 2;
+    f4 qres[G];
+    auto prefetch = [&](int p0) {
+#pragma unroll
+        for (int g = 0; g < G; ++g) {
+            const int lr = (p0 + g) * RPP + rp;
+            const int y = min(y0 + lr / kWinoGroupW, H - 1), xx = min(x0 + lr % kWinoGroupW, W - 1);
+            if (pre_res) qres[g] = *reinterpret_cast<const f4*>(ep.res + (((long)img * (H >> 1) + (y >> 1)) * (W >> 1) + (xx >> 1)) * ep.ldr + min(col, N - 4));
+        }
+    };
+    prefetch(0);
+    float* Cs = smem;
+    {
+        const int i = lane & 31, h = lane >> 5;
+#pragma unroll
+        for (int tm = 0; tm < TM; ++tm)
+#pragma unroll
+            for (int tn = 0; tn < TN; ++tn)
+#pragma unroll
+                for (int r = 0; r < 16; ++r)
+                    Cs[(wm + tm * 32 + (r & 3) + 8 * (r >> 2) + 4 * h) * LDC + wn + tn * 32 + i] = acc[tm][tn][r];
+    }
+    __syncthreads();
+    if (col >= N) return;
+    float4 sc = make_float4(1.f, 1.f, 1.f, 1.f), sh = make_float4(0.f, 0.f, 0.f, 0.f);
+    if (ep.scale) sc = *reinterpret_cast<const float4*>(ep.scale + col);
+    if (ep.shift) sh = *reinterpret_cast<const float4*>(ep.shift + col);
+#pragma unroll
+    for (int p0 = 0; p0 < PASSES; p0 += G) {
+        if (p0 > 0) prefetch(p0);
+#pragma unroll
+        for (int g = 0; g < G; ++g) {
+            const int lr = (p0 + g) * RPP + rp;
+            const int y = y0 + lr / kWinoGroupW, xx = x0 + lr % kWinoGroupW;
+            float4 v = *reinterpret_cast<const float4*>(&Cs[lr * LDC + 4 * c4]);
+            v.x = v.x * sc.x + sh.x; v.y = v.y * sc.y + sh.y; v.z = v.z * sc.z + sh.z; v.w = v.w * sc.w + sh.w;
+            if (pre_res) { v.x += qres[g][0]; v.y += qres[g][1]; v.z += qres[g][2]; v.w += qres[g][3]; }
+            if (ep.relu) { v.x = fmaxf(v.x, 0.f); v.y = fmaxf(v.y, 0.f); v.z = fmaxf(v.z, 0.f); v.w = fmaxf(v.w, 0.f); }
+            if (y < H && xx < W) *reinterpret_cast<float4*>(ep.C + (((long)img * H + y) * W + xx) * ep.ldc + col) = v;
+        }
+    }
+}
+
 template <int BM, int BN, class AL, class BL>
 __device__ __forceinline__ void igemm_mainloop(const AL& al, const BL& bl, float* smem, int m0, int n0, int kbeg, int kend,
                                                f32x16 (&acc)[BM / 64][BN / 64], int wm, int wn) {
@@ -786,6 +884,7 @@
 
 int conv2d_bf16x3(const dc_conv_desc* d, bool stem, const Epilogue& ep, int M, int N, int K, int bm, int bn, int split, void* workspace,
                   size_t workspace_bytes, hipStream_t s);
+int conv2d_bf16x3_tiles(const dc_conv_desc* d, const Epilogue& ep, const int* tiles, const int* count, hipStream_t s);
 
 bool conv_pw_stream_supported(const dc_conv_desc* d, const Epilogue& ep);
 int conv2d_pointwise_stream(const dc_conv_desc* d, const Epilogue& ep, int M, int N, hipStream_t s);
diff --git a/image-captioning_amd/csrc/roialign.hip b/image-captioning_amd/csrc/roialign.hip
--- a/image-captioning_amd/csrc/roialign.hip
+++ b/image-captioning_amd/csrc/roialign.hip
@@ -178,6 +178,8 @@
 struct RoiGroupsArgs {
     dc_roi_groups_desc d;
     int gy[4], gx[4], off[5];
+    int* lat_list;
+    int* lat_count;
 };
 
 __global__ __launch_bounds__(RG_THREADS) void roi_tile_groups_kernel(RoiGroupsArgs a) {
@@ -240,18 +242,46 @@
         const int hi = tid == 3 ? below[0] : (tid == 2 ? below[3] : (tid == 1 ? below[2] : below[1]));
         d.counts[tid] = hi - lo;
     }
+    if (a.lat_list == nullptr) return;
+    const int n0 = a.off[1], gy0 = a.gy[0], gx0 = a.gx[0], gpi0 = gy0 * gx0;
+    int listed = 0;
+    for (int c0 = 0; c0 < n0; c0 += RG_THREADS) {
+        const int i = c0 + tid;
+        bool on = false;
+        if (i < n0) {
+            const int img = i / gpi0, gr = i - img * gpi0, y = gr / gx0, x = gr - y * gx0;
+            const int* m = marks + img * gpi0;
+            for (int yy = max(y - 1, 0); yy <= min(y + 1, gy0 - 1); ++yy)
+                for (int xx = max(x - 1, 0); xx <= min(x + 1, gx0 - 1); ++xx) on = on || m[yy * gx0 + xx] != 0;
+        }
+        const unsigned long long b = __ballot(on);
+        if (lane == 0) wsum[0][wave] = __popcll(b);
+        __syncthreads();
+        int before = 0, all = 0;
+#pragma unroll
+        for (int w = 0; w < RG_WAVES; ++w) {
+            before += w < wave ? wsum[0][w] : 0;
+            all += wsum[0][w];
+        }
+        if (on) a.lat_list[listed + before + __popcll(b & ((1ull << lane) - 1ull))] = i;
+        listed += all;
+        __syncthreads();
+    }
+    if (tid == 0) a.lat_count[0] = listed;
 }
 
 }
 
 using namespace dcap;
 
-extern "C" int dc_roi_tile_groups(const dc_roi_groups_desc* d, void* stream) {
+static int roi_tile_groups_launch(const dc_roi_groups_desc* d, int32_t* lat_list, int32_t* lat_count, void* stream) {
     DC_REQUIRE(d && d->boxes && d->marks && d->counts, DC_EINVAL, "dc_roi_tile_groups: null pointer");
     DC_REQUIRE(d->B > 0 && d->R > 0 && d->pool > 0, DC_EINVAL, "dc_roi_tile_groups: bad B/R/pool");
     DC_REQUIRE(aligned16(d->boxes), DC_EALIGN, "dc_roi_tile_groups: boxes not 16-byte aligned");
     RoiGroupsArgs a;
     a.d = *d;
+    a.lat_list = lat_list;
+    a.lat_count = lat_count;
     long off = 0;
     for (int l = 0; l < 4; ++l) {
         DC_REQUIRE(d->lists[l] && d->Hs[l] > 0 && d->Ws[l] > 0, DC_EINVAL, "dc_roi_tile_groups: bad level %d", l);
@@ -266,6 +296,13 @@
     return check_launch("roi_tile_groups_kernel");
 }
 
+extern "C" int dc_roi_tile_groups(const dc_roi_groups_desc* d, void* stream) { return roi_tile_groups_launch(d, nullptr, nullptr, stream); }
+
+extern "C" int dc_roi_tile_groups_lateral(const dc_roi_groups_desc* d, int32_t* lat_list, int32_t* lat_count, void* stream) {
+    DC_REQUIRE(lat_list && lat_count, DC_EINVAL, "dc_roi_tile_groups_lateral: null lateral list / count");
+    return roi_tile_groups_launch(d, lat_list, lat_count, stream);
+}
+
 extern "C" int dc_roi_align_pyramid_bwd_f32(const dc_roialign_desc* d, void* stream) {
     DC_REQUIRE(d && d->boxes && d->out, DC_EINVAL, "dc_roi_align_pyramid_bwd: null pointer");
     DC_REQUIRE(d->B > 0 && d->R > 0 && d->pool > 0 && d->pool <= RA_MAX_POOL && d->C > 0 && (d->C & 3) == 0 && d->C <= 1024, DC_EINVAL,
diff --git a/image-captioning_amd/encoder.py b/image-captioning_amd/encoder.py
--- a/image-captioning_amd/encoder.py
+++ b/image-captioning_amd/encoder.py
@@ -313,7 +313,14 @@
         self.sparse_rois = (self.rpn is None and not self.fast_bf16 and not self.train_stages and not self._external_bn and len(pops) == 4 and
                             all(op[0] == "conv" and op[2] == "fpn_p%d" % (2 + i) and op[2] not in self._external and op[1].w_wino_b3
                                 for i, op in enumerate(pops)))
+        self._lat_tiles = False
+        lat = self._ops[self._n_lateral - 1]
+        if self.sparse_rois and lat[0] == "conv" and lat[2] == "fpn_c2p2" and lat[1].math == _lib.MATH_BF16X3:
+            bm, bn, sk = C.c_int(), C.c_int(), C.c_int()
+            check(self.lib.dc_conv2d_tile_config(C.byref(lat[1]), C.byref(bm), C.byref(bn), C.byref(sk)), "dc_conv2d_tile_config")
+            self._lat_tiles = (bm.value, bn.value, sk.value) == (128, 128, 1)
         self._roi_groups = None
+        self._roi_levels = None
         self._roi_boxes = {}
         if self.rpn is not None:
             from .utils import generate_pyramid_anchors
@@ -473,12 +480,23 @@
         cs.run(body, warm_calls=1, propagate=True)
 
     def _run_rois(self, boxes):
-        g = ops.roi_tile_groups(boxes, self._roi_groups, float(self.H * self.W), 7)
+        g = ops.roi_tile_groups(boxes, self._roi_groups, float(self.H * self.W), 7, lateral=self._lat_tiles)
         stream = C.c_void_p(torch.cuda.current_stream().cuda_stream)
-        for l, op in enumerate(self._ops[self._n_lateral:]):
-            rc = self.lib.dc_conv2d_winograd_groups_f32(C.byref(op[1]), C.c_void_p(g.lists[l].data_ptr()), g.count_ptr(l), stream)
+        if self._lat_tiles:
+            op = self._ops[self._n_lateral - 1]
+            rc = self.lib.dc_conv2d_nhwc_tiles_f32(C.byref(op[1]), C.c_void_p(g.lat_list.data_ptr()), C.c_void_p(g.lat_count.data_ptr()), stream)
             if rc:
-                check(rc, "dc_conv2d_winograd_groups_f32(%s)" % op[2])
+                check(rc, "dc_conv2d_nhwc_tiles_f32(%s)" % op[2])
+        if self._roi_levels is None:
+            descs, ptrs = (ConvDesc * 4)(), (C.c_void_p * 4)()
+            for l, op in enumerate(self._ops[self._n_lateral:]):
+                descs[l] = op[1]
+                ptrs[l] = g.lists[l].data_ptr()
+            self._roi_levels = (descs, ptrs)
+        descs, ptrs = self._roi_levels
+        rc = self.lib.dc_conv2d_winograd_levels_f32(descs, 4, ptrs, C.c_void_p(g.counts.data_ptr()), stream)
+        if rc:
+            check(rc, "dc_conv2d_winograd_levels_f32(fpn_p2..p5)")
 
     def forward_rois(self, images_u8, boxes_norm, out=None, before_align=None):
         if not self.sparse_rois:
@@ -497,7 +515,7 @@
         if boxes is None:
             boxes = self._roi_boxes[R] = torch.zeros((self.B, R, 4), dtype=torch.float32, device=self.device)
         boxes.copy_(boxes_norm, non_blocking=bool(boxes_norm.is_cuda or boxes_norm.is_pinned()))
-        self._run_part("lat", lambda: self._run_ops(0, self._n_lateral))
+        self._run_part("lat", lambda: self._run_ops(0, self._n_lateral - (1 if self._lat_tiles else 0)))
         self._run_part("rois%d" % R, lambda: self._run_rois(boxes))
         if before_align is not None:
             before_align()
diff --git a/image-captioning_amd/ops.py b/image-captioning_amd/ops.py
--- a/image-captioning_amd/ops.py
+++ b/image-captioning_amd/ops.py
@@ -520,12 +520,14 @@
         self.lists = [torch.zeros(self.B * n, dtype=torch.int32, device=device) for n in self.per_image]
         self.counts = torch.zeros(4, dtype=torch.int32, device=device)
         self.marks = torch.zeros(self.B * sum(self.per_image), dtype=torch.int32, device=device)
+        self.lat_list = torch.zeros(self.B * self.per_image[0], dtype=torch.int32, device=device)
+        self.lat_count = torch.zeros(1, dtype=torch.int32, device=device)
 
     def count_ptr(self, level):
         return C.c_void_p(self.counts.data_ptr() + 4 * level)
 
 
-def roi_tile_groups(boxes, groups, image_area, pool=7):
+def roi_tile_groups(boxes, groups, image_area, pool=7, lateral=False):
     lib = _lib.load()
     _chk(boxes, name="boxes")
     B, R, _ = boxes.shape
@@ -538,8 +540,38 @@
         d.lists[i] = groups.lists[i].data_ptr()
     d.boxes, d.image_area = boxes.data_ptr(), float(image_area)
     d.marks, d.counts = groups.marks.data_ptr(), groups.counts.data_ptr()
-    check(lib.dc_roi_tile_groups(C.byref(d), _stream()), "dc_roi_tile_groups")
+    if lateral:
+        check(lib.dc_roi_tile_groups_lateral(C.byref(d), _ptr(groups.lat_list), _ptr(groups.lat_count), _stream()), "dc_roi_tile_groups_lateral")
+    else:
+        check(lib.dc_roi_tile_groups(C.byref(d), _stream()), "dc_roi_tile_groups")
     return groups
+
+
+def conv2d_tiles(x, w_packed, tile_list, count, out, scale=None, shift=None, residual=None, res_mode=0, relu=False, split_k=1,
+                 math=_lib.MATH_BF16X3):
+    lib = _lib.load()
+    _chk(x, name="x"), _chk(w_packed, name="w"), _chk(out, name="out")
+    _chk(tile_list, torch.int32, "tile_list"), _chk(count, torch.int32, "count")
+    N, H, W, Cin = x.shape
+    Cout = w_packed.shape[0]
+    if not x.is_contiguous() or not w_packed.is_contiguous() or not out.is_contiguous() or tuple(out.shape) != (N, H, W, Cout):
+        raise _lib.DcapError("conv2d_tiles: x, w and out must be contiguous, out [N,H,W,Cout]")
+    if tuple(w_packed.shape) != (Cout, Cin):
+        raise _lib.DcapError("conv2d_tiles: w must be the packed kernel of a 1x1 layer, [Cout][Cin]")
+    if tile_list.numel() < N * lib.dc_conv2d_winograd_group_count(H, W) or count.numel() < 1:
+        raise _lib.DcapError("conv2d_tiles: the list must have room for every tile group of the map")
+    if residual is not None and (not _chk(residual, name="residual").is_contiguous() or tuple(residual.shape) != (N, H // 2, W // 2, Cout)):
+        raise _lib.DcapError("conv2d_tiles: the upsample-add operand must be contiguous [N,H/2,W/2,Cout]")
+    d = ConvDesc()
+    d.N, d.H, d.W, d.Cin = N, H, W, Cin
+    d.Cout, d.kh, d.kw, d.stride, d.pad_t, d.pad_l, d.Ho, d.Wo = Cout, 1, 1, 1, 0, 0, H, W
+    d.x, d.w, d.y = x.data_ptr(), w_packed.data_ptr(), out.data_ptr()
+    d.scale = None if scale is None else _chk(scale, name="scale").data_ptr()
+    d.shift = None if shift is None else _chk(shift, name="shift").data_ptr()
+    d.residual = None if residual is None else residual.data_ptr()
+    d.res_mode, d.relu, d.split_k, d.math = int(res_mode), int(relu), int(split_k), int(math)
+    check(lib.dc_conv2d_nhwc_tiles_f32(C.byref(d), _ptr(tile_list), _ptr(count), _stream()), "dc_conv2d_nhwc_tiles_f32")
+    return out
 
 
 def conv2d_winograd_groups(x, w_packed, w_wino_b3, group_list, count, out, scale=None, shift=None, relu=False):
@@ -564,6 +596,39 @@
     d.w_wino_b3 = _chk(w_wino_b3, torch.int16, "w_wino_b3").data_ptr()
     check(lib.dc_conv2d_winograd_groups_f32(C.byref(d), _ptr(group_list), _ptr(count), _stream()), "dc_conv2d_winograd_groups_f32")
     return out
+
+
+def conv2d_winograd_levels(xs, ws_packed, ws_wino_b3, lists, counts, outs, scales=None, shifts=None, relu=False):
+    lib = _lib.load()
+    n = len(xs)
+    if not 1 <= n <= 4 or any(len(v) != n for v in (ws_packed, ws_wino_b3, lists, outs)):
+        raise _lib.DcapError("conv2d_winograd_levels: one to four levels, every argument one entry per level")
+    _chk(counts, torch.int32, "counts")
+    if counts.numel() < n:
+        raise _lib.DcapError("conv2d_winograd_levels: counts must hold one entry per level")
+    descs, ptrs = (ConvDesc * n)(), (C.c_void_p * n)()
+    for l in range(n):
+        x, w, u, out = xs[l], ws_packed[l], ws_wino_b3[l], outs[l]
+        _chk(x, name="x"), _chk(w, name="w"), _chk(out, name="out"), _chk(lists[l], torch.int32, "list")
+        N, H, W, Cin = x.shape
+        Cout = w.shape[0]
+        if not x.is_contiguous() or not out.is_contiguous() or tuple(out.shape) != (N, H, W, Cout):
+            raise _lib.DcapError("conv2d_winograd_levels: x and out must be contiguous [N,H,W,C]")
+        if not u.is_contiguous() or u.numel() != 48 * Cin * Cout:
+            raise _lib.DcapError("conv2d_winograd_levels: w_wino_b3 must be the contiguous winograd_pack_b3() of the layer's kernel")
+        if lists[l].numel() < N * lib.dc_conv2d_winograd_group_count(H, W):
+            raise _lib.DcapError("conv2d_winograd_levels: a list must have room for every tile group of its layer")
+        d = descs[l]
+        d.N, d.H, d.W, d.Cin = N, H, W, Cin
+        d.Cout, d.kh, d.kw, d.stride, d.pad_t, d.pad_l, d.Ho, d.Wo = Cout, 3, 3, 1, 1, 1, H, W
+        d.x, d.w, d.y = x.data_ptr(), w.data_ptr(), out.data_ptr()
+        d.scale = None if scales is None or scales[l] is None else _chk(scales[l], name="scale").data_ptr()
+        d.shift = None if shifts is None or shifts[l] is None else _chk(shifts[l], name="shift").data_ptr()
+        d.relu = int(relu[l] if isinstance(relu, (list, tuple)) else relu)
+        d.w_wino_b3 = _chk(u, torch.int16, "w_wino_b3").data_ptr()
+        ptrs[l] = lists[l].data_ptr()
+    check(lib.dc_conv2d_winograd_levels_f32(descs, n, ptrs, _ptr(counts), _stream()), "dc_conv2d_winograd_levels_f32")
+    return outs
 
 
 def subsample2(x, out=None):
diff --git a/include/dcap.h b/include/dcap.h
--- a/include/dcap.h
+++ b/include/dcap.h
@@ -190,6 +190,10 @@
 int dc_conv2d_winograd_group_count(int H, int W);
 int dc_conv2d_winograd_groups_f32(const dc_conv_desc* d, const int32_t* groups, const int32_t* count, void* stream);
 
+int dc_conv2d_winograd_levels_f32(const dc_conv_desc* d, int nlevels, const int32_t* const* lists, const int32_t* counts, void* stream);
+int dc_roi_tile_groups_lateral(const dc_roi_groups_desc* d, int32_t* lat_list, int32_t* lat_count, void* stream);
+int dc_conv2d_nhwc_tiles_f32(const dc_conv_desc* d, const int32_t* tiles, const int32_t* count, void* stream);
+
 int dc_subsample2_f32(const float* x, float* y, int N, int H, int W, int C, void* stream);
 
 typedef struct {
```
